# IGLICT/GaussianMesh

Hardware: AMD Instinct MI355X
Metric: frames/sec (fwd), 1M Gaussians @1080p, deform+render (higher is better)
Workload: dtype f32; 1 GPU; C3: 1000000 Gaussians bound to 15k-face torus, per-frame mesh deform + SH colour + forward render 1920x1080, 64-camera orbit, views sharded by rank; gaussians=1000000, width=1920, height=1080, sh_degree=3, frames_per_launch=4, vertex_rs=gm_mesh_rs per frame, hip_streams=4, emission_policy=2, image_only=True, work_hint=True, cov6=True, depth_plan=False, frames_redone=0, parallelism=views x1

## Files before the change

### gaussianmesh_amd/_lib.py

```python
import ctypes as C
import os
import re
import subprocess

_HERE = os.path.dirname(os.path.abspath(__file__))
CSRC = os.path.join(_HERE, "csrc")
SO_PATH = os.path.join(CSRC, "libgmesh_hip.so")
HEADER = os.path.join(os.path.dirname(_HERE), "include", "gmesh_hip.h")
_lib = None

vp, i32, i64, f32, f64, sz = C.c_void_p, C.c_int, C.c_int64, C.c_float, C.c_double, C.c_size_t

GM_BATCH_MAX = 8
GM_SCENE_OBJECTS_MAX = 32
GM_ARAP_BATCH_MAX = 64


class BatchFrame(C.Structure):
    _fields_ = [("packed", vp), ("viewmatrix", vp), ("projmatrix", vp), ("cam_pos", vp), ("tan_fovx", f32), ("tan_fovy", f32),
                ("geom_buffer", vp), ("binning_buffer", vp), ("image_buffer", vp), ("out_color", vp), ("radii", vp), ("status_host", vp)]


SIGNATURES = {
    "gm_abi_version": (i32, []),
    "gm_last_error": (C.c_char_p, []),
    "gm_geom_bytes": (sz, [i32]),
    "gm_image_bytes": (sz, [i32, i32]),
    "gm_work_hint_bytes": (sz, [i32, i32]),
    "gm_binning_bytes": (sz, [i64]),
    "gm_forward_0": (i32, [vp, i32, i32, i32, vp, i32, i32, vp, vp, vp, vp, vp, f32, vp, vp, vp, vp, vp, f32, f32, i32,
                           vp, i32, vp, C.POINTER(i32)]),
    "gm_forward_0_async": (i32, [i32, vp, i32, i32, i32, vp, i32, i32, vp, vp, vp, vp, vp, f32, vp, vp, vp, vp, vp, f32, f32, i32,
                                 vp, i32, vp, vp, vp]),
    "gm_forward_1": (i32, [vp, vp, vp, i32, i32, i32, i32, vp, i32, i32, vp, vp, vp, vp, vp, f32, vp, vp, vp, vp, vp,
                           f32, f32, i32, vp, vp, i32, vp]),
    "gm_backward": (i32, [i32, i32, i32, i32, vp, i32, i32, vp, vp, vp, vp, f32, vp, vp, vp, vp, vp, f32, f32, vp, vp, vp,
                          vp, vp, vp, vp, vp, vp, vp, vp, vp, vp, vp, i32, vp]),
    "gm_backward_p": (i32, [i32, i32, i32, i32, i32, vp, i32, i32, vp, vp, vp, vp, f32, vp, vp, vp, vp, vp, f32, f32, vp, vp, vp,
                            vp, vp, vp, vp, vp, vp, vp, vp, vp, vp, vp, i32, vp]),
    "gm_backward_aux": (i32, [i32, i32, i32, i32, i32, vp, i32, i32, vp, vp, vp, vp, f32, vp, vp, vp, vp, vp, f32, f32, vp, vp, vp,
                              vp, vp, vp, vp, vp, vp, vp, vp, vp, vp, vp, vp, vp, vp, i32, vp]),
    "gm_backward_sh_step": (i32, [i32, i32, i32, i32, i32, vp, i32, i32, vp, vp, vp, f32, vp, vp, vp, vp, vp, f32, f32, vp, vp, vp, vp, vp, vp, vp, vp, vp, vp,
                                  vp, i32, vp, vp, f32, f32, f64, f64, f64, i32, i32, vp]),
    "gm_mark_visible": (i32, [i32, vp, vp, vp, vp, vp]),
    "gm_geom_field": (vp, [vp, i32, C.c_char_p]),
    "gm_splat_floats": (i32, []),
    "gm_image_field": (vp, [vp, i32, i32, C.c_char_p]),
    "gm_binning_field": (vp, [vp, i64, i32, i32, i32, C.c_char_p]),
    "gm_knn_workspace_bytes": (sz, [i32]),
    "gm_knn": (i32, [i32, vp, vp, vp, sz, vp]),
    "gm_knn_nearest_workspace_bytes": (sz, [i32, i32]),
    "gm_knn_nearest": (i32, [i32, vp, i32, vp, vp, vp, vp, sz, vp]),
    "gm_closest_face_workspace_bytes": (sz, [i32, i32]),
    "gm_closest_face": (i32, [i32, vp, i32, vp, i32, vp, vp, vp, vp, vp, sz, vp]),
    "gm_arap_workspace_bytes": (sz, [i32]),
    "gm_arap_solve": (i32, [i32, vp, vp, vp, vp, vp, vp, i32, i32, f64, vp, vp, vp, sz, vp]),
    "gm_arap_grid_workspace_bytes": (sz, [i32]),
    "gm_arap_solve_grid": (i32, [i32, vp, vp, vp, vp, vp, vp, i32, i32, f64, vp, vp, vp, sz, vp]),
    "gm_arap_batch_workspace_bytes": (sz, [i32, i32, i32]),
    "gm_arap_solve_batch": (i32, [i32, i32, i32, vp, vp, vp, vp, vp, vp, i32, i32, f64, vp, vp, vp, sz, vp]),
    "gm_ray_mesh_workspace_bytes": (sz, [i32, i32]),
    "gm_ray_mesh": (i32, [i32, vp, vp, i32, vp, i32, vp, f32, f32, vp, vp, vp, vp, sz, vp]),
    "gm_mesh_geodesic_workspace_bytes": (sz, [i32, i32, i32]),
    "gm_mesh_geodesic": (i32, [i32, vp, vp, vp, i32, vp, vp, f32, i32, i32, vp, vp, vp, sz, vp]),
    "gm_tsdf_integrate": (i32, [i32, i32, i32, vp, vp, vp, vp, i32, i32, i32, C.POINTER(f32), f32, f32, f32, i32, vp, vp, vp]),
    "gm_surface_nets_workspace_bytes": (sz, [i32, i32, i32]),
    "gm_surface_nets": (i32, [i32, i32, i32, C.POINTER(f32), f32, vp, vp, f32, i32, vp, i32, vp, vp, vp, sz, vp]),
    "gm_deform": (i32, [i32, vp, vp, vp, vp, vp, vp, vp, vp, vp, vp, vp, vp]),
    "gm_sh_colors": (i32, [i32, i32, i32, vp, vp, vp, vp, vp, vp]),
    "gm_deform_shade": (i32, [i32, i32, i32, vp, vp, vp, vp, vp, vp, vp, vp, vp, vp, vp, vp, vp, vp, vp]),
    "gm_pack_mesh_state": (i32, [i32, vp, vp, vp, vp]),
    "gm_forward_0_deformed_async": (i32, [i32, vp, i32, i32, i32, i32, i32, vp, vp, vp, vp, vp, vp, vp, vp, vp, vp, f32, f32, vp, vp, vp, vp,
                                          i32, vp, vp, vp]),
    "gm_forward_0_deformed_stream_async": (i32, [i32, vp, i32, i32, i32, i32, i32, vp, vp, vp, vp, vp, vp, vp, vp, vp, vp, f32, f32, vp, vp, vp, vp,
                                                 i32, vp, vp, vp, vp, vp, i32]),
    "gm_depth_plan_bytes": (sz, []),
    "gm_depth_slab_bytes": (sz, [i32]),
    "gm_forward_1_geom": (i32, [i32, vp, vp, vp, i32, i32, i64, vp, i32, i32, vp, i32, vp, vp, i32, vp]),
    "gm_forward_1_aux": (i32, [i32, vp, vp, vp, i32, i32, i64, vp, i32, i32, vp, i32, vp, vp, i32, vp, vp, vp]),
    "gm_forward_status_async": (i32, [vp, i32, vp, vp]),
    "gm_forward_deformed_batch_async": (i32, [i32, i32, C.POINTER(BatchFrame), i32, i32, i32, i32, i32, vp, vp, vp, vp, vp, vp, vp, i64, i32, vp, i32, vp]),
    "gm_forward_deformed_batch_aux_async": (i32, [i32, i32, C.POINTER(BatchFrame), i32, i32, i32, i32, i32, vp, vp, vp, vp, vp, vp, vp, i64, i32, vp,
                                                  i32, vp, C.POINTER(vp), C.POINTER(vp)]),
    "gm_forward_scene_batch_async": (i32, [i32, i32, C.POINTER(BatchFrame), i32, i32, i32, i32, i32, i32, C.POINTER(i32), C.POINTER(C.c_uint),
                                           vp, vp, vp, vp, vp, vp, vp, vp, vp, i64, i32, vp, i32, vp]),
    "gm_mesh_rs_packed_batch": (i32, [i32, i32, i32, vp, C.POINTER(vp), vp, vp, vp, C.POINTER(vp), vp]),
    "gm_deform_shade_packed": (i32, [i32, i32, i32, vp, vp, vp, vp, vp, vp, vp, vp, vp, vp, vp, vp, vp]),
    "gm_cov_to_scale_rot": (i32, [i32, vp, vp, vp, vp]),
    "gm_sh_rotate": (i32, [i32, i32, i32, vp, vp, vp, vp]),
    "gm_mesh_rs": (i32, [i32, i32, vp, vp, vp, vp, vp, vp, vp, vp, vp]),
    "gm_mesh_rs_packed": (i32, [i32, i32, vp, vp, vp, vp, vp, vp, vp]),
    "gm_mesh_activate_fwd": (i32, [i32, f32] + [vp] * 10 + [vp] * 4 + [f32, vp] + [vp]),
    "gm_mesh_activate_bwd": (i32, [i32, f32] + [vp] * 10 + [vp] * 4 + [vp] * 5 + [f32, vp] + [vp]),
    "gm_plain_activate_fwd": (i32, [i32] + [vp] * 4 + [vp] * 4 + [i32, i32, vp]),
    "gm_plain_activate_bwd": (i32, [i32] + [vp] * 3 + [vp] * 4 + [i32, i32] + [vp] * 4 + [vp]),
    "gm_adam_step": (i32, [i32, vp, vp, vp, vp, vp, vp, vp, vp, vp, f64, f64, f64, i32, vp]),
    "gm_adam_step_active": (i32, [i32, vp, vp, vp, vp, vp, vp, vp, vp, vp, vp, f64, f64, f64, i32, vp]),
    "gm_densify_stats": (i32, [i32, vp, vp, vp, vp, vp, vp]),
    "gm_ssim_partials": (i64, [i32, i32, i32]),
    "gm_ssim_fwd": (i32, [vp, vp, i32, i32, i32, vp, vp, vp, vp, vp]),
    "gm_ssim_bwd": (i32, [vp, vp, vp, vp, vp, i32, i32, i32, vp, vp, vp, vp]),
    "gm_loss_combine": (i32, [vp, i64, f64, f64, f64, vp, vp]),
    "gm_ssim_fwd_u8": (i32, [vp, vp, vp, i64, vp, i32, i32, i32, vp, vp, vp, vp, vp]),
    "gm_ssim_bwd_u8": (i32, [vp, vp, vp, i64, vp, vp, vp, vp, i32, i32, i32, vp, vp, vp, vp]),
    "gm_profile_enable": (None, [i32]),
    "gm_profile_reset": (None, []),
    "gm_profile_read": (i32, [C.c_char_p, C.POINTER(C.c_double), C.POINTER(i64)]),
    "gm_debug_render_trace": (None, [vp]),
    "gm_debug_bucket_trace": (None, [vp]),
}


def header_symbols():
    txt = open(HEADER).read()
    txt = re.sub(r"/\*.*?\*/", "", txt, flags=re.S)
    return sorted(set(re.findall(r"\b(gm_[a-z0-9_]+)\s*\(", txt)))


def build(verbose=False):
    cmd = ["make", "-C", CSRC, "-j8"]
    res = subprocess.run(cmd, stdout=subprocess.PIPE, stderr=subprocess.STDOUT, text=True)
    if verbose or res.returncode != 0:
        print(res.stdout)
    if res.returncode != 0:
        raise RuntimeError("building libgmesh_hip.so failed")
    return SO_PATH


def lib():
    global _lib
    if _lib is None:
        if not os.path.exists(SO_PATH):
            raise ImportError(
                "gaussianmesh_amd: %s is missing. Build it with `python -c 'import __graft_entry__ as g; g.build()'` "
                "(or `make -C gaussianmesh_amd/csrc`). There is no CPU fallback." % SO_PATH)
        l = C.CDLL(SO_PATH)
        for name, (res, args) in SIGNATURES.items():
            fn = getattr(l, name)
            fn.restype = res
            fn.argtypes = args
        if l.gm_abi_version() != 3:
            raise ImportError("libgmesh_hip.so ABI version mismatch")
        _lib = l
    return _lib


class GmeshError(RuntimeError):
    pass


def check(rc):
    if rc != 0:
        raise GmeshError("libgmesh_hip: error %d: %s" % (rc, lib().gm_last_error().decode()))
```

### gaussianmesh_amd/csrc/gm_api.hip

```cpp
#include "gm_common.h"
#include <cmath>
#include <cstdlib>
#include "../../include/gmesh_hip.h"
#include <cstdarg>
#include <cstdio>
#include <cstring>
#include <mutex>
#include <vector>

namespace gm {

static thread_local char g_err[512] = "";

void set_error(const char* fmt, ...) {
  va_list ap;
  va_start(ap, fmt);
  vsnprintf(g_err, sizeof g_err, fmt, ap);
  va_end(ap);
}
int hip_fail(hipError_t e, const char* what, const char* file, int line) {
  set_error("HIP error %d (%s) at %s:%d in %s", (int)e, hipGetErrorString(e), file, line, what);
  return GM_ERR_HIP;
}

// ... 167 lines not shown
                       float tan_fovy, int prefiltered, int* radii, int debug, void* stream, int* num_rendered_host,
                       void* count_event) {
  if (int rc = check_policy(emission_policy)) return rc;
  FILL_ARGS(a, emission_policy)
  if (int rc = check_raster_args(a)) return rc;
  if (P == 0) { if (num_rendered_host) *num_rendered_host = 0; return GM_OK; }
  if (!geom_buffer) { set_error("geom_buffer is null"); return GM_ERR_INVALID_ARG; }
  GeomState g = GeomState::from(geom_buffer, (size_t)P);
  if (int rc = launch_arm_counters(g, a.stream)) return rc;
  if (int rc = launch_preprocess(a, g, radii)) return rc;
  return order_and_count(g, P, debug, a.stream, num_rendered_host, count_event);
}

size_t gm_depth_plan_bytes(void) { return sizeof(uint32_t) * GM_PLAN_WORDS; }
size_t gm_depth_slab_bytes(int P) {
  DepthSlab d = DepthSlab::from(nullptr, (size_t)(P > 0 ? P : 1));
  return (size_t)d.end + 256;
}

int gm_forward_0_deformed_async(int emission_policy, void* geom_buffer, int P, int deg, int M, int width, int height, const int* tri,
                                const float* w, const float* packed, const float* cov, const float* pos, const float* shs,
                                const float* opacities, const float* viewmatrix, const float* projmatrix, const float* cam_pos,
                                float tan_fovx, float tan_fovy, float* pos_out, float* cov6_out, float* rgb_out, int* radii, int debug,
                                void* stream, int* num_rendered_host, void* count_event) {
  return gm_forward_0_deformed_stream_async(emission_policy, geom_buffer, P, deg, M, width, height, tri, w, packed, cov, pos, shs, opacities,
                                            viewmatrix, projmatrix, cam_pos, tan_fovx, tan_fovy, pos_out, cov6_out, rgb_out, radii, debug, stream,
                                            num_rendered_host, count_event, nullptr, nullptr, 0);
}

int gm_forward_0_deformed_stream_async(int emission_policy, void* geom_buffer, int P, int deg, int M, int width, int height, const int* tri,
                                       const float* w, const float* packed, const float* cov, const float* pos, const float* shs,
                                       const float* opacities, const float* viewmatrix, const float* projmatrix, const float* cam_pos,
                                       float tan_fovx, float tan_fovy, float* pos_out, float* cov6_out, float* rgb_out, int* radii,
                                       int debug, void* stream, int* num_rendered_host, void* count_event, void* depth_slab,
                                       unsigned int* depth_plan, int flags) {
  if (int rc = check_policy(emission_policy)) return rc;
  if (flags & ~(GM_STREAM_DIRECT | GM_STREAM_COV6)) { set_error("gm_forward_0_deformed_stream: unknown flags 0x%x", flags); return GM_ERR_INVALID_ARG; }
  const int direct = flags & GM_STREAM_DIRECT;
  const bool cov6 = (flags & GM_STREAM_COV6) != 0;
  if (direct && (!depth_slab || !depth_plan)) { set_error("gm_forward_0_deformed_stream: direct placement needs depth_slab and depth_plan"); return GM_ERR_INVALID_ARG; }
  if (P < 0 || width <= 0 || height <= 0) { set_error("invalid sizes P=%d W=%d H=%d", P, width, height); return GM_ERR_INVALID_ARG; }
  if (int rc = check_tile_grid(width, height)) return rc;
  if (P == 0) { if (num_rendered_host) *num_rendered_host = 0; return GM_OK; }
  if (deg < 0 || deg > 3 || M != 16) { set_error("gm_forward_0_deformed: needs SH rows of M == 16 coefficients, degree 0..3"); return GM_ERR_INVALID_ARG; }
  if (!geom_buffer || !tri || !w || !packed || !cov || !pos || !shs || !opacities || !viewmatrix || !projmatrix || !cam_pos) {
    set_error("gm_forward_0_deformed: null required input"); return GM_ERR_INVALID_ARG;
  }
  const int nout = (pos_out != nullptr) + (cov6_out != nullptr) + (rgb_out != nullptr);
  if (nout != 0 && nout != 3) { set_error("gm_forward_0_deformed: pass pos_out, cov6_out and rgb_out together or none"); return GM_ERR_INVALID_ARG; }
  RasterArgs a{};
  a.P = P; a.D = deg; a.M = M; a.W = width; a.H = height; a.opacities = opacities; a.viewmatrix = viewmatrix; a.projmatrix = projmatrix;
  a.cam_pos = cam_pos; a.scale_modifier = 1.0f; a.tan_fovx = tan_fovx; a.tan_fovy = tan_fovy; a.debug = debug; a.tile_cull = emission_policy;
  a.stream = reinterpret_cast<hipStream_t>(stream);
  if (TileGrid(width, height, emission_policy).ptiles > 65536) { set_error("too many list tiles for emission policy %d", emission_policy); return GM_ERR_INVALID_ARG; }
  GeomState g = GeomState::from(geom_buffer, (size_t)P);
  if (direct) {
    DepthSlab d = DepthSlab::from(depth_slab, (size_t)P);
    if (int rc = launch_arm_direct(g, d, depth_plan, a.stream)) return rc;
    GM_HIP(hipMemsetD32Async(reinterpret_cast<hipDeviceptr_t>(g.counters + GM_CNT_DEPTH_STALE), 1, 1, a.stream));
    if (int rc = launch_deform_shade_pre(a, g, radii, deg, tri, w, packed, cov, pos, shs, pos_out, cov6_out, rgb_out, &d, cov6)) return rc;
    if (debug_stop_after() == 1) return GM_OK;
    return launch_depth_order_direct(g, d, depth_plan, P, debug, a.stream, num_rendered_host, reinterpret_cast<hipEvent_t>(count_event));
  }
  if (int rc = launch_arm_counters(g, a.stream)) return rc;
  if (int rc = launch_deform_shade_pre(a, g, radii, deg, tri, w, packed, cov, pos, shs, pos_out, cov6_out, rgb_out, nullptr, cov6)) return rc;
  if (int rc = order_and_count(g, P, debug, a.stream, num_rendered_host, count_event)) return rc;
  if (depth_plan && debug_stop_after() != 1) return launch_publish_depth_plan(g, depth_plan, a.stream);
  return GM_OK;
}

static int forward_1_impl(int emission_policy, void* geom_buffer, void* binning_buffer, void* image_buffer, int P, int num_rendered,
                          int64_t binning_capacity, const float* background, int width, int height, float* out_color, int debug, void* stream,
                          int* status_host, int flags, unsigned int* work_hint, bool aux, float* out_depth, float* out_alpha) {
  if (int rc = check_policy(emission_policy)) return rc;
  if (flags & ~(GM_FWD_IMAGE_ONLY | GM_FWD_EXACT_EXPONENT)) { set_error("unknown flags 0x%x", flags); return GM_ERR_INVALID_ARG; }
  if ((flags & GM_FWD_IMAGE_ONLY) && (flags & GM_FWD_EXACT_EXPONENT)) {
    set_error("GM_FWD_EXACT_EXPONENT is for a forward a backward pass follows: not together with GM_FWD_IMAGE_ONLY"); return GM_ERR_INVALID_ARG;
  }
  if (P < 0 || width <= 0 || height <= 0) { set_error("invalid sizes P=%d W=%d H=%d", P, width, height); return GM_ERR_INVALID_ARG; }
  if (int rc = check_tile_grid(width, height)) return rc;
  if (!image_buffer || !out_color || !background) { set_error("null image_buffer / out_color / background"); return GM_ERR_INVALID_ARG; }
  const bool device_count = num_rendered < 0;
  const int64_t cap = device_count ? binning_capacity : (int64_t)num_rendered;
  if (cap < 0) { set_error("negative binning capacity"); return GM_ERR_INVALID_ARG; }
  if (P > 0 && (!geom_buffer || (cap > 0 && !binning_buffer))) { set_error("null scratch buffer"); return GM_ERR_INVALID_ARG; }
  hipStream_t st = reinterpret_cast<hipStream_t>(stream);
  const int mode = emission_policy;
  ImageState img = ImageState::from(image_buffer, width, height);
  const int tiles = TileGrid(width, height, mode).ptiles;
  if (tiles > 65536) { set_error("too many list tiles for emission policy %d", mode); return GM_ERR_INVALID_ARG; }
  GeomState g = GeomState::from(geom_buffer, (size_t)(P > 0 ? P : 1));
  BinningState b = BinningState::from(binning_buffer, (size_t)cap);
  const int slot = sort_final_slot(tiles);
  bool order_done = false;
  if (const int stop = debug_stop_after()) {
    if (stop <= 2) return GM_OK;
    if (stop == 3) return launch_duplicate(g, b, P, width, height, mode, (size_t)cap, debug, st);
  }
  if (P > 0 && cap > 0) {
    if (int rc = launch_duplicate(g, b, P, width, height, mode, (size_t)cap, debug, st)) return rc;
    if (int rc = launch_tile_sort(g, b, img, (size_t)cap, device_count ? g.counters + GM_CNT_RENDERED : nullptr, tiles, &order_done, work_hint, debug, st)) return rc;
    if (slot == 0)
      if (int rc = launch_tile_ranges(g, b, slot, img, (int)cap, device_count ? g.counters + GM_CNT_RENDERED : nullptr, tiles, debug, st)) return rc;
  } else {
    GM_HIP(hipMemsetAsync(img.ranges, 0, sizeof(uint2) * (size_t)tiles, st));
  }
  if (!order_done)
    if (int rc = launch_tile_order(img, tiles, work_hint, debug, st)) return rc;
  if (status_host && P == 0) {
    status_host[0] = 0; status_host[1] = 0; status_host[2] = mode; status_host[3] = 0;
    status_host = nullptr;
  }
  if (debug_stop_after() == 4) return GM_OK;
  return launch_render_fwd(g, b.pairs[slot], img, width, height, mode, background, out_color, status_host, (flags & GM_FWD_IMAGE_ONLY) != 0,
                           work_hint, debug, st, (flags & GM_FWD_EXACT_EXPONENT) != 0, nullptr, out_depth, out_alpha, aux,
                           P > 0 ? g.counters : nullptr);
}

int gm_forward_1_geom(int emission_policy, void* geom_buffer, void* binning_buffer, void* image_buffer, int P, int num_rendered,
                      int64_t binning_capacity, const float* background, int width, int height, float* out_color, int debug, void* stream,
                      int* status_host, int flags, unsigned int* work_hint) {
  return forward_1_impl(emission_policy, geom_buffer, binning_buffer, image_buffer, P, num_rendered, binning_capacity, background, width, height,
                        out_color, debug, stream, status_host, flags, work_hint, false, nullptr, nullptr);
}

static bool overlaps(const float* a, size_t na, const float* b, size_t nb) {
  return a && b && a < b + nb && b < a + na;
}

int gm_forward_1_aux(int emission_policy, void* geom_buffer, void* binning_buffer, void* image_buffer, int P, int num_rendered,
                     int64_t binning_capacity, const float* background, int width, int height, float* out_color, int debug, void* stream,
                     int* status_host, int flags, unsigned int* work_hint, float* out_depth, float* out_alpha) {
  if (width > 0 && height > 0) {
    const size_t HW = (size_t)width * height;
    if (overlaps(out_depth, HW, out_color, 3 * HW) || overlaps(out_alpha, HW, out_color, 3 * HW) || overlaps(out_depth, HW, out_alpha, HW)) {
      set_error("gm_forward_1_aux: out_depth / out_alpha overlap out_color or each other"); return GM_ERR_INVALID_ARG;
    }
  }
  return forward_1_impl(emission_policy, geom_buffer, binning_buffer, image_buffer, P, num_rendered, binning_capacity, background, width, height,
                        out_color, debug, stream, status_host, flags, work_hint, true, out_depth, out_alpha);
}

struct SceneRows {
  int n_objects;
  const int* object_rows;
  const unsigned int* deformed;
  const float *scales, *rots;
};

static int check_scene_batch(const char* who, const SceneRows& sc, int K, const gm_batch_frame* frames, int P, int width, int height,
                             int64_t binning_capacity, const int* tri, const float* w, const float* cov) {
  const int n = sc.n_objects;
  if (n < 0 || n > GM_SCENE_OBJECTS_MAX) { set_error("%s: n_objects = %d, not in 0..GM_SCENE_OBJECTS_MAX (%d)", who, n, GM_SCENE_OBJECTS_MAX); return GM_ERR_INVALID_ARG; }
  for (int j = 0; j <= n; j++) {
    const int r = sc.object_rows[j];
    if (r < 0 || r > P || (j > 0 && r < sc.object_rows[j - 1])) {
      set_error("%s: object_rows must ascend within [0, P = %d]: object_rows[%d] = %d", who, P, j, r); return GM_ERR_INVALID_ARG;
    }
  }
  for (int k = 0; k < K; k++) {
    const unsigned int m = sc.deformed[k];
    if (n < 32 && (m >> n)) { set_error("%s: frame %d: deformed mask 0x%x has a bit at or above n_objects = %d", who, k, m, n); return GM_ERR_INVALID_ARG; }
    if (m && !frames[k].packed) { set_error("%s: frame %d deforms objects (mask 0x%x) but packed is NULL", who, k, m); return GM_ERR_INVALID_ARG; }
    if (m && (!tri || !w || !cov)) { set_error("%s: frame %d deforms objects: tri / w / cov are required", who, k); return GM_ERR_INVALID_ARG; }
  }
  struct Range { uintptr_t a; size_t n; int k; const char* what; };
  Range rg[6 * GM_BATCH_MAX];
  int nr = 0;
  const size_t HW = (size_t)width * height;
  for (int k = 0; k < K; k++) {
    const gm_batch_frame& f = frames[k];
    rg[nr++] = {reinterpret_cast<uintptr_t>(f.geom_buffer), gm_geom_bytes(P), k, "geometry"};
    rg[nr++] = {reinterpret_cast<uintptr_t>(f.binning_buffer), gm_binning_bytes(binning_capacity), k, "binning"};
    rg[nr++] = {reinterpret_cast<uintptr_t>(f.image_buffer), gm_image_bytes(width, height), k, "image"};
    rg[nr++] = {reinterpret_cast<uintptr_t>(f.out_color), 3 * HW * sizeof(float), k, "out_color"};
    if (f.radii) rg[nr++] = {reinterpret_cast<uintptr_t>(f.radii), (size_t)P * sizeof(int), k, "radii"};
    if (f.status_host) rg[nr++] = {reinterpret_cast<uintptr_t>(f.status_host), 4 * sizeof(int), k, "status_host"};
  }
  for (int x = 0; x < nr; x++)
    for (int y = x + 1; y < nr; y++)
      if (rg[x].a < rg[y].a + rg[y].n && rg[y].a < rg[x].a + rg[x].n) {
        set_error("%s: frame %d's %s buffer overlaps frame %d's %s buffer", who, rg[x].k, rg[x].what, rg[y].k, rg[y].what);
        return GM_ERR_INVALID_ARG;
      }
  return GM_OK;
}

static int forward_batch_impl(const char* who, int emission_policy, int K, const gm_batch_frame* frames, int P, int deg, int M, int width, int height,
                              const int* tri, const float* w, const float* cov, const float* pos, const float* shs, const float* opacities,
                              const float* background, int64_t binning_capacity, int flags, unsigned int* work_hint, int debug, void* stream,
                              bool aux, float* const* out_depth, float* const* out_alpha, const SceneRows* scene = nullptr) {
  if (int rc = check_policy(emission_policy)) return rc;
  if (K < 1 || K > GM_BATCH_MAX || !frames) { set_error("%s: 1..%d frames", who, GM_BATCH_MAX); return GM_ERR_INVALID_ARG; }
  if (flags & ~(scene ? GM_BATCH_IMAGE_ONLY : (GM_BATCH_IMAGE_ONLY | GM_BATCH_COV6))) { set_error("%s: unknown flags 0x%x", who, flags); return GM_ERR_INVALID_ARG; }
  if (P <= 0 || width <= 0 || height <= 0) { set_error("%s: invalid sizes P=%d W=%d H=%d (an empty cloud goes through the single-frame calls)", who, P, width, height); return GM_ERR_INVALID_ARG; }
  if (deg < 0 || deg > 3 || M != 16) { set_error("%s: needs SH rows of M == 16 coefficients, degree 0..3", who); return GM_ERR_INVALID_ARG; }
  if (scene ? (!pos || !scene->scales || !scene->rots || !shs || !opacities || !background || !scene->object_rows || !scene->deformed)
            : (!tri || !w || !cov || !pos || !shs || !opacities || !background)) {
    set_error("%s: null required input", who); return GM_ERR_INVALID_ARG;
  }
  if (binning_capacity <= 0) { set_error("%s: binning_capacity must be positive (sync-free second half)", who); return GM_ERR_INVALID_ARG; }
  if (int rc = check_tile_grid(width, height)) return rc;
  const TileGrid tg(width, height, emission_policy);
  if (tg.ptiles > (1 << GM_BUCKET_BITS)) {
    set_error("%s: %dx%d has %d list tiles under policy %d; a batch needs the one-pass tile sort (<= 2048)", who, width, height, tg.ptiles, emission_policy);
    return GM_ERR_INVALID_ARG;
  }
  hipStream_t st = reinterpret_cast<hipStream_t>(stream);
  BatchFrameArgs fr[GM_BATCH_MAX];
  BatchOfs B{};
  B.frames = K;
  for (int k = 0; k < K; k++) {
    const gm_batch_frame& f = frames[k];
    if ((!scene && !f.packed) || !f.viewmatrix || !f.projmatrix || !f.cam_pos || !f.geom_buffer || !f.binning_buffer || !f.image_buffer || !f.out_color) {
      set_error("%s: frame %d has a null pointer", who, k); return GM_ERR_INVALID_ARG;
    }
    if ((reinterpret_cast<uintptr_t>(f.geom_buffer) | reinterpret_cast<uintptr_t>(f.binning_buffer) | reinterpret_cast<uintptr_t>(f.image_buffer)) & 255) {
      set_error("%s: frame %d: scratch buffers must be 256-byte aligned", who, k); return GM_ERR_INVALID_ARG;
    }
    for (int j = 0; j < k; j++)
      if (frames[j].geom_buffer == f.geom_buffer || frames[j].binning_buffer == f.binning_buffer || frames[j].image_buffer == f.image_buffer || frames[j].out_color == f.out_color) {
        set_error("%s: frames %d and %d share a buffer", who, j, k); return GM_ERR_INVALID_ARG;
      }
    fr[k].packed = f.packed; fr[k].viewmatrix = f.viewmatrix; fr[k].projmatrix = f.projmatrix; fr[k].cam_pos = f.cam_pos;
    fr[k].tan_fovx = f.tan_fovx; fr[k].tan_fovy = f.tan_fovy; fr[k].radii = f.radii;
    fr[k].g = GeomState::from(f.geom_buffer, (size_t)P);
    B.geom.d[k] = (long long)(reinterpret_cast<intptr_t>(f.geom_buffer) - reinterpret_cast<intptr_t>(frames[0].geom_buffer));
    B.binning.d[k] = (long long)(reinterpret_cast<intptr_t>(f.binning_buffer) - reinterpret_cast<intptr_t>(frames[0].binning_buffer));
    B.image.d[k] = (long long)(reinterpret_cast<intptr_t>(f.image_buffer) - reinterpret_cast<intptr_t>(frames[0].image_buffer));
    B.color.d[k] = (long long)(reinterpret_cast<intptr_t>(f.out_color) - reinterpret_cast<intptr_t>(frames[0].out_color));
    B.status[k] = f.status_host;
  }
  if (scene)
    if (int rc = check_scene_batch(who, *scene, K, frames, P, width, height, binning_capacity, tri, w, cov)) return rc;
  if (aux) {
    const size_t HW = (size_t)width * height;
    const float* r[3 * GM_BATCH_MAX];
    for (int k = 0; k < K; k++) {
      if ((out_depth && !out_depth[k]) || (out_alpha && !out_alpha[k])) { set_error("%s: frame %d: null map pointer in a non-null array", who, k); return GM_ERR_INVALID_ARG; }
      r[k] = frames[k].out_color; r[K + k] = out_depth ? out_depth[k] : nullptr; r[2 * K + k] = out_alpha ? out_alpha[k] : nullptr;
    }
    for (int i = K; i < 3 * K; i++) {
      if (!r[i]) continue;
      const int k = i % K;
      if (reinterpret_cast<uintptr_t>(r[i]) & 3) { set_error("%s: frame %d: unaligned map pointer", who, k); return GM_ERR_INVALID_ARG; }
      for (int j = 0; j < 3 * K; j++)
        if (j != i && overlaps(r[i], HW, r[j], j < K ? 3 * HW : HW)) {
          set_error("%s: frame %d's %s map overlaps a colour image or another map of the batch", who, k, i < 2 * K ? "depth" : "alpha");
          return GM_ERR_INVALID_ARG;
        }
      (i < 2 * K ? B.depth : B.alpha).d[k] = (long long)(reinterpret_cast<intptr_t>(r[i]) - reinterpret_cast<intptr_t>(r[i - k]));
    }
  }
  GeomState g = fr[0].g;
  ImageState img = ImageState::from(frames[0].image_buffer, width, height);
  BinningState b = BinningState::from(frames[0].binning_buffer, (size_t)binning_capacity);
  if (int rc = launch_arm_counters(g, st, &B)) return rc;
  if (scene) {
    if (int rc = launch_scene_shade_pre_batch(K, fr, scene->deformed, scene->n_objects, scene->object_rows, P, deg, width, height, emission_policy, pos,
                                              scene->scales, scene->rots, shs, opacities, tri, w, cov, debug, st)) return rc;
  } else if (int rc = launch_deform_shade_pre_batch(K, fr, P, deg, width, height, emission_policy, tri, w, cov, pos, shs, opacities, (flags & GM_BATCH_COV6) != 0, debug, st)) {
    return rc;
  }
  if (int rc = launch_depth_order(g, P, debug, st, nullptr, nullptr, &B)) return rc;
  if (int rc = launch_duplicate(g, b, P, width, height, emission_policy, (size_t)binning_capacity, debug, st, &B)) return rc;
  bool order_done = false;
  if (int rc = launch_tile_sort(g, b, img, (size_t)binning_capacity, g.counters + GM_CNT_RENDERED, tg.ptiles, &order_done, work_hint, debug, st, &B)) return rc;
  if (!order_done) { set_error("%s: internal: the tile pass did not produce the dispatch order", who); return GM_ERR_INVALID_ARG; }
  return launch_render_fwd(g, b.pairs[sort_final_slot(tg.ptiles)], img, width, height, emission_policy, background, frames[0].out_color, frames[0].status_host,
                           (flags & GM_BATCH_IMAGE_ONLY) != 0, work_hint, debug, st, false, &B,
                           aux && out_depth ? out_depth[0] : nullptr, aux && out_alpha ? out_alpha[0] : nullptr, aux, aux ? g.counters : nullptr);
}

int gm_forward_deformed_batch_async(int emission_policy, int K, const gm_batch_frame* frames, int P, int deg, int M, int width, int height,
                                    const int* tri, const float* w, const float* cov, const float* pos, const float* shs, const float* opacities,
                                    const float* background, int64_t binning_capacity, int flags, unsigned int* work_hint, int debug, void* stream) {
  return forward_batch_impl("gm_forward_deformed_batch", emission_policy, K, frames, P, deg, M, width, height, tri, w, cov, pos, shs, opacities,
                            background, binning_capacity, flags, work_hint, debug, stream, false, nullptr, nullptr);
}

int gm_forward_deformed_batch_aux_async(int emission_policy, int K, const gm_batch_frame* frames, int P, int deg, int M, int width, int height,
                                        const int* tri, const float* w, const float* cov, const float* pos, const float* shs, const float* opacities,
                                        const float* background, int64_t binning_capacity, int flags, unsigned int* work_hint, int debug, void* stream,
                                        float* const* out_depth, float* const* out_alpha) {
  return forward_batch_impl("gm_forward_deformed_batch_aux", emission_policy, K, frames, P, deg, M, width, height, tri, w, cov, pos, shs, opacities,
                            background, binning_capacity, flags, work_hint, debug, stream, true, out_depth, out_alpha);
}

int gm_forward_scene_batch_async(int emission_policy, int K, const gm_batch_frame* frames, int P, int deg, int M, int width, int height,
                                 int n_objects, const int* object_rows, const unsigned int* deformed, const float* pos, const float* scales,
                                 const float* rots, const float* shs, const float* opacities, const int* tri, const float* w, const float* cov,
                                 const float* background, int64_t binning_capacity, int flags, unsigned int* work_hint, int debug, void* stream) {
  const SceneRows scene{n_objects, object_rows, deformed, scales, rots};
  return forward_batch_impl("gm_forward_scene_batch", emission_policy, K, frames, P, deg, M, width, height, tri, w, cov, pos, shs, opacities,
                            background, binning_capacity, flags, work_hint, debug, stream, false, nullptr, nullptr, &scene);
}


int gm_mesh_rs_packed_batch(int K, int Vm, int nfaces, const float* V0, const float* const* V1, const int* faces, const int* adj_offsets,
                            const int* adj_faces, float* const* packed, void* stream) {
  if (K < 1 || K > GM_BATCH_MAX || Vm < 0 || nfaces < 0 || !V1 || !packed || (Vm > 0 && (!V0 || !adj_offsets || (nfaces > 0 && (!faces || !adj_faces))))) {
    set_error("gm_mesh_rs_packed_batch: bad args"); return GM_ERR_INVALID_ARG;
  }
  for (int k = 0; k < K; k++)
    if (Vm > 0 && (!V1[k] || !packed[k] || (reinterpret_cast<uintptr_t>(packed[k]) & 15))) { set_error("gm_mesh_rs_packed_batch: frame %d: null or unaligned pointer", k); return GM_ERR_INVALID_ARG; }
  return launch_mesh_rs_batch(K, Vm, V0, V1, faces, adj_offsets, adj_faces, packed, reinterpret_cast<hipStream_t>(stream));
}

int gm_forward_status_async(void* geom_buffer, int P, int* status_host, void* stream) {
  if (!status_host) { set_error("status_host is null"); return GM_ERR_INVALID_ARG; }
  if (P <= 0) { status_host[0] = 0; status_host[1] = 0; status_host[2] = 0; status_host[3] = 0; return GM_OK; }
  if (!geom_buffer) { set_error("geom_buffer is null"); return GM_ERR_INVALID_ARG; }
  GeomState g = GeomState::from(geom_buffer, (size_t)P);
  GM_HIP(hipMemcpyAsync(status_host, g.counters, 4 * sizeof(uint32_t), hipMemcpyDeviceToHost, reinterpret_cast<hipStream_t>(stream)));
  return GM_OK;
}

int gm_forward_0(void* geom_buffer, int P, int D, int M, const float* background, int width, int height,
                 const float* means3D, const float* shs, const float* colors_precomp, const float* opacities,
                 const float* scales, float scale_modifier, const float* rotations, const float* cov3D_precomp,
                 const float* viewmatrix, const float* projmatrix, const float* cam_pos, float tan_fovx,
                 float tan_fovy, int prefiltered, int* radii, int debug, void* stream, int* num_rendered) {
  if (!num_rendered) { set_error("num_rendered is null"); return GM_ERR_INVALID_ARG; }
  *num_rendered = 0;
  if (int rc = gm_forward_0_async(GM_POLICY_DEFAULT, geom_buffer, P, D, M, background, width, height, means3D, shs, colors_precomp, opacities,
                                  scales, scale_modifier, rotations, cov3D_precomp, viewmatrix, projmatrix, cam_pos, tan_fovx, tan_fovy,
                                  prefiltered, radii, debug, stream, nullptr, nullptr)) return rc;
  if (P == 0) return GM_OK;
  GeomState g = GeomState::from(geom_buffer, (size_t)P);
  uint32_t rw[2] = {0u, 0u};
  hipStream_t st = reinterpret_cast<hipStream_t>(stream);
  GM_HIP(hipMemcpyAsync(rw, g.counters + GM_CNT_RENDERED, 2 * sizeof(uint32_t), hipMemcpyDeviceToHost, st));
  GM_HIP(hipStreamSynchronize(st));
  const uint32_t r = rw[0];
  if (rw[1]) { set_error("Point is filtered although prefiltered is set. This shouldn't happen!"); return GM_ERR_INVALID_ARG; }
  if (r > 0x7FFFFFFFu) { set_error("num_rendered overflows int32 (%u)", r); return GM_ERR_INVALID_ARG; }
  *num_rendered = (int)r;
  return GM_OK;
}

int gm_forward_1(void* geom_buffer, void* binning_buffer, void* image_buffer, int P, int D, int M, int num_rendered,
                 const float* background, int width, int height, const float* means3D, const float* shs,
                 const float* colors_precomp, const float* opacities, const float* scales, float scale_modifier,
                 const float* rotations, const float* cov3D_precomp, const float* viewmatrix, const float* projmatrix,
                 const float* cam_pos, float tan_fovx, float tan_fovy, int prefiltered, float* out_color, int* radii,
                 int debug, void* stream) {
  FILL_ARGS(a, GM_POLICY_DEFAULT)
  if (int rc = check_raster_args(a)) return rc;
  (void)radii;
  if (num_rendered < 0) { set_error("negative num_rendered"); return GM_ERR_INVALID_ARG; }
  return gm_forward_1_geom(GM_POLICY_DEFAULT, geom_buffer, binning_buffer, image_buffer, P, num_rendered, 0, background, width, height, out_color,
                           debug, stream, nullptr, 0, nullptr);
}

static int backward_impl(int emission_policy, int P, int D, int M, int R, const float* background, int width, int height, const float* means3D,
                         const float* shs, const float* colors_precomp, const float* scales, float scale_modifier,
                         const float* rotations, const float* cov3D_precomp, const float* viewmatrix, const float* projmatrix,
                         const float* campos, float tan_fovx, float tan_fovy, const int* radii, void* geom_buffer,
                         void* binning_buffer, void* image_buffer, const float* dL_dpix, float* dL_dmean2D, float* dL_dconic,
                         float* dL_dopacity, float* dL_dcolor, float* dL_dmean3D, float* dL_dcov3D, float* dL_dsh,
                         float* dL_dscale, float* dL_drot, int debug, void* stream, const ShAdamArgs* sh_adam,
                         const float* dL_ddepth = nullptr, const float* dL_dalpha = nullptr, float* dL_dz = nullptr) {
  if (int rc = check_policy(emission_policy)) return rc;
  const float* opacities = reinterpret_cast<const float*>(1);
  const float* cam_pos = campos;
  const int prefiltered = 0;
  FILL_ARGS(a, emission_policy)
  if (int rc = check_raster_args(a)) return rc;
  if (P == 0) return GM_OK;
  if (!geom_buffer || !image_buffer || !dL_dpix || !dL_dmean2D || !dL_dopacity || (!shs && !dL_dcolor) ||
      !dL_dmean3D || (!scales && !dL_dcov3D) || (shs && !dL_dsh && !sh_adam) || (scales && (!dL_dscale || !dL_drot))) {
    set_error("gm_backward: null buffer"); return GM_ERR_INVALID_ARG;
  }
  GeomState g = GeomState::from(geom_buffer, (size_t)P);
  ImageState img = ImageState::from(image_buffer, width, height);
  BinningState b = BinningState::from(binning_buffer, (size_t)(R > 0 ? R : 0));
  const int slot = sort_final_slot(TileGrid(width, height, a.tile_cull).ptiles);
  GM_HIP(hipMemsetAsync(g.grad_acc, 0, sizeof(float) * 12 * (size_t)P, a.stream));
  if (R > 0) {
    if (!binning_buffer) { set_error("gm_backward: null binning buffer"); return GM_ERR_INVALID_ARG; }
    if (int rc = launch_render_bwd(g, b.pairs[slot], img, width, height, a.tile_cull, background, dL_dpix, debug, a.stream,
                                   dL_ddepth || dL_dalpha, dL_ddepth, dL_dalpha)) return rc;
  }
  if (int rc = launch_preprocess_bwd(a, g, radii, dL_dmean2D, dL_dconic, dL_dopacity, dL_dcolor, dL_dmean3D, dL_dcov3D, dL_dsh,
                                     dL_dscale, dL_drot, sh_adam)) return rc;
  if (dL_ddepth || dL_dz) return launch_depth_grad(P, g, viewmatrix, dL_dmean3D, dL_dz, a.stream);
  return GM_OK;
}

int gm_backward_aux(int emission_policy, int P, int D, int M, int R, const float* background, int width, int height, const float* means3D,
                    const float* shs, const float* colors_precomp, const float* scales, float scale_modifier,
                    const float* rotations, const float* cov3D_precomp, const float* viewmatrix, const float* projmatrix,
                    const float* campos, float tan_fovx, float tan_fovy, const int* radii, void* geom_buffer,
                    void* binning_buffer, void* image_buffer, const float* dL_dpix, float* dL_dmean2D, float* dL_dconic,
                    float* dL_dopacity, float* dL_dcolor, float* dL_dmean3D, float* dL_dcov3D, float* dL_dsh,
                    float* dL_dscale, float* dL_drot, const float* dL_ddepth, const float* dL_dalpha, float* dL_dz, int debug, void* stream) {
  if (P > 0) {
    const size_t n = (size_t)P;
    if (overlaps(dL_dz, n, dL_dmean3D, 3 * n) || overlaps(dL_dz, n, dL_dmean2D, 3 * n) || overlaps(dL_dz, n, dL_dopacity, n)) {
      set_error("gm_backward_aux: dL_dz overlaps another gradient output"); return GM_ERR_INVALID_ARG;
    }
  }
  return backward_impl(emission_policy, P, D, M, R, background, width, height, means3D, shs, colors_precomp, scales, scale_modifier, rotations, cov3D_precomp,
                       viewmatrix, projmatrix, campos, tan_fovx, tan_fovy, radii, geom_buffer, binning_buffer, image_buffer, dL_dpix, dL_dmean2D, dL_dconic,
                       dL_dopacity, dL_dcolor, dL_dmean3D, dL_dcov3D, dL_dsh, dL_dscale, dL_drot, debug, stream, nullptr, dL_ddepth, dL_dalpha, dL_dz);
}

int gm_backward_p(int emission_policy, int P, int D, int M, int R, const float* background, int width, int height, const float* means3D,
                  const float* shs, const float* colors_precomp, const float* scales, float scale_modifier,
                  const float* rotations, const float* cov3D_precomp, const float* viewmatrix, const float* projmatrix,
                  const float* campos, float tan_fovx, float tan_fovy, const int* radii, void* geom_buffer,
                  void* binning_buffer, void* image_buffer, const float* dL_dpix, float* dL_dmean2D, float* dL_dconic,
                  float* dL_dopacity, float* dL_dcolor, float* dL_dmean3D, float* dL_dcov3D, float* dL_dsh,
                  float* dL_dscale, float* dL_drot, int debug, void* stream) {
  return backward_impl(emission_policy, P, D, M, R, background, width, height, means3D, shs, colors_precomp, scales, scale_modifier, rotations, cov3D_precomp,
                       viewmatrix, projmatrix, campos, tan_fovx, tan_fovy, radii, geom_buffer, binning_buffer, image_buffer, dL_dpix, dL_dmean2D, dL_dconic,
                       dL_dopacity, dL_dcolor, dL_dmean3D, dL_dcov3D, dL_dsh, dL_dscale, dL_drot, debug, stream, nullptr);
}

int gm_backward_sh_step(int emission_policy, int P, int D, int M, int R, const float* background, int width, int height, const float* means3D,
                        float* shs, const float* scales, float scale_modifier, const float* rotations, const float* cov3D_precomp,
                        const float* viewmatrix, const float* projmatrix, const float* campos, float tan_fovx, float tan_fovy, const int* radii,
                        void* geom_buffer, void* binning_buffer, void* image_buffer, const float* dL_dpix, float* dL_dmean2D, float* dL_dopacity,
                        float* dL_dmean3D, float* dL_dcov3D, float* dL_dscale, float* dL_drot, int rows, float* exp_avg, float* exp_avg_sq,
                        float lr_dc, float lr_rest, double beta1, double beta2, double eps, int step, int debug, void* stream) {
  if (!shs || M != 16 || D < 0 || D > 3) { set_error("gm_backward_sh_step: needs the [P,16,3] SH operand"); return GM_ERR_INVALID_ARG; }
  if (rows < 0 || rows > P || !exp_avg || !exp_avg_sq || step < 1) { set_error("gm_backward_sh_step: bad optimizer state (rows %d of %d, step %d)", rows, P, step); return GM_ERR_INVALID_ARG; }
  ShAdamArgs ad;
  ad.p = shs; ad.m = exp_avg; ad.v = exp_avg_sq; ad.rows = rows;
  ad.b1 = (float)beta1; ad.b2 = (float)beta2; ad.c1 = (float)(1.0 - beta1); ad.c2 = (float)(1.0 - beta2); ad.eps = (float)eps;
  const double corr = sqrt(1.0 - pow(beta2, (double)step)) / (1.0 - pow(beta1, (double)step));
  ad.step_lo = (float)(lr_dc * corr); ad.step_hi = (float)(lr_rest * corr);
  return backward_impl(emission_policy, P, D, M, R, background, width, height, means3D, shs, nullptr, scales, scale_modifier, rotations, cov3D_precomp,
                       viewmatrix, projmatrix, campos, tan_fovx, tan_fovy, radii, geom_buffer, binning_buffer, image_buffer, dL_dpix, dL_dmean2D, nullptr,
                       dL_dopacity, nullptr, dL_dmean3D, dL_dcov3D, nullptr, dL_dscale, dL_drot, debug, stream, &ad);
}

int gm_backward(int P, int D, int M, int R, const float* background, int width, int height, const float* means3D,
                const float* shs, const float* colors_precomp, const float* scales, float scale_modifier,
                const float* rotations, const float* cov3D_precomp, const float* viewmatrix, const float* projmatrix,
                const float* campos, float tan_fovx, float tan_fovy, const int* radii, void* geom_buffer,
                void* binning_buffer, void* image_buffer, const float* dL_dpix, float* dL_dmean2D, float* dL_dconic,
                float* dL_dopacity, float* dL_dcolor, float* dL_dmean3D, float* dL_dcov3D, float* dL_dsh,
                float* dL_dscale, float* dL_drot, int debug, void* stream) {
  return gm_backward_p(GM_POLICY_DEFAULT, P, D, M, R, background, width, height, means3D, shs, colors_precomp, scales, scale_modifier, rotations,
                       cov3D_precomp, viewmatrix, projmatrix, campos, tan_fovx, tan_fovy, radii, geom_buffer, binning_buffer, image_buffer,
                       dL_dpix, dL_dmean2D, dL_dconic, dL_dopacity, dL_dcolor, dL_dmean3D, dL_dcov3D, dL_dsh, dL_dscale, dL_drot, debug, stream);
}

int gm_mark_visible(int P, const float* means3D, const float* viewmatrix, const float* projmatrix, uint8_t* present,
                    void* stream) {
  (void)projmatrix;
  if (P < 0 || (P > 0 && (!means3D || !viewmatrix || !present))) { set_error("gm_mark_visible: bad args"); return GM_ERR_INVALID_ARG; }
  return launch_mark_visible(P, means3D, viewmatrix, present, reinterpret_cast<hipStream_t>(stream));
}

int gm_splat_floats(void) { return GM_SPLAT_STRIDE; }
void* gm_geom_field(void* geom_buffer, int P, const char* name) {
  GeomState g = GeomState::from(geom_buffer, (size_t)(P > 0 ? P : 1));
  if (!strcmp(name, "splat")) return g.splat;
  if (!strcmp(name, "depth_key")) return g.depth_key;
  if (!strcmp(name, "radii")) return g.radii;
  if (!strcmp(name, "tiles_touched")) return g.tiles_touched;
  if (!strcmp(name, "bin")) return g.bin;
  if (!strcmp(name, "inst16")) return g.inst16;
  if (!strcmp(name, "bin_sorted")) return g.bin_sorted;
  if (!strcmp(name, "grad_acc")) return g.grad_acc;
  if (!strcmp(name, "cov3D")) return g.cov3D;
  if (!strcmp(name, "clamped")) return g.clamped;
  if (!strcmp(name, "order")) return g.order;
  if (!strcmp(name, "bucket_start")) return g.bucket_start;
  if (!strcmp(name, "counters")) return g.counters;
  if (!strcmp(name, "bmap")) return g.bmap;
  if (!strcmp(name, "dmap")) return g.dmap;
  return nullptr;
}
void* gm_image_field(void* image_buffer, int W, int H, const char* name) {
  ImageState s = ImageState::from(image_buffer, W, H);
  if (!strcmp(name, "final_T")) return s.final_T;
  if (!strcmp(name, "n_contrib")) return s.n_contrib;
  if (!strcmp(name, "ranges")) return s.ranges;
  if (!strcmp(name, "tile_order")) return s.tile_order;
  return nullptr;
}
void* gm_binning_field(void* binning_buffer, int64_t R, int W, int H, int emission_policy, const char* name) {
  BinningState b = BinningState::from(binning_buffer, (size_t)(R > 0 ? R : 0));
  const int slot = sort_final_slot(TileGrid(W, H, emission_policy < 0 ? 0 : (emission_policy > 3 ? 3 : emission_policy)).ptiles);
  if (!strcmp(name, "pairs")) return b.pairs[slot];
  return nullptr;
}

size_t gm_knn_workspace_bytes(int P) { return knn_workspace_bytes(P); }
int gm_knn(int P, const float* points, float* meanDists, void* workspace, size_t workspace_bytes, void* stream) {
  if (P < 0 || (P > 0 && (!points || !meanDists || !workspace))) { set_error("gm_knn: bad args"); return GM_ERR_INVALID_ARG; }
  return launch_knn(P, points, meanDists, workspace, workspace_bytes, reinterpret_cast<hipStream_t>(stream));
}

size_t gm_knn_nearest_workspace_bytes(int Pq, int Pr) { return knn_nearest_workspace_bytes(Pq, Pr); }
int gm_knn_nearest(int Pq, const float* query, int Pr, const float* ref, float* out_d2, int* out_idx, void* workspace, size_t workspace_bytes,
                   void* stream) {
  if (Pq < 0 || Pr < 0) { set_error("gm_knn_nearest: negative size"); return GM_ERR_INVALID_ARG; }
  if (Pr == 0) { set_error("gm_knn_nearest: empty reference set (Pr == 0)"); return GM_ERR_INVALID_ARG; }
  if (Pq > 0 && (!query || !ref || !out_d2 || !out_idx || !workspace)) { set_error("gm_knn_nearest: null pointer"); return GM_ERR_INVALID_ARG; }
  return launch_knn_nearest(Pq, query, Pr, ref, out_d2, out_idx, workspace, workspace_bytes, reinterpret_cast<hipStream_t>(stream));
}

size_t gm_closest_face_workspace_bytes(int N, int F) { return closest_face_workspace_bytes(N, F); }
int gm_closest_face(int N, const float* points, int Vm, const float* vertices, int F, const int* faces, float* out_d2, int* out_face,
                    float* out_closest, void* workspace, size_t workspace_bytes, void* stream) {
  if (N < 0 || Vm < 0 || F < 0) { set_error("gm_closest_face: negative size N=%d Vm=%d F=%d", N, Vm, F); return GM_ERR_INVALID_ARG; }
  if (N == 0) return GM_OK;
  if (F == 0 || Vm == 0) { set_error("gm_closest_face: empty mesh (F == %d, Vm == %d)", F, Vm); return GM_ERR_INVALID_ARG; }
  if (!points || !vertices || !faces || !out_d2 || !out_face || !workspace) { set_error("gm_closest_face: null pointer"); return GM_ERR_INVALID_ARG; }
  return launch_closest_face(N, points, Vm, vertices, F, faces, out_d2, out_face, out_closest, workspace, workspace_bytes,
                             reinterpret_cast<hipStream_t>(stream));
}

size_t gm_arap_workspace_bytes(int Vm) { return arap_workspace_bytes(Vm); }
int gm_arap_solve(int Vm, const int* row_offsets, const int* cols, const double* weights, const float* V0, const unsigned char* fixed,
                  const float* V_init, int outer_iterations, int cg_iterations, double cg_tolerance, float* V_out, double* stats,
                  void* workspace, size_t workspace_bytes, void* stream) {
  return arap_solve_checked("gm_arap_solve", launch_arap_solve, Vm, row_offsets, cols, weights, V0, fixed, V_init, outer_iterations, cg_iterations,
                            cg_tolerance, V_out, stats, workspace, workspace_bytes, stream);
}

size_t gm_arap_grid_workspace_bytes(int Vm) { return arap_grid_workspace_bytes(Vm); }
int gm_arap_solve_grid(int Vm, const int* row_offsets, const int* cols, const double* weights, const float* V0, const unsigned char* fixed,
                       const float* V_init, int outer_iterations, int cg_iterations, double cg_tolerance, float* V_out, double* stats,
                       void* workspace, size_t workspace_bytes, void* stream) {
  return arap_solve_checked("gm_arap_solve_grid", launch_arap_solve_grid, Vm, row_offsets, cols, weights, V0, fixed, V_init, outer_iterations,
                            cg_iterations, cg_tolerance, V_out, stats, workspace, workspace_bytes, stream);
}

size_t gm_arap_batch_workspace_bytes(int Vm, int B, int global_step) {
  if (Vm <= 0 || B < 1 || B > GM_ARAP_BATCH_MAX || (global_step != 0 && global_step != 1)) return 0;
  return arap_batch_workspace_bytes(Vm, B, global_step);
}
int gm_arap_solve_batch(int B, int global_step, int Vm, const int* row_offsets, const int* cols, const double* weights, const float* V0,
                        const unsigned char* fixed, const float* V_init, int outer_iterations, int cg_iterations, double cg_tolerance, float* V_out,
                        double* stats, void* workspace, size_t workspace_bytes, void* stream) {
  const char* fn = "gm_arap_solve_batch";
  if (B < 1 || B > GM_ARAP_BATCH_MAX) { set_error("%s: B = %d (1 .. %d)", fn, B, GM_ARAP_BATCH_MAX); return GM_ERR_INVALID_ARG; }
  if (global_step != 0 && global_step != 1) { set_error("%s: global_step = %d (0 column, 1 grid)", fn, global_step); return GM_ERR_INVALID_ARG; }
  if (int rc = arap_args_checked(fn, B, Vm, row_offsets, cols, weights, V0, fixed, V_init, outer_iterations, cg_iterations, cg_tolerance, V_out, stats,
                                 workspace, workspace_bytes))
    return rc;
  return launch_arap_solve_batch(B, global_step, Vm, row_offsets, cols, weights, V0, fixed, V_init, outer_iterations, cg_iterations, cg_tolerance, V_out, stats,
                                 workspace, workspace_bytes, reinterpret_cast<hipStream_t>(stream));
}

size_t gm_ray_mesh_workspace_bytes(int R, int F) { return ray_mesh_workspace_bytes(R, F); }
int gm_ray_mesh(int R, const float* origins, const float* dirs, int Vm, const float* vertices, int F, const int* faces, float t_min, float t_max,
                float* out_t, int* out_face, float* out_uv, void* workspace, size_t workspace_bytes, void* stream) {
  if (R < 0 || Vm < 0 || F < 0) { set_error("gm_ray_mesh: negative size R=%d Vm=%d F=%d", R, Vm, F); return GM_ERR_INVALID_ARG; }
  if (!(t_min >= 0.f) || t_max != t_max) { set_error("gm_ray_mesh: t_min must be >= 0 and neither bound NaN"); return GM_ERR_INVALID_ARG; }
  if (R == 0) return GM_OK;
  if (F == 0 || Vm == 0) { set_error("gm_ray_mesh: empty mesh (F == %d, Vm == %d)", F, Vm); return GM_ERR_INVALID_ARG; }
  if (!origins || !dirs || !vertices || !faces || !out_t || !out_face || !workspace) { set_error("gm_ray_mesh: null pointer"); return GM_ERR_INVALID_ARG; }
  if (ray_mesh_blocks(R, F) > 0x7FFFFFFFull) {
    set_error("gm_ray_mesh: R x F too large for one launch (%llu workgroups); split the rays", ray_mesh_blocks(R, F)); return GM_ERR_INVALID_ARG;
  }
  return launch_ray_mesh(R, origins, dirs, Vm, vertices, F, faces, t_min, t_max, out_t, out_face, out_uv, workspace, workspace_bytes,
                         reinterpret_cast<hipStream_t>(stream));
}

size_t gm_mesh_geodesic_workspace_bytes(int Vm, int B, int sweeps) { return mesh_geodesic_workspace_bytes(Vm, B, sweeps); }
int gm_mesh_geodesic(int Vm, const int* row_offsets, const int* cols, const float* lengths, int B, const int* source_offsets, const int* sources,
                     float max_distance, int sweeps, int resume, float* dist, int* unsettled, void* workspace, size_t workspace_bytes, void* stream) {
  if (Vm < 0 || B < 0) { set_error("gm_mesh_geodesic: negative size Vm=%d B=%d", Vm, B); return GM_ERR_INVALID_ARG; }
  if (sweeps < 1) { set_error("gm_mesh_geodesic: sweeps must be >= 1; got %d", sweeps); return GM_ERR_INVALID_ARG; }
  if (!(max_distance >= 0.f)) { set_error("gm_mesh_geodesic: max_distance must be >= 0 and not NaN (+inf: no cutoff)"); return GM_ERR_INVALID_ARG; }
  if (Vm == 0) return GM_OK;
  if (B < 1 || B > 65535) { set_error("gm_mesh_geodesic: B must be 1 .. 65535 source sets; got %d", B); return GM_ERR_INVALID_ARG; }
  if (!row_offsets || !cols || !lengths || !source_offsets || !sources || !dist || !unsettled || !workspace) {
    set_error("gm_mesh_geodesic: null pointer"); return GM_ERR_INVALID_ARG;
  }
  return launch_mesh_geodesic(Vm, row_offsets, cols, lengths, B, source_offsets, sources, max_distance, sweeps, resume, dist, unsettled, workspace,
                              workspace_bytes, reinterpret_cast<hipStream_t>(stream));
}

#define GM_TSDF_MAX_SAMPLES (1ll << 28)
static int check_tsdf_grid(const char* fn, int nx, int ny, int nz, int least, const float* origin, float voxel) {
  if (nx < least || ny < least || nz < least) { set_error("%s: grid %d x %d x %d (every side at least %d)", fn, nx, ny, nz, least); return GM_ERR_INVALID_ARG; }
  if ((long long)nx * ny > GM_TSDF_MAX_SAMPLES || (long long)nx * ny * nz > GM_TSDF_MAX_SAMPLES) {
    set_error("%s: grid %d x %d x %d has more than 2^28 samples", fn, nx, ny, nz); return GM_ERR_INVALID_ARG;
  }
  if (!origin) { set_error("%s: null pointer (origin)", fn); return GM_ERR_INVALID_ARG; }
  if (!(voxel > 0.f) || voxel > 3.4028234e38f || !(origin[0] - origin[0] == 0.f) || !(origin[1] - origin[1] == 0.f) || !(origin[2] - origin[2] == 0.f)) {
    set_error("%s: voxel must be positive and finite, origin finite", fn); return GM_ERR_INVALID_ARG;
  }
  return 0;
}

int gm_tsdf_integrate(int K, int H, int W, const float* depth, const float* alpha, const float* views, const float* tanfov, int nx, int ny, int nz,
                      const float* origin, float voxel, float trunc, float alpha_min, int carve, float* tsdf, float* weight, void* stream) {
  if (K < 0 || H <= 0 || W <= 0 || H > (1 << 24) || W > (1 << 24)) {
    set_error("gm_tsdf_integrate: invalid sizes K=%d H=%d W=%d", K, H, W); return GM_ERR_INVALID_ARG;
  }
  if (int rc = check_tsdf_grid("gm_tsdf_integrate", nx, ny, nz, 1, origin, voxel)) return rc;
  if (!(trunc > 0.f) || trunc > 3.4028234e38f || alpha_min != alpha_min) {
    set_error("gm_tsdf_integrate: trunc must be positive and finite, alpha_min not NaN"); return GM_ERR_INVALID_ARG;
  }
  if (!tsdf || !weight) { set_error("gm_tsdf_integrate: null pointer (tsdf / weight)"); return GM_ERR_INVALID_ARG; }
  const size_t n = (size_t)nx * ny * nz, maps = (size_t)K * H * W;
  if (overlaps(tsdf, n, weight, n)) { set_error("gm_tsdf_integrate: tsdf overlaps weight"); return GM_ERR_INVALID_ARG; }
  if (K == 0) return GM_OK;
  if (!depth || !alpha || !views || !tanfov) { set_error("gm_tsdf_integrate: null pointer"); return GM_ERR_INVALID_ARG; }
  const struct { const float* p; size_t n; const char* what; } in[4] = {{depth, maps, "depth"}, {alpha, maps, "alpha"}, {views, 16 * (size_t)K, "views"},
                                                                       {tanfov, 2 * (size_t)K, "tanfov"}};
  for (int i = 0; i < 4; i++)
    if (overlaps(tsdf, n, in[i].p, in[i].n) || overlaps(weight, n, in[i].p, in[i].n)) {
      set_error("gm_tsdf_integrate: the volume overlaps %s", in[i].what); return GM_ERR_INVALID_ARG;
    }
  return launch_tsdf_integrate(K, H, W, depth, alpha, views, tanfov, nx, ny, nz, origin, voxel, trunc, alpha_min, carve, tsdf, weight,
                               reinterpret_cast<hipStream_t>(stream));
}

size_t gm_surface_nets_workspace_bytes(int nx, int ny, int nz) { return surface_nets_workspace_bytes(nx, ny, nz); }
int gm_surface_nets(int nx, int ny, int nz, const float* origin, float voxel, const float* tsdf, const float* weight, float min_weight,
                    int max_vertices, float* out_vertices, int max_faces, int* out_faces, int* out_counts, void* workspace, size_t workspace_bytes,
                    void* stream) {
  if (int rc = check_tsdf_grid("gm_surface_nets", nx, ny, nz, 2, origin, voxel)) return rc;
  if (min_weight != min_weight) { set_error("gm_surface_nets: min_weight is NaN"); return GM_ERR_INVALID_ARG; }
  if (max_vertices < 0 || max_faces < 0) { set_error("gm_surface_nets: negative capacity (%d vertices, %d faces)", max_vertices, max_faces); return GM_ERR_INVALID_ARG; }
  if (!tsdf || !weight || !out_counts || !workspace || (max_vertices > 0 && !out_vertices) || (max_faces > 0 && !out_faces)) {
    set_error("gm_surface_nets: null pointer"); return GM_ERR_INVALID_ARG;
  }
  const size_t n = (size_t)nx * ny * nz;
  const struct { const char* p; size_t n; const char* what; } rg[6] = {
      {reinterpret_cast<const char*>(tsdf), 4 * n, "tsdf"}, {reinterpret_cast<const char*>(weight), 4 * n, "weight"},
      {reinterpret_cast<const char*>(out_vertices), 12 * (size_t)max_vertices, "out_vertices"},
      {reinterpret_cast<const char*>(out_faces), 12 * (size_t)max_faces, "out_faces"}, {reinterpret_cast<const char*>(out_counts), 8, "out_counts"},
      {reinterpret_cast<const char*>(workspace), workspace_bytes, "workspace"}};
  for (int a = 0; a < 6; a++)
    for (int b = (a < 2 ? 2 : a + 1); b < 6; b++) {
      if (!rg[a].p || !rg[b].p || !rg[a].n || !rg[b].n) continue;
      if (rg[a].p < rg[b].p + rg[b].n && rg[b].p < rg[a].p + rg[a].n) {
        set_error("gm_surface_nets: %s overlaps %s", rg[a].what, rg[b].what); return GM_ERR_INVALID_ARG;
      }
    }
  return launch_surface_nets(nx, ny, nz, origin, voxel, tsdf, weight, min_weight, max_vertices, out_vertices, max_faces, out_faces, out_counts, workspace,
                             workspace_bytes, reinterpret_cast<hipStream_t>(stream));
}

int gm_deform(int N, const int* tri, const float* w, const float* dV, const float* Rv, const float* Sv,
              const float* cov, const float* pos, float* pos_out, float* cov_out, float* rot_out, float* cov6_out,
              void* stream) {
  if (N < 0 || (N > 0 && (!tri || !w || !dV || !Rv || !Sv || !cov || !pos || !pos_out || !cov_out || !rot_out))) {
    set_error("gm_deform: bad args"); return GM_ERR_INVALID_ARG;
  }
  return launch_deform(N, tri, w, dV, Rv, Sv, cov, pos, pos_out, cov_out, rot_out, cov6_out, reinterpret_cast<hipStream_t>(stream));
}

int gm_sh_colors(int N, int deg, int M, const float* pos, const float* campos, const float* rot, const float* shs,
                 float* rgb, void* stream) {
  if (N < 0 || deg < 0 || deg > 3 || M < (deg + 1) * (deg + 1) || (N > 0 && (!pos || !campos || !shs || !rgb))) {
    set_error("gm_sh_colors: bad args"); return GM_ERR_INVALID_ARG;
  }
  return launch_sh_colors(N, deg, M, pos, campos, rot, shs, rgb, reinterpret_cast<hipStream_t>(stream));
}

int gm_deform_shade(int N, int deg, int M, const int* tri, const float* w, const float* dV, const float* Rv, const float* Sv,
                    const float* cov, const float* pos, const float* shs, const float* campos, float* pos_out, float* cov6_out,
                    float* rgb_out, float* cov_out, float* rot_out, void* stream) {
  if (N < 0 || deg < 0 || deg > 3 || M < (deg + 1) * (deg + 1) ||
      (N > 0 && (!tri || !w || !dV || !Rv || !Sv || !cov || !pos || !shs || !campos || !pos_out || !cov6_out || !rgb_out)) ||
      ((cov_out == nullptr) != (rot_out == nullptr))) {
    set_error("gm_deform_shade: bad args"); return GM_ERR_INVALID_ARG;
  }
  return launch_deform_shade(N, deg, M, tri, w, dV, Rv, Sv, cov, pos, shs, campos, pos_out, cov6_out, rgb_out, cov_out, rot_out,
                             reinterpret_cast<hipStream_t>(stream));
}

int gm_pack_mesh_state(int Vm, const float* state, const float* verts, float* packed, void* stream) {
  if (Vm < 0 || (Vm > 0 && (!state || !verts || !packed))) { set_error("gm_pack_mesh_state: bad args"); return GM_ERR_INVALID_ARG; }
  if (Vm > 0 && (reinterpret_cast<uintptr_t>(packed) & 15)) { set_error("gm_pack_mesh_state: packed must be 16-byte aligned"); return GM_ERR_INVALID_ARG; }
  return launch_pack_mesh_state(Vm, state, verts, packed, reinterpret_cast<hipStream_t>(stream));
}

int gm_deform_shade_packed(int N, int deg, int M, const int* tri, const float* w, const float* packed, const float* cov,
                           const float* pos, const float* shs, const float* campos, float* pos_out, float* cov6_out,
                           float* rgb_out, float* cov_out, float* rot_out, void* stream) {
  if (N < 0 || deg < 0 || deg > 3 || M < (deg + 1) * (deg + 1) ||
      (N > 0 && (!tri || !w || !packed || !cov || !pos || !shs || !campos || !pos_out || !cov6_out || !rgb_out)) ||
      ((cov_out == nullptr) != (rot_out == nullptr))) {
    set_error("gm_deform_shade_packed: bad args"); return GM_ERR_INVALID_ARG;
  }
  return launch_deform_shade_packed(N, deg, M, tri, w, packed, cov, pos, shs, campos, pos_out, cov6_out, rgb_out, cov_out, rot_out,
                                    reinterpret_cast<hipStream_t>(stream));
}

int gm_mesh_rs(int Vm, int nfaces, const float* V0, const float* V1, const int* faces, const int* adj_offsets, const int* adj_faces,
               float* R, float* S, float* state, void* stream) {
  if (Vm < 0 || nfaces < 0 || (Vm > 0 && (!V0 || !V1 || !adj_offsets || (nfaces > 0 && (!faces || !adj_faces)) || (!R && !S && !state)))) {
    set_error("gm_mesh_rs: bad args"); return GM_ERR_INVALID_ARG;
  }
  if ((R == nullptr) != (S == nullptr)) { set_error("gm_mesh_rs: pass R and S together"); return GM_ERR_INVALID_ARG; }
  return launch_mesh_rs(Vm, V0, V1, faces, adj_offsets, adj_faces, R, S, state, nullptr, reinterpret_cast<hipStream_t>(stream));
}

int gm_mesh_rs_packed(int Vm, int nfaces, const float* V0, const float* V1, const int* faces, const int* adj_offsets, const int* adj_faces,
                      float* packed, void* stream) {
  if (Vm < 0 || nfaces < 0 || (Vm > 0 && (!V0 || !V1 || !adj_offsets || !packed || (nfaces > 0 && (!faces || !adj_faces))))) {
    set_error("gm_mesh_rs_packed: bad args"); return GM_ERR_INVALID_ARG;
  }
  if (reinterpret_cast<uintptr_t>(packed) & 15) { set_error("gm_mesh_rs_packed: packed must be 16-byte aligned"); return GM_ERR_INVALID_ARG; }
  return launch_mesh_rs(Vm, V0, V1, faces, adj_offsets, adj_faces, nullptr, nullptr, nullptr, packed, reinterpret_cast<hipStream_t>(stream));
}

int gm_cov_to_scale_rot(int N, const float* cov, float* scales, float* rots, void* stream) {
  if (N < 0 || (N > 0 && (!cov || !scales || !rots))) { set_error("gm_cov_to_scale_rot: bad args"); return GM_ERR_INVALID_ARG; }
  if (N > 0 && (reinterpret_cast<uintptr_t>(rots) & 15)) { set_error("gm_cov_to_scale_rot: rots must be 16-byte aligned"); return GM_ERR_INVALID_ARG; }
  return launch_cov_to_scale_rot(N, cov, scales, rots, reinterpret_cast<hipStream_t>(stream));
}

int gm_sh_rotate(int N, int deg, int M, const float* shs, const float* rot, float* shs_out, void* stream) {
  if (N < 0) { set_error("gm_sh_rotate: negative N = %d", N); return GM_ERR_INVALID_ARG; }
  if (N == 0) return GM_OK;
  if (deg < 0 || deg > 3) { set_error("gm_sh_rotate: degree %d out of range 0..3", deg); return GM_ERR_INVALID_ARG; }
  if (M < (deg + 1) * (deg + 1)) { set_error("gm_sh_rotate: rows of M = %d coefficients hold no degree %d", M, deg); return GM_ERR_INVALID_ARG; }
  if (!shs || !rot || !shs_out) { set_error("gm_sh_rotate: null pointer"); return GM_ERR_INVALID_ARG; }
  const size_t n = (size_t)N * (size_t)M * 3;
  if (shs_out != shs && overlaps(shs_out, n, shs, n)) { set_error("gm_sh_rotate: shs_out overlaps shs without being equal to it"); return GM_ERR_INVALID_ARG; }
  if (overlaps(shs_out, n, rot, (size_t)N * 9)) { set_error("gm_sh_rotate: shs_out overlaps rot"); return GM_ERR_INVALID_ARG; }
  return launch_sh_rotate(N, deg, M, shs, rot, shs_out, reinterpret_cast<hipStream_t>(stream));
}

int64_t gm_ssim_partials(int planes, int H, int W) {
  if (planes < 0 || H < 0 || W < 0) return 0;
  return (int64_t)planes * ((H + 31) / 32) * ((W + 31) / 32);
}

int gm_ssim_fwd(const float* img1, const float* img2, int planes, int H, int W, float* dS_dmu1, float* dS_dE11, float* dS_dE12,
                float* partial, void* stream) {
  if (planes < 0 || H < 0 || W < 0) { set_error("gm_ssim_fwd: negative size"); return GM_ERR_INVALID_ARG; }
  if (planes == 0 || H == 0 || W == 0) return GM_OK;
  if (!img1 || !img2 || !partial) { set_error("gm_ssim_fwd: null image or partial buffer"); return GM_ERR_INVALID_ARG; }
  const int nmaps = (dS_dmu1 != nullptr) + (dS_dE11 != nullptr) + (dS_dE12 != nullptr);
  if (nmaps != 0 && nmaps != 3) { set_error("gm_ssim_fwd: pass all three derivative maps or none"); return GM_ERR_INVALID_ARG; }
  if (planes > 65535) { set_error("gm_ssim_fwd: at most 65535 image planes per call"); return GM_ERR_INVALID_ARG; }
  return launch_ssim_fwd(img1, img2, planes, H, W, dS_dmu1, dS_dE11, dS_dE12, partial, reinterpret_cast<hipStream_t>(stream));
}

int gm_ssim_bwd(const float* img1, const float* img2, const float* dS_dmu1, const float* dS_dE11, const float* dS_dE12, int planes,
                int H, int W, const float* g_ssim, const float* g_l1, float* dL_dimg1, void* stream) {
  if (planes < 0 || H < 0 || W < 0) { set_error("gm_ssim_bwd: negative size"); return GM_ERR_INVALID_ARG; }
  if (planes == 0 || H == 0 || W == 0) return GM_OK;
  if (!img1 || !img2 || !dS_dmu1 || !dS_dE11 || !dS_dE12 || !g_ssim || !dL_dimg1) { set_error("gm_ssim_bwd: null argument"); return GM_ERR_INVALID_ARG; }
  if (planes > 65535) { set_error("gm_ssim_bwd: at most 65535 image planes per call"); return GM_ERR_INVALID_ARG; }
  return launch_ssim_bwd(img1, img2, dS_dmu1, dS_dE11, dS_dE12, planes, H, W, g_ssim, g_l1, dL_dimg1, reinterpret_cast<hipStream_t>(stream));
}

static int check_u8_target(const char* who, const unsigned char* rgb, const unsigned char* mask, int64_t mask_plane_stride,
                           const float* background, int planes, int H, int W) {
  char msg[160];
  if (planes != 3) { snprintf(msg, sizeof msg, "%s: an 8-bit target has 3 planes", who); set_error(msg); return GM_ERR_INVALID_ARG; }
  if (!rgb) { snprintf(msg, sizeof msg, "%s: null rgb", who); set_error(msg); return GM_ERR_INVALID_ARG; }
  if (mask && !background) { snprintf(msg, sizeof msg, "%s: a mask needs the background colour (device float[3])", who); set_error(msg); return GM_ERR_INVALID_ARG; }
  if (mask && mask_plane_stride != 0 && mask_plane_stride < (int64_t)H * W) {
    snprintf(msg, sizeof msg, "%s: mask_plane_stride is 0 (one shared plane) or at least H*W", who); set_error(msg); return GM_ERR_INVALID_ARG;
  }
  return GM_OK;
}

int gm_ssim_fwd_u8(const float* img1, const uint8_t* rgb, const uint8_t* mask, int64_t mask_plane_stride, const float* background,
                   int planes, int H, int W, float* dS_dmu1, float* dS_dE11, float* dS_dE12, float* partial, void* stream) {
  if (planes < 0 || H < 0 || W < 0) { set_error("gm_ssim_fwd_u8: negative size"); return GM_ERR_INVALID_ARG; }
  if (planes == 0 || H == 0 || W == 0) return GM_OK;
  if (!img1 || !partial) { set_error("gm_ssim_fwd_u8: null image or partial buffer"); return GM_ERR_INVALID_ARG; }
  const int nmaps = (dS_dmu1 != nullptr) + (dS_dE11 != nullptr) + (dS_dE12 != nullptr);
  if (nmaps != 0 && nmaps != 3) { set_error("gm_ssim_fwd_u8: pass all three derivative maps or none"); return GM_ERR_INVALID_ARG; }
  if (int rc = check_u8_target("gm_ssim_fwd_u8", rgb, mask, mask_plane_stride, background, planes, H, W)) return rc;
  return launch_ssim_fwd_u8(img1, rgb, mask, (size_t)mask_plane_stride, background, H, W, dS_dmu1, dS_dE11, dS_dE12, partial,
                            reinterpret_cast<hipStream_t>(stream));
}

int gm_ssim_bwd_u8(const float* img1, const uint8_t* rgb, const uint8_t* mask, int64_t mask_plane_stride, const float* background,
                   const float* dS_dmu1, const float* dS_dE11, const float* dS_dE12, int planes, int H, int W, const float* g_ssim,
                   const float* g_l1, float* dL_dimg1, void* stream) {
  if (planes < 0 || H < 0 || W < 0) { set_error("gm_ssim_bwd_u8: negative size"); return GM_ERR_INVALID_ARG; }
  if (planes == 0 || H == 0 || W == 0) return GM_OK;
  if (!img1 || !dS_dmu1 || !dS_dE11 || !dS_dE12 || !g_ssim || !dL_dimg1) { set_error("gm_ssim_bwd_u8: null argument"); return GM_ERR_INVALID_ARG; }
  if (int rc = check_u8_target("gm_ssim_bwd_u8", rgb, mask, mask_plane_stride, background, planes, H, W)) return rc;
  return launch_ssim_bwd_u8(img1, rgb, mask, (size_t)mask_plane_stride, background, dS_dmu1, dS_dE11, dS_dE12, H, W, g_ssim, g_l1,
                            dL_dimg1, reinterpret_cast<hipStream_t>(stream));
}

int gm_loss_combine(const float* partial, int64_t n_partials, double c_ssim, double c_l1, double offset, float* out, void* stream) {
  if (n_partials < 0) { set_error("gm_loss_combine: negative count"); return GM_ERR_INVALID_ARG; }
  if (!out || (n_partials > 0 && !partial)) { set_error("gm_loss_combine: null partial / out"); return GM_ERR_INVALID_ARG; }
  return launch_loss_combine(partial, (long long)n_partials, c_ssim, c_l1, offset, out, reinterpret_cast<hipStream_t>(stream));
}

static int fill_act(ActArgs& a, int N, float alpha, const float* bc, const float* dist, const float* scaling, const float* rotation,
                    const float* opacity, const float* v1, const float* v2, const float* v3, const float* normal, const float* r) {
  if (N < 0) { set_error("gm_mesh_activate: negative N"); return GM_ERR_INVALID_ARG; }
  if (N > 0 && (!bc || !dist || !scaling || !rotation || !opacity || !v1 || !v2 || !v3 || !normal || !r)) {
    set_error("gm_mesh_activate: null input"); return GM_ERR_INVALID_ARG;
  }
  if (N > 0 && (reinterpret_cast<uintptr_t>(rotation) & 15)) { set_error("gm_mesh_activate: rotation must be 16-byte aligned"); return GM_ERR_INVALID_ARG; }
  a.N = N; a.alpha = alpha; a.bc = bc; a.dist = dist; a.scaling = scaling; a.rotation = rotation; a.opacity = opacity;
  a.v1 = v1; a.v2 = v2; a.v3 = v3; a.normal = normal; a.r = r;
  return GM_OK;
}

int gm_mesh_activate_fwd(int N, float alpha, const float* bc, const float* dist, const float* scaling, const float* rotation,
                         const float* opacity, const float* v1, const float* v2, const float* v3, const float* normal, const float* r,
                         float* xyz, float* scales, float* rots, float* opac, float mr_weight, float* mr_partial, void* stream) {
  ActArgs a;
  if (int rc = fill_act(a, N, alpha, bc, dist, scaling, rotation, opacity, v1, v2, v3, normal, r)) return rc;
  if (N > 0 && (!xyz || !scales || !rots || !opac || (reinterpret_cast<uintptr_t>(rots) & 15))) {
    set_error("gm_mesh_activate_fwd: null output or unaligned rots"); return GM_ERR_INVALID_ARG;
  }
  return launch_mesh_activate_fwd(a, xyz, scales, rots, opac, mr_weight, mr_partial, reinterpret_cast<hipStream_t>(stream));
}

int gm_mesh_activate_bwd(int N, float alpha, const float* bc, const float* dist, const float* scaling, const float* rotation,
                         const float* opacity, const float* v1, const float* v2, const float* v3, const float* normal, const float* r,
                         const float* d_xyz, const float* d_scales, const float* d_rots, const float* d_opac, float* d_bc, float* d_dist,
                         float* d_scaling, float* d_rotation, float* d_opacity, float mr_weight, const float* d_mr, void* stream) {
  ActArgs a;
  if (int rc = fill_act(a, N, alpha, bc, dist, scaling, rotation, opacity, v1, v2, v3, normal, r)) return rc;
  if (N > 0 && (!d_bc || !d_dist || !d_scaling || !d_rotation || !d_opacity || (reinterpret_cast<uintptr_t>(d_rotation) & 15) ||
                (d_rots && (reinterpret_cast<uintptr_t>(d_rots) & 15)))) {
    set_error("gm_mesh_activate_bwd: null output or unaligned rotation gradient"); return GM_ERR_INVALID_ARG;
  }
  return launch_mesh_activate_bwd(a, d_xyz, d_scales, d_rots, d_opac, d_bc, d_dist, d_scaling, d_rotation, d_opacity, mr_weight, d_mr,
                                  reinterpret_cast<hipStream_t>(stream));
}

int gm_plain_activate_fwd(int N, const float* xyz, const float* scaling, const float* rotation, const float* opacity, float* out_xyz,
                          float* out_scales, float* out_rots, float* out_opac, int row0, int capacity, void* stream) {
  if (N < 0 || row0 < 0 || capacity < 0 || (long long)row0 + N > capacity) {
    set_error("gm_plain_activate_fwd: rows [%d, %d + %d) do not fit a capacity of %d", row0, row0, N, capacity); return GM_ERR_INVALID_ARG;
  }
  if (N > 0 && (!xyz || !scaling || !rotation || !opacity || !out_xyz || !out_scales || !out_rots || !out_opac)) {
    set_error("gm_plain_activate_fwd: null pointer"); return GM_ERR_INVALID_ARG;
  }
  if (N > 0 && ((reinterpret_cast<uintptr_t>(rotation) | reinterpret_cast<uintptr_t>(out_rots)) & 15)) {
    set_error("gm_plain_activate_fwd: rotation / out_rots must be 16-byte aligned"); return GM_ERR_INVALID_ARG;
  }
  const size_t r = (size_t)row0;
  return launch_plain_activate_fwd(N, xyz, scaling, rotation, opacity, out_xyz + 3 * r, out_scales + 3 * r, out_rots + 4 * r, out_opac + r,
                                   reinterpret_cast<hipStream_t>(stream));
}

int gm_plain_activate_bwd(int N, const float* scaling, const float* rotation, const float* opacity, const float* g_xyz, const float* g_scales,
                          const float* g_rots, const float* g_opac, int row0, int capacity, float* d_xyz, float* d_scaling, float* d_rotation,
                          float* d_opacity, void* stream) {
  if (N < 0 || row0 < 0 || capacity < 0 || (long long)row0 + N > capacity) {
    set_error("gm_plain_activate_bwd: rows [%d, %d + %d) do not fit a capacity of %d", row0, row0, N, capacity); return GM_ERR_INVALID_ARG;
  }
  if (N > 0 && (!scaling || !rotation || !opacity || !d_xyz || !d_scaling || !d_rotation || !d_opacity)) {
    set_error("gm_plain_activate_bwd: null pointer"); return GM_ERR_INVALID_ARG;
  }
  if (N > 0 && ((reinterpret_cast<uintptr_t>(rotation) | reinterpret_cast<uintptr_t>(d_rotation) | reinterpret_cast<uintptr_t>(g_rots)) & 15)) {
    set_error("gm_plain_activate_bwd: rotation / g_rots / d_rotation must be 16-byte aligned"); return GM_ERR_INVALID_ARG;
  }
  const size_t r = (size_t)row0;
  return launch_plain_activate_bwd(N, scaling, rotation, opacity, g_xyz ? g_xyz + 3 * r : nullptr, g_scales ? g_scales + 3 * r : nullptr,
                                   g_rots ? g_rots + 4 * r : nullptr, g_opac ? g_opac + r : nullptr, d_xyz, d_scaling, d_rotation, d_opacity,
                                   reinterpret_cast<hipStream_t>(stream));
}

int gm_adam_step(int count, float* const* params, const float* const* grads, float* const* exp_avg, float* const* exp_avg_sq,
                 const uint64_t* sizes, const float* lr, const float* lr_rest, const uint32_t* period, const uint32_t* split,
                 double beta1, double beta2, double eps, int step, void* stream) {
  return gm_adam_step_active(count, params, grads, exp_avg, exp_avg_sq, sizes, lr, lr_rest, period, split, nullptr, beta1, beta2, eps, step, stream);
}

int gm_adam_step_active(int count, float* const* params, const float* const* grads, float* const* exp_avg, float* const* exp_avg_sq,
                        const uint64_t* sizes, const float* lr, const float* lr_rest, const uint32_t* period, const uint32_t* split,
                        const uint32_t* active, double beta1, double beta2, double eps, int step, void* stream) {
  if (count < 0 || count > 8 || step < 1) { set_error("gm_adam_step: 0..8 tensors per call, step >= 1"); return GM_ERR_INVALID_ARG; }
  if (count > 0 && (!params || !grads || !exp_avg || !exp_avg_sq || !sizes || !lr)) { set_error("gm_adam_step: null table"); return GM_ERR_INVALID_ARG; }
  AdamTable tab;
  tab.count = 0; tab.b1 = (float)beta1; tab.b2 = (float)beta2; tab.eps = (float)eps;
  tab.omb1 = (float)(1.0 - beta1); tab.omb2 = (float)(1.0 - beta2);
  const double corr = sqrt(1.0 - pow(beta2, (double)step)) / (1.0 - pow(beta1, (double)step));
  for (int i = 0; i < count; i++) {
    if (sizes[i] == 0) continue;
    if (!params[i] || !grads[i] || !exp_avg[i] || !exp_avg_sq[i]) { set_error("gm_adam_step: null tensor %d", i); return GM_ERR_INVALID_ARG; }
    if ((reinterpret_cast<uintptr_t>(params[i]) | reinterpret_cast<uintptr_t>(grads[i]) | reinterpret_cast<uintptr_t>(exp_avg[i]) |
         reinterpret_cast<uintptr_t>(exp_avg_sq[i])) & 15) { set_error("gm_adam_step: tensor %d is not 16-byte aligned", i); return GM_ERR_INVALID_ARG; }
    AdamTensor& t = tab.t[tab.count++];
    t.p = params[i]; t.g = grads[i]; t.m = exp_avg[i]; t.v = exp_avg_sq[i]; t.n = sizes[i];
    t.step_lo = (float)(lr[i] * corr);
    t.period = period ? period[i] : 0u; t.split = split ? split[i] : 0u;
    if (t.period & 3u) { set_error("gm_adam_step: period must be a multiple of 4"); return GM_ERR_INVALID_ARG; }
    t.active = (active && active[i] && t.period && active[i] < t.period) ? active[i] : 0u;
    if (t.active && (t.n % t.period) != 0) { set_error("gm_adam_step_active: tensor %d is not a whole number of periods", i); return GM_ERR_INVALID_ARG; }
    t.step_hi = (float)((lr_rest && t.period) ? lr_rest[i] * corr : lr[i] * corr);
  }
  return launch_adam(tab, reinterpret_cast<hipStream_t>(stream));
}

int gm_densify_stats(int N, const int* radii, const float* viewspace_grad, float* max_radii2D, float* grad_accum, float* denom, void* stream) {
  if (N < 0 || (N > 0 && (!radii || !viewspace_grad || !max_radii2D || !grad_accum || !denom))) {
    set_error("gm_densify_stats: bad args"); return GM_ERR_INVALID_ARG;
  }
  return launch_densify_stats(N, radii, viewspace_grad, max_radii2D, grad_accum, denom, reinterpret_cast<hipStream_t>(stream));
}

void gm_profile_enable(int on) { g_prof_on = on != 0; }
void gm_profile_reset(void) {
  drain_profile();
  std::lock_guard<std::mutex> lk(g_prof_mu);
  for (int i = 0; i < ST_COUNT; i++) { g_ms[i] = 0; g_n[i] = 0; }
}
int gm_profile_read(const char* stage, double* total_ms, int64_t* launches) {
  drain_profile();
  for (int i = 0; i < ST_COUNT; i++)
    if (!strcmp(stage, kStageNames[i])) {
      if (total_ms) *total_ms = g_ms[i];
      if (launches) *launches = g_n[i];
      return GM_OK;
    }
  set_error("unknown stage '%s'", stage);
  return GM_ERR_INVALID_ARG;
}

}
```

### gaussianmesh_amd/csrc/gm_common.h

```cpp
#pragma once
#include <hip/hip_runtime.h>
#include <stdint.h>
#include <stddef.h>
#include <string>
#include <type_traits>

#define GM_TILE 16
#define GM_WAVE 64

namespace gm {

void set_error(const char* fmt, ...);
int hip_fail(hipError_t e, const char* what, const char* file, int line);

#define GM_HIP(call)                                                            \
  do {                                                                          \
    hipError_t _e = (call);                                                     \
    if (_e != hipSuccess) return gm::hip_fail(_e, #call, __FILE__, __LINE__);   \
  } while (0)

#define GM_LAUNCH_CHECK(debug, stream)                                          \
  do {                                                                          \
    GM_HIP(hipGetLastError());                                                  \
    if (debug) GM_HIP(hipStreamSynchronize(stream));                            \
// ... 36 lines not shown
#endif
#ifndef GM_TP_ROUNDS
#define GM_TP_ROUNDS 16
#endif
#ifndef GM_BS_ROUNDS
#define GM_BS_ROUNDS 16
#endif
#define GM_BK_ROUNDS_MIN (GM_DP_ROUNDS < GM_TP_ROUNDS ? GM_DP_ROUNDS : GM_TP_ROUNDS)
#define GM_BK_TILE (4 * GM_BK_ROUNDS_MIN * 64)
#define GM_BK_CHUNK 32
static inline size_t bk_blocks(size_t n) { return (n + GM_BK_TILE - 1) / GM_BK_TILE; }
static inline size_t bk_chunks(size_t n) { return (bk_blocks(n) + GM_BK_CHUNK - 1) / GM_BK_CHUNK; }
#define GM_ACC_SLOTS 512
static inline size_t bk_acc_words(size_t n) { return GM_ACC_SLOTS + (bk_chunks(n) << GM_BUCKET_BITS); }
#define GM_COARSE_SHIFT 20
#define GM_COARSE_BINS 2048
#define GM_COARSE_COPIES 8
__host__ __device__ __forceinline__ uint32_t coarse_index(uint32_t bin, uint32_t copy) {
  return ((bin & 15u) * GM_COARSE_COPIES + copy) * (GM_COARSE_BINS / 16u) + (bin >> 4);
}
#define GM_BUCKET_BUDGET 1792
#define GM_CNT_RENDERED 0
#define GM_CNT_PREFILTER 1
#define GM_CNT_POLICY 2
#define GM_CNT_REFUSED 3
#define GM_CNT_VISIBLE 4
#define GM_CNT_NBUCKETS 5
#define GM_CNT_CMIN 6
#define GM_CNT_CMAX 7
#define GM_CNT_DIRECT_FAIL 8
#define GM_CNT_DEPTH_STALE 9
#define GM_CNT_COUNT 32
#define GM_SLOTS 256
#define GM_SLOT_STRIDE 32

#define GM_BIN_COUNT_SAT 0xFFFFu
__host__ __device__ __forceinline__ uint4 bin_pack(uint32_t x0, uint32_t y0, uint32_t w, uint32_t h, uint32_t count, unsigned long long mask) {
  const uint32_t c = count < GM_BIN_COUNT_SAT ? count : GM_BIN_COUNT_SAT;
  return make_uint4(x0 | ((c & 0xFu) << 12) | (y0 << 16) | (((c >> 4) & 0xFu) << 28),
                    w | (((c >> 8) & 0xFu) << 12) | (h << 16) | ((c >> 12) << 28), (uint32_t)mask, (uint32_t)(mask >> 32));
}
__host__ __device__ __forceinline__ uint32_t bin_x0(const uint4& b) { return b.x & 0xFFFu; }
__host__ __device__ __forceinline__ uint32_t bin_y0(const uint4& b) { return (b.x >> 16) & 0xFFFu; }
__host__ __device__ __forceinline__ uint32_t bin_w(const uint4& b) { return b.y & 0xFFFu; }
__host__ __device__ __forceinline__ uint32_t bin_h(const uint4& b) { return (b.y >> 16) & 0xFFFu; }
__host__ __device__ __forceinline__ uint32_t bin_count(const uint4& b) {
  return ((b.x >> 12) & 0xFu) | ((b.x >> 28) << 4) | (((b.y >> 12) & 0xFu) << 8) | ((b.y >> 28) << 12);
}

#ifndef GM_SPLAT_STRIDE
#define GM_SPLAT_STRIDE 9
#endif
typedef float gm_f4u __attribute__((ext_vector_type(4), aligned(4)));
__device__ __forceinline__ float4 splat_row(const float4* splat, size_t id, int row) {
  const gm_f4u v = *reinterpret_cast<const gm_f4u*>(reinterpret_cast<const float*>(splat) + GM_SPLAT_STRIDE * id + 4 * row);
  return make_float4(v.x, v.y, v.z, v.w);
}
__device__ __forceinline__ float splat_blue(const float4* splat, size_t id) { return reinterpret_cast<const float*>(splat)[GM_SPLAT_STRIDE * id + 8]; }
__device__ __forceinline__ void splat_store(float4* splat, size_t id, float x, float y, float conx, float cony, float conz, float opacity,
                                            float r, float g, float b, float depth) {
  float* p = reinterpret_cast<float*>(splat) + GM_SPLAT_STRIDE * id;
  *reinterpret_cast<gm_f4u*>(p) = gm_f4u{x, y, conx, cony};
  *reinterpret_cast<gm_f4u*>(p + 4) = gm_f4u{conz, opacity, r, g};
  if (GM_SPLAT_STRIDE >= 12) *reinterpret_cast<gm_f4u*>(p + 8) = gm_f4u{b, depth, 0.f, 0.f};
  else p[8] = b;
}

struct GeomState {
  float4* splat;
  int* radii;
  uint32_t* tiles_touched;
  uint4* bin;
  uint16_t* inst16;
  float* cov3D;
  uint8_t* clamped;
  uint32_t* depth_key;
  uint2* dpairs[2];
  uint32_t* order;
  uint4* bin_sorted;
  uint32_t* hist;
  uint32_t* bucket_start;
  uint32_t* chunk_inst;
  uint32_t* dmap;
  uint32_t* bmap;
  uint32_t* slots;
  uint32_t* coarse;
  uint32_t* counters;
  uint32_t* acc;
  float* grad_acc;
  static GeomState from(void* buf, size_t P) {
    char* p = reinterpret_cast<char*>(buf);
    GeomState g;
    constexpr size_t ND = size_t(1) << GM_BUCKET_BITS;
    g.splat = reinterpret_cast<float4*>(carve<float>(p, GM_SPLAT_STRIDE * P + 4));
    g.radii = carve<int>(p, P);
    g.tiles_touched = carve<uint32_t>(p, P);
    g.bin = carve<uint4>(p, P);
    g.inst16 = carve<uint16_t>(p, P);
    g.cov3D = carve<float>(p, 6 * P);
    g.clamped = carve<uint8_t>(p, P);
    g.depth_key = carve<uint32_t>(p, P);
    g.dpairs[0] = carve<uint2>(p, P);
    g.dpairs[1] = carve<uint2>(p, P);
    g.order = carve<uint32_t>(p, P);
    g.bin_sorted = carve<uint4>(p, P);
    g.hist = carve<uint32_t>(p, ND * bk_blocks(P));
    g.bucket_start = carve<uint32_t>(p, ND + 1);
    g.dmap = carve<uint32_t>(p, GM_COARSE_BINS);
    g.bmap = carve<uint32_t>(p, 2 * ND);
    const size_t nchunk = (P / GM_SCAN_ITEMS + 1 + 63) & ~size_t(63);
    g.slots = carve<uint32_t>(p, GM_SLOT_STRIDE * GM_SLOTS + GM_CNT_COUNT + GM_COARSE_COPIES * GM_COARSE_BINS + bk_acc_words(P) + nchunk);
    g.counters = g.slots + GM_SLOT_STRIDE * GM_SLOTS;
    g.coarse = g.counters + GM_CNT_COUNT;
    g.acc = g.coarse + GM_COARSE_COPIES * GM_COARSE_BINS;
    g.chunk_inst = g.acc + bk_acc_words(P);
    g.arm_words = GM_SLOT_STRIDE * GM_SLOTS + GM_CNT_COUNT + GM_COARSE_COPIES * GM_COARSE_BINS + bk_acc_words(P) + nchunk;
    g.grad_acc = carve<float>(p, 12 * P);
    g.end = p;
    return g;
  }
  size_t arm_words;
  char* end;
};

#define GM_PLAN_SLOTS 16
#define GM_PLAN_WORDS (2 + GM_PLAN_SLOTS + GM_PLAN_SLOTS * GM_COARSE_BINS)
#define GM_SLAB_CNT_STRIDE 32
#define GM_SLAB_HDR_WORDS 64
static inline uint32_t slab_capacity(size_t P) {
  size_t c = 256;
  while (c < 4096 && c * 128 < P) c <<= 1;
  return (uint32_t)c;
}
struct DepthSlab {
  uint32_t* hdr;
  uint32_t* cnt;
  uint2* pairs;
  uint4* recs;
  uint32_t cap;
  static DepthSlab from(void* buf, size_t P) {
    char* p = reinterpret_cast<char*>(buf);
    DepthSlab d;
    constexpr size_t ND = size_t(1) << GM_BUCKET_BITS;
    d.cap = slab_capacity(P);
    d.hdr = carve<uint32_t>(p, GM_SLAB_HDR_WORDS);
    d.cnt = carve<uint32_t>(p, ND * GM_SLAB_CNT_STRIDE);
    d.pairs = carve<uint2>(p, ND * d.cap);
    d.recs = carve<uint4>(p, ND * d.cap);
    d.end = p;
    return d;
  }
  char* end;
};

struct ImageState {
  float* final_T;
  uint32_t* n_contrib;
  uint2* ranges;
  uint32_t* tile_order;
  uint32_t* tile_work;
  uint32_t* tile_order_bwd;
  uint32_t* epoch;
  static ImageState from(void* buf, int W, int H) {
    char* p = reinterpret_cast<char*>(buf);
    const size_t N = (size_t)W * H;
    const size_t T = (size_t)((W + GM_TILE - 1) / GM_TILE) * ((H + GM_TILE - 1) / GM_TILE);
    ImageState s;
    s.final_T = carve<float>(p, N);
    s.n_contrib = carve<uint32_t>(p, N);
    s.ranges = carve<uint2>(p, T);
    s.tile_order = carve<uint32_t>(p, T);
    s.tile_work = carve<uint32_t>(p, T);
    s.tile_order_bwd = carve<uint32_t>(p, T);
    s.epoch = carve<uint32_t>(p, 1);
    s.end = p;
    return s;
  }
  char* end;
};

struct BinningState {
  uint2* pairs[2];
  uint32_t* hist;
  uint32_t* acc;
  static BinningState from(void* buf, size_t R) {
    char* p = reinterpret_cast<char*>(buf);
    BinningState b;
    const size_t Rp = R ? R : 1;
    constexpr size_t ND = size_t(1) << GM_BUCKET_BITS;
    b.pairs[0] = carve<uint2>(p, Rp);
    b.pairs[1] = carve<uint2>(p, Rp);
    b.hist = carve<uint32_t>(p, ND * bk_blocks(Rp));
    b.acc = carve<uint32_t>(p, bk_acc_words(Rp));
    b.end = p;
    return b;
  }
  char* end;
};

#define GM_BATCH_MAX 8
#define GM_SCENE_OBJECTS_MAX 32
struct FrameOfs { long long d[GM_BATCH_MAX]; };
template <class T>
__device__ __forceinline__ T* frame_ptr(T* p, const FrameOfs& o) {
  typedef typename std::conditional<std::is_const<T>::value, const char, char>::type B;
  return p ? reinterpret_cast<T*>(reinterpret_cast<B*>(p) + o.d[blockIdx.z]) : p;
}
struct BatchOfs {
  int frames;
  FrameOfs geom, binning, image, color;
  int* status[GM_BATCH_MAX];
  FrameOfs depth, alpha;
};
static inline BatchOfs single_frame() { BatchOfs b{}; b.frames = 1; return b; }

static inline int tile_bits(int tiles) {
  int b = 1;
  while ((1 << b) < tiles) b++;
  return b;
}
static inline int sort_final_slot(int tiles) { return tiles <= (1 << GM_BUCKET_BITS) ? 1 : 0; }

#define GM_KEY_MASK_SHIFT 16
#define GM_KEY_TILE_MASK 0xFFFFu
static inline int tile_shift_of(int mode) { return mode >= 2 ? mode - 1 : 0; }
struct TileGrid {
  int s, gx, gy, pgx, pgy, ptiles;
  TileGrid(int W, int H, int mode) {
    s = tile_shift_of(mode);
    gx = (W + GM_TILE - 1) / GM_TILE; gy = (H + GM_TILE - 1) / GM_TILE;
    pgx = (gx + (1 << s) - 1) >> s; pgy = (gy + (1 << s) - 1) >> s;
    ptiles = pgx * pgy;
  }
};

struct RasterArgs {
  int P, D, M, W, H;
  const float *background, *means3D, *shs, *colors_precomp, *opacities, *scales, *rotations, *cov3D_precomp;
  const float *viewmatrix, *projmatrix, *cam_pos;
  float scale_modifier, tan_fovx, tan_fovy;
  int prefiltered, debug;
  int tile_cull;
  hipStream_t stream;
};

int launch_preprocess(const RasterArgs& a, GeomState& g, int* radii);
int launch_mark_visible(int P, const float* means3D, const float* view, uint8_t* present, hipStream_t s);
int launch_preprocess_bwd(const RasterArgs& a, GeomState& g, const int* radii, float* dL_dmean2D, float* dL_dconic,
                          float* dL_dopacity, float* dL_dcolor, float* dL_dmean3D, float* dL_dcov3D, float* dL_dsh,
                          float* dL_dscale, float* dL_drot, const struct ShAdamArgs* sh_adam = nullptr);

int radix_sort_pairs(uint32_t* keys[2], uint32_t* vals[2], uint32_t* hist, uint32_t* digit_total, size_t n,
                     int bits, bool iota_values, int debug, hipStream_t s);

int launch_depth_order(GeomState& g, int P, int debug, hipStream_t s, int* num_rendered_host, hipEvent_t count_event, const BatchOfs* bt = nullptr);
int launch_arm_counters(GeomState& g, hipStream_t s, const BatchOfs* bt = nullptr);
int launch_arm_direct(GeomState& g, DepthSlab& d, uint32_t* plan, hipStream_t s);
int launch_depth_order_direct(GeomState& g, DepthSlab& d, uint32_t* plan, int P, int debug, hipStream_t s, int* num_rendered_host, hipEvent_t count_event);
int launch_publish_depth_plan(GeomState& g, uint32_t* plan, hipStream_t s);
int launch_duplicate(GeomState& g, BinningState& b, int P, int W, int H, int tile_cull, size_t capacity, int debug, hipStream_t s, const BatchOfs* bt = nullptr);
int launch_tile_sort(GeomState& g, BinningState& b, ImageState& img, size_t n, const uint32_t* n_dev, int tiles, bool* order_done,
                     uint32_t* work_hint, int debug, hipStream_t s, const BatchOfs* bt = nullptr);
int launch_tile_ranges(const GeomState& g, BinningState& b, int slot, ImageState& img, int R, const uint32_t* R_dev, int tiles, int debug, hipStream_t s);
int launch_tile_order(ImageState& img, int tiles, uint32_t* work_hint, int debug, hipStream_t s);
int launch_render_fwd(const GeomState& g, const uint2* pairs, ImageState& img, int W, int H, int mode,
                      const float* background, float* out_color, int* status_host, bool image_only, uint32_t* work_hint, int debug,
                      hipStream_t s, bool exact_exponent = false, const BatchOfs* bt = nullptr,
                      float* out_depth = nullptr, float* out_alpha = nullptr, bool aux = false,
                      uint32_t* aux_latch = nullptr);
int launch_render_bwd(const GeomState& g, const uint2* pairs, ImageState& img, int W, int H, int mode,
                      const float* background, const float* dL_dpix, int debug, hipStream_t s,
                      bool aux = false, const float* dL_ddepth = nullptr, const float* dL_dalpha = nullptr);
int launch_depth_grad(int P, const GeomState& g, const float* viewmatrix, float* dL_dmean3D, float* dL_dz, hipStream_t s);

int launch_deform(int N, const int* tri, const float* w, const float* dV, const float* Rv, const float* Sv,
                  const float* cov, const float* pos, float* pos_out, float* cov_out, float* rot_out, float* cov6_out,
                  hipStream_t s);
int launch_sh_colors(int N, int deg, int M, const float* pos, const float* campos, const float* rot,
                     const float* shs, float* rgb, hipStream_t s);
int launch_deform_shade(int N, int deg, int M, const int* tri, const float* w, const float* dV, const float* Rv, const float* Sv,
                        const float* cov, const float* pos, const float* shs, const float* campos, float* pos_out,
                        float* cov6_out, float* rgb_out, float* cov_out, float* rot_out, hipStream_t s);
int launch_deform_shade_pre(const RasterArgs& r, GeomState& g, int* radii, int deg, const int* tri, const float* w, const float* packed,
                            const float* cov, const float* pos, const float* shs, float* pos_out, float* cov6_out, float* rgb_out,
                            const struct DepthSlab* slab = nullptr, bool cov6 = false);
int launch_pack_mesh_state(int Vm, const float* state, const float* verts, float* packed, hipStream_t s);
int launch_deform_shade_packed(int N, int deg, int M, const int* tri, const float* w, const float* packed, const float* cov,
                               const float* pos, const float* shs, const float* campos, float* pos_out, float* cov6_out,
                               float* rgb_out, float* cov_out, float* rot_out, hipStream_t s);
int launch_cov_to_scale_rot(int N, const float* cov, float* scales, float* rots, hipStream_t s);
int launch_sh_rotate(int N, int deg, int M, const float* shs, const float* rot, float* shs_out, hipStream_t s);
int launch_mesh_rs(int Vm, const float* V0, const float* V1, const int* faces, const int* adj_offsets, const int* adj_faces, float* R,
                   float* S, float* state, float* packed, hipStream_t s);
int launch_mesh_rs_batch(int frames, int Vm, const float* V0, const float* const* V1, const int* faces, const int* adj_offsets, const int* adj_faces,
                         float* const* packed, hipStream_t s);
struct BatchFrameArgs {
  const float *packed, *viewmatrix, *projmatrix, *cam_pos;
  float tan_fovx, tan_fovy;
  GeomState g;
  int* radii;
};
int launch_deform_shade_pre_batch(int frames, const BatchFrameArgs* fr, int P, int deg, int W, int H, int tile_cull, const int* tri, const float* w,
                                  const float* cov, const float* pos, const float* shs, const float* opacities, bool cov6, int debug, hipStream_t s);
int launch_scene_shade_pre_batch(int frames, const BatchFrameArgs* fr, const uint32_t* deformed, int n_obj, const int* object_rows, int P, int deg,
                                 int W, int H, int tile_cull, const float* pos, const float* scales, const float* rots, const float* shs,
                                 const float* opacities, const int* tri, const float* w, const float* cov, int debug, hipStream_t s);
int launch_ssim_fwd(const float* img1, const float* img2, int planes, int H, int W, float* d_mu1, float* d_e11, float* d_e12,
                    float* partial, hipStream_t s);
int launch_loss_combine(const float* partial, long long n, double c_ssim, double c_l1, double offset, float* out, hipStream_t s);
int launch_ssim_bwd(const float* img1, const float* img2, const float* d_mu1, const float* d_e11, const float* d_e12, int planes,
                    int H, int W, const float* g_ssim, const float* g_l1, float* dL_dimg1, hipStream_t s);
int launch_ssim_fwd_u8(const float* img1, const unsigned char* rgb, const unsigned char* mask, size_t mask_stride, const float* bg, int H,
                       int W, float* d_mu1, float* d_e11, float* d_e12, float* partial, hipStream_t s);
int launch_ssim_bwd_u8(const float* img1, const unsigned char* rgb, const unsigned char* mask, size_t mask_stride, const float* bg,
                       const float* d_mu1, const float* d_e11, const float* d_e12, int H, int W, const float* g_ssim, const float* g_l1,
                       float* dL_dimg1, hipStream_t s);
struct ActArgs {
  int N;
  float alpha;
  const float *bc, *dist, *scaling, *rotation, *opacity, *v1, *v2, *v3, *normal, *r;
};
struct AdamTensor {
  float* p; const float* g; float* m; float* v;
  unsigned long long n;
  float step_lo, step_hi;
  unsigned period, split;
  unsigned active;
};
struct AdamTable { AdamTensor t[8]; int count; float b1, b2, eps, omb1, omb2; };
__device__ __forceinline__ void adam_update(float& p, float& m, float& v, float g, float b1, float b2, float c1, float c2, float eps, float st) {
  m = __builtin_fmaf(b1, m, c1 * g);
  v = __builtin_fmaf(b2, v, c2 * g * g);
  p -= st * m / (sqrtf(v) + eps);
}
struct ShAdamArgs {
  float *p, *m, *v;
  int rows;
  float b1, b2, c1, c2, eps, step_lo, step_hi;
};
int launch_mesh_activate_fwd(const ActArgs& a, float* xyz, float* scales, float* rots, float* opac, float mr_weight, float* mr_partial,
                             hipStream_t s);
int launch_mesh_activate_bwd(const ActArgs& a, const float* d_xyz, const float* d_scales, const float* d_rots, const float* d_opac,
                             float* d_bc, float* d_dist, float* d_scaling, float* d_rotation, float* d_opacity, float mr_weight,
                             const float* d_mr, hipStream_t s);
int launch_plain_activate_fwd(int N, const float* xyz_in, const float* scaling, const float* rotation, const float* opacity, float* xyz,
                              float* scales, float* rots, float* opac, hipStream_t s);
int launch_plain_activate_bwd(int N, const float* scaling, const float* rotation, const float* opacity, const float* g_xyz,
                              const float* g_scales, const float* g_rots, const float* g_opac, float* d_xyz, float* d_scaling,
                              float* d_rotation, float* d_opacity, hipStream_t s);
int launch_adam(const AdamTable& tab, hipStream_t s);
int launch_densify_stats(int N, const int* radii, const float* grad2d, float* max_radii2D, float* grad_accum, float* denom, hipStream_t s);
int launch_knn(int P, const float* points, float* meanDists, void* ws, size_t ws_bytes, hipStream_t s);
size_t knn_workspace_bytes(int P);
int launch_knn_nearest(int Pq, const float* query, int Pr, const float* ref, float* out_d2, int* out_idx, void* ws, size_t ws_bytes,
                       hipStream_t s);
size_t knn_nearest_workspace_bytes(int Pq, int Pr);
int launch_closest_face(int N, const float* points, int Vm, const float* vertices, int F, const int* faces, float* out_d2, int* out_face,
                        float* out_closest, void* ws, size_t ws_bytes, hipStream_t s);
size_t closest_face_workspace_bytes(int N, int F);
int launch_arap_solve(int Vm, const int* row_offsets, const int* cols, const double* weights, const float* V0, const unsigned char* fixed,
                      const float* V_init, int outer_iterations, int cg_iterations, double cg_tolerance, float* V_out, double* stats, void* ws,
                      size_t ws_bytes, hipStream_t s);
size_t arap_workspace_bytes(int Vm);
int launch_arap_solve_grid(int Vm, const int* row_offsets, const int* cols, const double* weights, const float* V0, const unsigned char* fixed,
                           const float* V_init, int outer_iterations, int cg_iterations, double cg_tolerance, float* V_out, double* stats, void* ws,
                           size_t ws_bytes, hipStream_t s);
size_t arap_grid_workspace_bytes(int Vm);
int launch_arap_solve_batch(int B, int global_step, int Vm, const int* row_offsets, const int* cols, const double* weights, const float* V0,
                            const unsigned char* fixed, const float* V_init, int outer_iterations, int cg_iterations, double cg_tolerance, float* V_out,
                            double* stats, void* ws, size_t ws_bytes, hipStream_t s);
size_t arap_batch_workspace_bytes(int Vm, int B, int global_step);
int launch_ray_mesh(int R, const float* origins, const float* dirs, int Vm, const float* vertices, int F, const int* faces, float t_min,
                    float t_max, float* out_t, int* out_face, float* out_uv, void* ws, size_t ws_bytes, hipStream_t s);
size_t ray_mesh_workspace_bytes(int R, int F);
unsigned long long ray_mesh_blocks(int R, int F);
int launch_mesh_geodesic(int Vm, const int* row_offsets, const int* cols, const float* lengths, int B, const int* source_offsets,
                         const int* sources, float max_distance, int sweeps, int resume, float* dist, int* unsettled, void* ws,
                         size_t ws_bytes, hipStream_t s);
size_t mesh_geodesic_workspace_bytes(int Vm, int B, int sweeps);
int launch_tsdf_integrate(int K, int H, int W, const float* depth, const float* alpha, const float* views, const float* tans, int nx, int ny,
                          int nz, const float* origin, float voxel, float trunc, float alpha_min, int carve, float* tsdf, float* weight,
                          hipStream_t s);
int launch_surface_nets(int nx, int ny, int nz, const float* origin, float voxel, const float* tsdf, const float* weight, float min_weight,
                        int max_vertices, float* out_vertices, int max_faces, int* out_faces, int* out_counts, void* ws, size_t ws_bytes,
                        hipStream_t s);
size_t surface_nets_workspace_bytes(int nx, int ny, int nz);

__device__ __forceinline__ uint32_t lanes_below(unsigned long long mask) {
  return __builtin_amdgcn_mbcnt_hi((uint32_t)(mask >> 32), __builtin_amdgcn_mbcnt_lo((uint32_t)mask, 0u));
}

}
```

### gaussianmesh_amd/csrc/gm_deform.hip

```cpp
#include "gm_common.h"
#pragma clang fp contract(off)
#include "gm_sh.h"
#include "gm_stage.h"
#include "gm_pre_body.h"
#include <cstdlib>

namespace gm {

__global__ __launch_bounds__(256) void deform_kernel(int N, const int* __restrict__ tri, const float* __restrict__ w,
                                                     const float* __restrict__ dV, const float* __restrict__ Rv,
                                                     const float* __restrict__ Sv, const float* __restrict__ cov,
                                                     const float* __restrict__ pos, float* __restrict__ pos_out,
                                                     float* __restrict__ cov_out, float* __restrict__ rot_out,
                                                     float* __restrict__ cov6_out) {
  const int i = blockIdx.x * 256 + threadIdx.x;
  if (i >= N) return;
  const int t0 = tri[3 * (size_t)i], t1 = tri[3 * (size_t)i + 1], t2 = tri[3 * (size_t)i + 2];
  const float w0 = w[3 * (size_t)i], w1 = w[3 * (size_t)i + 1], w2 = w[3 * (size_t)i + 2];
  float d[3], Rb[9], Sb[9];
#pragma unroll
  for (int k = 0; k < 3; k++) d[k] = (w0 * dV[3 * (size_t)t0 + k] + w1 * dV[3 * (size_t)t1 + k]) + w2 * dV[3 * (size_t)t2 + k];
#pragma unroll
  for (int k = 0; k < 9; k++) {
    Rb[k] = (w0 * Rv[9 * (size_t)t0 + k] + w1 * Rv[9 * (size_t)t1 + k]) + w2 * Rv[9 * (size_t)t2 + k];
    Sb[k] = (w0 * Sv[9 * (size_t)t0 + k] + w1 * Sv[9 * (size_t)t1 + k]) + w2 * Sv[9 * (size_t)t2 + k];
  }
  float Rt[9], RS[9], A[9], C[9], O[9];
#pragma unroll
  for (int a = 0; a < 3; a++)
#pragma unroll
    for (int b = 0; b < 3; b++) Rt[3 * a + b] = Rb[3 * b + a];
#pragma unroll
  for (int a = 0; a < 3; a++)
#pragma unroll
    for (int b = 0; b < 3; b++) RS[3 * a + b] = (Rt[3 * a] * Sb[b] + Rt[3 * a + 1] * Sb[3 + b]) + Rt[3 * a + 2] * Sb[6 + b];
#pragma unroll
  for (int k = 0; k < 9; k++) C[k] = cov[9 * (size_t)i + k];
#pragma unroll
  for (int a = 0; a < 3; a++)
#pragma unroll
    for (int b = 0; b < 3; b++) A[3 * a + b] = (RS[3 * a] * C[b] + RS[3 * a + 1] * C[3 + b]) + RS[3 * a + 2] * C[6 + b];
#pragma unroll
  for (int a = 0; a < 3; a++)
#pragma unroll
    for (int b = 0; b < 3; b++) O[3 * a + b] = (A[3 * a] * RS[3 * b] + A[3 * a + 1] * RS[3 * b + 1]) + A[3 * a + 2] * RS[3 * b + 2];
#pragma unroll
  for (int k = 0; k < 9; k++) { cov_out[9 * (size_t)i + k] = O[k]; rot_out[9 * (size_t)i + k] = Rt[k]; }
#pragma unroll
  for (int k = 0; k < 3; k++) pos_out[3 * (size_t)i + k] = pos[3 * (size_t)i + k] + d[k];
  if (cov6_out) {
    float* o = cov6_out + 6 * (size_t)i;
    o[0] = O[0]; o[1] = O[1]; o[2] = O[2]; o[3] = O[4]; o[4] = O[5]; o[5] = O[8];
  }
}

int launch_deform(int N, const int* tri, const float* w, const float* dV, const float* Rv, const float* Sv,
                  const float* cov, const float* pos, float* pos_out, float* cov_out, float* rot_out, float* cov6_out,
                  hipStream_t s) {
  StageScope sc(ST_DEFORM, s);
  if (N > 0)
    hipLaunchKernelGGL(deform_kernel, dim3((N + 255) / 256), dim3(256), 0, s, N, tri, w, dV, Rv, Sv, cov, pos, pos_out, cov_out,
                       rot_out, cov6_out);
  GM_HIP(hipGetLastError());
  return 0;
}

__global__ __launch_bounds__(256) void sh_colors_kernel(int N, int deg, int M, const float* __restrict__ pos,
                                                        const float* __restrict__ campos, const float* __restrict__ rot,
                                                        const float* __restrict__ shs, float* __restrict__ rgb) {
  const int i = blockIdx.x * 256 + threadIdx.x;
  if (i >= N) return;
  float dx = pos[3 * (size_t)i] - campos[0], dy = pos[3 * (size_t)i + 1] - campos[1], dz = pos[3 * (size_t)i + 2] - campos[2];
  const float len = sqrtf(dx * dx + dy * dy + dz * dz);
  dx = dx / len; dy = dy / len; dz = dz / len;
  float x = dx, y = dy, z = dz;
  if (rot) {
    const float* R = rot + 9 * (size_t)i;
    x = (R[0] * dx + R[3] * dy) + R[6] * dz;
    y = (R[1] * dx + R[4] * dy) + R[7] * dz;
    z = (R[2] * dx + R[5] * dy) + R[8] * dz;
  }
  float sh[48];
  load_sh(shs, i, M, (deg + 1) * (deg + 1), sh);
#pragma unroll
  for (int ch = 0; ch < 3; ch++) {
    const float r = sh_channel(deg, [&](int k) { return sh[3 * k + ch]; }, x, y, z);
    rgb[3 * (size_t)i + ch] = fmaxf(r + 0.5f, 0.0f);
  }
}

int launch_sh_colors(int N, int deg, int M, const float* pos, const float* campos, const float* rot,
                     const float* shs, float* rgb, hipStream_t s) {
  StageScope sc(ST_SH_COLORS, s);
  if (N > 0) hipLaunchKernelGGL(sh_colors_kernel, dim3((N + 255) / 256), dim3(256), 0, s, N, deg, M, pos, campos, rot, shs, rgb);
  GM_HIP(hipGetLastError());
  return 0;
}

constexpr int DS_THREADS = 64;

__device__ __forceinline__ void stage_sh_rows(float4* l_sh, const float* __restrict__ shs, size_t row0, int nrows, int t, size_t i) {
  if (nrows == DS_THREADS) {
    const char* gsh = reinterpret_cast<const char*>(shs + row0 * 48) + t * 16;
#pragma unroll
    for (int q = 0; q < 12; q++) dma16(gsh + q * 1024, reinterpret_cast<char*>(l_sh) + q * 1024);
  } else if (t < nrows) {
#pragma unroll
    for (int c = 0; c < 12; c++) l_sh[t * 12 + c] = reinterpret_cast<const float4*>(shs)[i * 12 + c];
  }
}

__device__ __forceinline__ void load_rest_cov(float* C, const float* __restrict__ cov, size_t i, bool live, bool cov6) {
  if (!live) {
#pragma unroll
    for (int k = 0; k < 9; k++) C[k] = 0.f;
    return;
  }
  if (cov6) {
    float c6[6];
#pragma unroll
    for (int k = 0; k < 6; k++) c6[k] = cov[i * 6 + k];
    C[0] = c6[0]; C[1] = c6[1]; C[2] = c6[2]; C[3] = c6[1]; C[4] = c6[3]; C[5] = c6[4]; C[6] = c6[2]; C[7] = c6[4]; C[8] = c6[5];
  } else {
#pragma unroll
    for (int k = 0; k < 9; k++) C[k] = cov[i * 9 + k];
  }
}

__device__ __forceinline__ void gather_blend(const float4* __restrict__ tab, int t0, int t1, int t2, float w0, float w1, float w2, float* d,
                                             float* Rb, float* Sb) {
  float va[24], vb[24], vc[24];
#pragma unroll
  for (int q = 0; q < 6; q++) {
    const float4 a = tab[6 * (size_t)t0 + q], b = tab[6 * (size_t)t1 + q], c = tab[6 * (size_t)t2 + q];
    va[4 * q] = a.x; va[4 * q + 1] = a.y; va[4 * q + 2] = a.z; va[4 * q + 3] = a.w;
    vb[4 * q] = b.x; vb[4 * q + 1] = b.y; vb[4 * q + 2] = b.z; vb[4 * q + 3] = b.w;
    vc[4 * q] = c.x; vc[4 * q + 1] = c.y; vc[4 * q + 2] = c.z; vc[4 * q + 3] = c.w;
  }
#pragma unroll
  for (int k = 0; k < 3; k++) d[k] = (w0 * va[k] + w1 * vb[k]) + w2 * vc[k];
#pragma unroll
  for (int k = 0; k < 9; k++) {
    Rb[k] = (w0 * va[4 + k] + w1 * vb[4 + k]) + w2 * vc[4 + k];
    Sb[k] = (w0 * va[13 + k] + w1 * vb[13 + k]) + w2 * vc[13 + k];
  }
}

__device__ __forceinline__ void deform_cov(const float* Rb, const float* Sb, const float* C, float* Rt, float* O) {
  float RS[9], A[9];
#pragma unroll
  for (int a = 0; a < 3; a++)
#pragma unroll
    for (int b = 0; b < 3; b++) Rt[3 * a + b] = Rb[3 * b + a];
#pragma unroll
  for (int a = 0; a < 3; a++)
#pragma unroll
    for (int b = 0; b < 3; b++) RS[3 * a + b] = (Rt[3 * a] * Sb[b] + Rt[3 * a + 1] * Sb[3 + b]) + Rt[3 * a + 2] * Sb[6 + b];
#pragma unroll
  for (int a = 0; a < 3; a++)
#pragma unroll
    for (int b = 0; b < 3; b++) A[3 * a + b] = (RS[3 * a] * C[b] + RS[3 * a + 1] * C[3 + b]) + RS[3 * a + 2] * C[6 + b];
#pragma unroll
  for (int a = 0; a < 3; a++)
#pragma unroll
    for (int b = 0; b < 3; b++) O[3 * a + b] = (A[3 * a] * RS[3 * b] + A[3 * a + 1] * RS[3 * b + 1]) + A[3 * a + 2] * RS[3 * b + 2];
}

__device__ __forceinline__ void shade_rotated(int deg, const float* Rt, const float* npos, const float* __restrict__ campos, const float4* row,
                                              float* col) {
  float dx = npos[0] - campos[0], dy = npos[1] - campos[1], dz = npos[2] - campos[2];
  const float len = sqrtf(dx * dx + dy * dy + dz * dz);
  dx = dx / len; dy = dy / len; dz = dz / len;
  const float x = (Rt[0] * dx + Rt[3] * dy) + Rt[6] * dz;
  const float y = (Rt[1] * dx + Rt[4] * dy) + Rt[7] * dz;
  const float z = (Rt[2] * dx + Rt[5] * dy) + Rt[8] * dz;
  float sh[48];
#pragma unroll
  for (int c = 0; c < 12; c++) {
    const float4 v = row[c];
    sh[4 * c] = v.x; sh[4 * c + 1] = v.y; sh[4 * c + 2] = v.z; sh[4 * c + 3] = v.w;
  }
#pragma unroll
  for (int ch = 0; ch < 3; ch++) {
    const float r = sh_channel(deg, [&](int k) { return sh[3 * k + ch]; }, x, y, z);
    col[ch] = fmaxf(r + 0.5f, 0.0f);
  }
}

struct PreSinks { float4* splat; int* radii_int; int* radii_out; uint32_t* tiles; uint4* bin; uint16_t* inst16; uint32_t* counters; uint32_t* slots; uint32_t* coarse; uint32_t* depth_key; };

static PreSinks pre_sinks(const GeomState& g, int* radii) {
  return PreSinks{g.splat, g.radii, radii, g.tiles_touched, g.bin, g.inst16, g.counters, g.slots, g.coarse, g.depth_key};
}

template <bool DIRECT>
__device__ __forceinline__ void pre_write_row(const PreSinks& o, size_t i, int radius_i, uint32_t tiles, const uint4& dbin, uint32_t dkey,
                                              int tile_cull) {
  if (o.radii_out) o.radii_out[i] = radius_i; else o.radii_int[i] = radius_i;
  if (tiles >= GM_BIN_COUNT_SAT) o.tiles[i] = tiles;
  if (!DIRECT) {
    o.bin[i] = dbin;
    o.inst16[i] = (uint16_t)bin_count(dbin);
    o.depth_key[i] = dkey;
  }
  if (i == 0) o.counters[GM_CNT_POLICY] = (uint32_t)tile_cull;
}

static PreCam pre_cam(int W, int H, int tile_cull, const float* view, const float* proj, float tanx, float tany) {
  PreCam c;
  c.W = W; c.H = H; c.gx = (W + GM_TILE - 1) / GM_TILE; c.gy = (H + GM_TILE - 1) / GM_TILE;
  c.tile_cull = tile_cull; c.view = view; c.proj = proj;
  c.tanx = tanx; c.tany = tany;
  c.fy = H / (2.0f * tany); c.fx = W / (2.0f * tanx);
  return c;
}

struct FusedPre {
  PreCam cam;
  const float* opac;
  PreSinks out;
  const uint32_t* dmap; uint32_t* slab_cnt; uint2* slab_pairs; uint4* slab_recs; uint32_t slab_cap;
  int cov6;
};

#ifndef GM_DIRECT_GROUPS
#define GM_DIRECT_GROUPS 6
#endif
struct DirectSlot { uint32_t bucket, base, rank; int leader; };
__device__ __forceinline__ DirectSlot direct_reserve(const FusedPre& fp, uint32_t dkey) {
  const bool vis = dkey != 0xFFFFFFFFu;
  const int lane = threadIdx.x & 63;
  DirectSlot d;
  d.bucket = 0;
  if (vis) {
    const uint32_t e = fp.dmap[(dkey >> GM_COARSE_SHIFT) & (GM_COARSE_BINS - 1)];
    d.bucket = (e >> 16) + (((dkey & ((1u << GM_COARSE_SHIFT) - 1u)) * (e & 0xFFFFu)) >> GM_COARSE_SHIFT);
    d.bucket = min(d.bucket, (1u << GM_BUCKET_BITS) - 1u);
  }
  unsigned long long todo = __ballot(vis);
  uint32_t nsame = 1;
  d.rank = 0; d.leader = lane;
#pragma unroll 1
  for (int it = 0; it < GM_DIRECT_GROUPS && todo; it++) {
    const int l = __ffsll(todo) - 1;
    const uint32_t bl = (uint32_t)__builtin_amdgcn_readlane((int)d.bucket, l);
    const unsigned long long same = __ballot(vis && d.bucket == bl);
    if (vis && d.bucket == bl) { d.rank = lanes_below(same); d.leader = l; nsame = (uint32_t)__popcll(same); }
    todo &= ~same;
  }
  d.base = 0;
  if (vis && d.leader == lane) d.base = atomicAdd(fp.slab_cnt + (size_t)d.bucket * GM_SLAB_CNT_STRIDE, nsame);
  return d;
}
__device__ __forceinline__ void direct_store(const FusedPre& fp, const DirectSlot& d, uint32_t id, uint32_t dkey, const uint4& bin) {
  const uint32_t pos = (uint32_t)__shfl((int)d.base, d.leader) + d.rank;
  if (dkey != 0xFFFFFFFFu && pos < fp.slab_cap) {
    const size_t at = (size_t)d.bucket * fp.slab_cap + pos;
    fp.slab_pairs[at] = make_uint2(dkey, id);
    fp.slab_recs[at] = bin;
  }
}

template <bool PACKED, bool PRE, bool DIRECT = false>
__global__ __launch_bounds__(64) void deform_shade_kernel(int N, int deg, const int* __restrict__ tri, const float* __restrict__ w,
                                                          const float* __restrict__ dV, const float* __restrict__ Rv,
                                                          const float* __restrict__ Sv, const float* __restrict__ cov,
                                                          const float* __restrict__ pos, const float* __restrict__ shs,
                                                          const float* __restrict__ campos, float* __restrict__ pos_out,
                                                          float* __restrict__ cov6_out, float* __restrict__ rgb_out,
                                                          float* __restrict__ cov_out, float* __restrict__ rot_out, const FusedPre fp) {
  extern __shared__ __attribute__((aligned(16))) float lds[];
  float4* l_sh = reinterpret_cast<float4*>(lds);
  const size_t row0 = (size_t)blockIdx.x * DS_THREADS;
  const int nrows = min(DS_THREADS, N - (int)row0);
  const int t = threadIdx.x;
  const size_t i = row0 + t;
  const bool live = t < nrows;
  float O[9], Rt[9], npos[3], col[3];
  int t0 = 0, t1 = 0, t2 = 0; float w0 = 0.f, w1 = 0.f, w2 = 0.f, p0 = 0.f, p1 = 0.f, p2 = 0.f;
  if (live) {
    t0 = tri[3 * i]; t1 = tri[3 * i + 1]; t2 = tri[3 * i + 2];
    w0 = w[3 * i]; w1 = w[3 * i + 1]; w2 = w[3 * i + 2];
    p0 = pos[3 * i]; p1 = pos[3 * i + 1]; p2 = pos[3 * i + 2];
  }
  __builtin_amdgcn_sched_barrier(0);
  stage_sh_rows(l_sh, shs, row0, nrows, t, i);
  float C[9];
  load_rest_cov(C, cov, i, live, PRE && fp.cov6);
  float d[3], Rb[9], Sb[9];
  if (PACKED) {
    gather_blend(reinterpret_cast<const float4*>(dV), t0, t1, t2, w0, w1, w2, d, Rb, Sb);
  } else {
#pragma unroll
    for (int k = 0; k < 3; k++) d[k] = (w0 * dV[3 * (size_t)t0 + k] + w1 * dV[3 * (size_t)t1 + k]) + w2 * dV[3 * (size_t)t2 + k];
#pragma unroll
    for (int k = 0; k < 9; k++) {
      Rb[k] = (w0 * Rv[9 * (size_t)t0 + k] + w1 * Rv[9 * (size_t)t1 + k]) + w2 * Rv[9 * (size_t)t2 + k];
      Sb[k] = (w0 * Sv[9 * (size_t)t0 + k] + w1 * Sv[9 * (size_t)t1 + k]) + w2 * Sv[9 * (size_t)t2 + k];
    }
  }
  __builtin_amdgcn_s_waitcnt(0x0F70);
  __syncthreads();
  deform_cov(Rb, Sb, C, Rt, O);
  npos[0] = p0 + d[0]; npos[1] = p1 + d[1]; npos[2] = p2 + d[2];
  shade_rotated(deg, Rt, npos, campos, l_sh + t * 12, col);
  uint32_t tiles = 0, dkey = 0xFFFFFFFFu;
  uint4 dbin = make_uint4(0u, 0u, 0u, 0u);
  PreGeom pg;
  bool vis = false;
  if (PRE && live) {
    const V3 p = {npos[0], npos[1], npos[2]};
    const float c3[6] = {O[0], O[1], O[2], O[4], O[5], O[8]};
    vis = pre_project(fp.cam, p, c3, pg);
    if (vis) dkey = __float_as_uint(pg.depth);
  }
  DirectSlot slot;
  if (PRE && DIRECT) slot = direct_reserve(fp, dkey);
  if (PRE && live) {
    int radius_i = 0;
    if (vis) {
      const float opac = fp.opac[i];
      splat_store(fp.out.splat, i, pg.pix, pg.piy, pg.conx, pg.cony, pg.conz, opac, col[0], col[1], col[2], pg.depth);
      radius_i = (int)pg.radius;
      pre_emit(fp.cam, pg, opac, tiles, dbin);
    }
    pre_write_row<DIRECT>(fp.out, i, radius_i, tiles, dbin, dkey, fp.cam.tile_cull);
  }
  if (PRE && DIRECT) direct_store(fp, slot, (uint32_t)i, dkey, dbin);
  if (PRE) slot_accumulate(fp.out.slots, fp.out.coarse, tiles, dkey);
  if (!pos_out) return;
  __syncthreads();
  float* o_pos = lds;
  float* o_rgb = lds + DS_THREADS * 3;
  float* o_c6 = lds + DS_THREADS * 6;
  float* o_cov = lds + DS_THREADS * 13;
  float* o_rot = lds + DS_THREADS * 22;
#pragma unroll
  for (int k = 0; k < 3; k++) { o_pos[t * 3 + k] = npos[k]; o_rgb[t * 3 + k] = col[k]; }
  o_c6[t * 7 + 0] = O[0]; o_c6[t * 7 + 1] = O[1]; o_c6[t * 7 + 2] = O[2]; o_c6[t * 7 + 3] = O[4]; o_c6[t * 7 + 4] = O[5]; o_c6[t * 7 + 5] = O[8];
  if (cov_out) {
#pragma unroll
    for (int k = 0; k < 9; k++) { o_cov[t * 9 + k] = O[k]; o_rot[t * 9 + k] = Rt[k]; }
  }
  __syncthreads();
  unstage_rows<3, 3, DS_THREADS>(pos_out, row0, nrows, o_pos);
  unstage_rows<3, 3, DS_THREADS>(rgb_out, row0, nrows, o_rgb);
  unstage_rows<6, 7, DS_THREADS>(cov6_out, row0, nrows, o_c6);
  if (cov_out) {
    unstage_rows<9, 9, DS_THREADS>(cov_out, row0, nrows, o_cov);
    unstage_rows<9, 9, DS_THREADS>(rot_out, row0, nrows, o_rot);
  }
}

struct FusedFrame {
  PreCam cam;
  const float4* tab; const float* campos;
  PreSinks out;
};
struct FusedBatch { int frames, cov6; const float* opac; FusedFrame f[GM_BATCH_MAX]; };

__global__ __launch_bounds__(64) void deform_shade_pre_batch_kernel(int N, int deg, const int* __restrict__ tri, const float* __restrict__ w,
                                                                     const float* __restrict__ cov, const float* __restrict__ pos,
                                                                     const float* __restrict__ shs, const FusedBatch fb) {
  extern __shared__ __attribute__((aligned(16))) float lds[];
  float4* l_sh = reinterpret_cast<float4*>(lds);
  const size_t row0 = (size_t)blockIdx.x * DS_THREADS;
  const int nrows = min(DS_THREADS, N - (int)row0);
  const int t = threadIdx.x;
  const size_t i = row0 + t;
  const bool live = t < nrows;
  int t0 = 0, t1 = 0, t2 = 0; float w0 = 0.f, w1 = 0.f, w2 = 0.f, p0 = 0.f, p1 = 0.f, p2 = 0.f, opac = 0.f;
  if (live) {
    t0 = tri[3 * i]; t1 = tri[3 * i + 1]; t2 = tri[3 * i + 2];
    w0 = w[3 * i]; w1 = w[3 * i + 1]; w2 = w[3 * i + 2];
    p0 = pos[3 * i]; p1 = pos[3 * i + 1]; p2 = pos[3 * i + 2];
    opac = fb.opac[i];
  }
  __builtin_amdgcn_sched_barrier(0);
  stage_sh_rows(l_sh, shs, row0, nrows, t, i);
  float C[9];
  load_rest_cov(C, cov, i, live, fb.cov6);
  __builtin_amdgcn_s_waitcnt(0x0F70);
  __syncthreads();
#pragma unroll 1
  for (int f = 0; f < fb.frames; f++) {
    const FusedFrame& F = fb.f[f];
    float d[3], Rb[9], Sb[9], O[9], Rt[9], npos[3], col[3];
    gather_blend(F.tab, t0, t1, t2, w0, w1, w2, d, Rb, Sb);
    deform_cov(Rb, Sb, C, Rt, O);
    npos[0] = p0 + d[0]; npos[1] = p1 + d[1]; npos[2] = p2 + d[2];
    shade_rotated(deg, Rt, npos, F.campos, l_sh + t * 12, col);
    uint32_t tiles = 0, dkey = 0xFFFFFFFFu;
    uint4 dbin = make_uint4(0u, 0u, 0u, 0u);
    PreGeom pg;
    bool vis = false;
    if (live) {
      const V3 p = {npos[0], npos[1], npos[2]};
      const float c3[6] = {O[0], O[1], O[2], O[4], O[5], O[8]};
      vis = pre_project(F.cam, p, c3, pg);
      if (vis) dkey = __float_as_uint(pg.depth);
      int radius_i = 0;
      if (vis) {
        splat_store(F.out.splat, i, pg.pix, pg.piy, pg.conx, pg.cony, pg.conz, opac, col[0], col[1], col[2], pg.depth);
        radius_i = (int)pg.radius;
        pre_emit(F.cam, pg, opac, tiles, dbin);
      }
      pre_write_row<false>(F.out, i, radius_i, tiles, dbin, dkey, F.cam.tile_cull);
    }
    slot_accumulate(F.out.slots, F.out.coarse, tiles, dkey);
  }
}

static FusedFrame fused_frame(const BatchFrameArgs& a, int W, int H, int tile_cull) {
  return FusedFrame{pre_cam(W, H, tile_cull, a.viewmatrix, a.projmatrix, a.tan_fovx, a.tan_fovy), reinterpret_cast<const float4*>(a.packed),
                    a.cam_pos, pre_sinks(a.g, a.radii)};
}

int launch_deform_shade_pre_batch(int frames, const BatchFrameArgs* fr, int P, int deg, int W, int H, int tile_cull, const int* tri, const float* w,
                                  const float* cov, const float* pos, const float* shs, const float* opacities, bool cov6, int debug, hipStream_t s) {
  if (P <= 0) return 0;
  if (frames < 1 || frames > GM_BATCH_MAX) { set_error("batched fused pass: 1..%d frames", GM_BATCH_MAX); return 1; }
  if (!aligned16(shs) || !aligned16(cov)) { set_error("gm_forward_deformed_batch: shs / cov must be 16-byte aligned"); return 1; }
  StageScope sc(ST_DEFORM, s);
  FusedBatch fb{};
  fb.frames = frames; fb.cov6 = cov6 ? 1 : 0; fb.opac = opacities;
  for (int k = 0; k < frames; k++) {
    if (!aligned16(fr[k].packed)) { set_error("gm_forward_deformed_batch: packed tables must be 16-byte aligned"); return 1; }
    fb.f[k] = fused_frame(fr[k], W, H, tile_cull);
  }
  hipLaunchKernelGGL(deform_shade_pre_batch_kernel, dim3((P + 63) / 64), dim3(64), sizeof(float) * 64 * 48, s, P, deg, tri, w, cov, pos, shs, fb);
  GM_LAUNCH_CHECK(debug, s);
  return 0;
}

__global__ __launch_bounds__(256) void pack_mesh_state_kernel(int Vm, const float* __restrict__ state, const float* __restrict__ verts,
                                                               float4* __restrict__ packed) {
  const int v = blockIdx.x * 256 + threadIdx.x;
  if (v >= Vm) return;
  const float* s = state + 21 * (size_t)v;
  float4* o = packed + 6 * (size_t)v;
  o[0] = make_float4(s[0] - verts[3 * (size_t)v], s[1] - verts[3 * (size_t)v + 1], s[2] - verts[3 * (size_t)v + 2], 0.f);
  o[1] = make_float4(s[3], s[4], s[5], s[6]);
  o[2] = make_float4(s[7], s[8], s[9], s[10]);
  o[3] = make_float4(s[11], s[12], s[13], s[14]);
  o[4] = make_float4(s[15], s[16], s[17], s[18]);
  o[5] = make_float4(s[19], s[20], 0.f, 0.f);
}

int launch_pack_mesh_state(int Vm, const float* state, const float* verts, float* packed, hipStream_t s) {
  if (Vm <= 0) return 0;
  StageScope sc(ST_DEFORM, s);
  hipLaunchKernelGGL(pack_mesh_state_kernel, dim3((Vm + 255) / 256), dim3(256), 0, s, Vm, state, verts, reinterpret_cast<float4*>(packed));
  GM_HIP(hipGetLastError());
  return 0;
}

int launch_deform_shade_packed(int N, int deg, int M, const int* tri, const float* w, const float* packed, const float* cov,
                               const float* pos, const float* shs, const float* campos, float* pos_out, float* cov6_out,
                               float* rgb_out, float* cov_out, float* rot_out, hipStream_t s) {
  if (N <= 0) return 0;
  if (M != 16 || !aligned16(shs) || !aligned16(cov) || !aligned16(pos_out) || !aligned16(cov6_out) || !aligned16(rgb_out) ||
      !aligned16(packed) || (cov_out && (!aligned16(cov_out) || !aligned16(rot_out)))) {
    set_error("gm_deform_shade_packed: needs M == 16 and 16-byte aligned buffers"); return 1;
  }
  StageScope sc(ST_DEFORM, s);
  const size_t lds_bytes = sizeof(float) * 64 * 48;
  hipLaunchKernelGGL((deform_shade_kernel<true, false>), dim3((N + 63) / 64), dim3(64), lds_bytes, s, N, deg, tri, w, packed, nullptr, nullptr,
                     cov, pos, shs, campos, pos_out, cov6_out, rgb_out, cov_out, rot_out, FusedPre{});
  GM_HIP(hipGetLastError());
  return 0;
}

int launch_deform_shade_pre(const RasterArgs& r, GeomState& g, int* radii, int deg, const int* tri, const float* w, const float* packed,
                            const float* cov, const float* pos, const float* shs, float* pos_out, float* cov6_out, float* rgb_out,
                            const DepthSlab* slab, bool cov6) {
  const int N = r.P;
  if (N <= 0) return 0;
  if (!aligned16(shs) || !aligned16(cov) || !aligned16(packed) ||
      (pos_out && (!aligned16(pos_out) || !aligned16(cov6_out) || !aligned16(rgb_out)))) {
    set_error("gm_forward_0_deformed: shs / cov / packed / outputs must be 16-byte aligned"); return 1;
  }
  StageScope sc(ST_DEFORM, r.stream);
  FusedPre fp;
  fp.cam = pre_cam(r.W, r.H, r.tile_cull, r.viewmatrix, r.projmatrix, r.tan_fovx, r.tan_fovy);
  fp.opac = r.opacities;
  fp.out = pre_sinks(g, radii);
  fp.cov6 = cov6 ? 1 : 0;
  fp.dmap = g.dmap; fp.slab_cnt = nullptr; fp.slab_pairs = nullptr; fp.slab_recs = nullptr; fp.slab_cap = 0;
  if (slab) { fp.slab_cnt = slab->cnt; fp.slab_pairs = slab->pairs; fp.slab_recs = slab->recs; fp.slab_cap = slab->cap; }
  const size_t lds_bytes = sizeof(float) * 64 * 48;
  if (slab)
    hipLaunchKernelGGL((deform_shade_kernel<true, true, true>), dim3((N + 63) / 64), dim3(64), lds_bytes, r.stream, N, deg, tri, w, packed, nullptr,
                       nullptr, cov, pos, shs, r.cam_pos, pos_out, cov6_out, rgb_out, nullptr, nullptr, fp);
  else
    hipLaunchKernelGGL((deform_shade_kernel<true, true>), dim3((N + 63) / 64), dim3(64), lds_bytes, r.stream, N, deg, tri, w, packed, nullptr,
                       nullptr, cov, pos, shs, r.cam_pos, pos_out, cov6_out, rgb_out, nullptr, nullptr, fp);
  GM_LAUNCH_CHECK(r.debug, r.stream);
  return 0;
}

int launch_deform_shade(int N, int deg, int M, const int* tri, const float* w, const float* dV, const float* Rv, const float* Sv,
                        const float* cov, const float* pos, const float* shs, const float* campos, float* pos_out,
                        float* cov6_out, float* rgb_out, float* cov_out, float* rot_out, hipStream_t s) {
  if (N <= 0) return 0;
  if (M != 16 || !aligned16(shs) || !aligned16(cov) || !aligned16(pos_out) || !aligned16(cov6_out) || !aligned16(rgb_out) ||
      (cov_out && (!aligned16(cov_out) || !aligned16(rot_out)))) {
    if (!cov_out || !rot_out) { set_error("gm_deform_shade: M != 16 or unaligned buffers need cov_out/rot_out"); return 1; }
    if (int rc = launch_deform(N, tri, w, dV, Rv, Sv, cov, pos, pos_out, cov_out, rot_out, cov6_out, s)) return rc;
    return launch_sh_colors(N, deg, M, pos_out, campos, rot_out, shs, rgb_out, s);
  }
  StageScope sc(ST_DEFORM, s);
  const size_t lds_bytes = sizeof(float) * 64 * 48;
  hipLaunchKernelGGL((deform_shade_kernel<false, false>), dim3((N + 63) / 64), dim3(64), lds_bytes, s, N, deg, tri, w, dV, Rv, Sv, cov, pos,
                     shs, campos, pos_out, cov6_out, rgb_out, cov_out, rot_out, FusedPre{});
  GM_HIP(hipGetLastError());
  return 0;
}

__device__ __forceinline__ void cov_to_scale_rot_row(const float* cov, float4* rots, float* scales, int i) {
#include "gm_cov_to_scale_rot_body.inc"
}

__global__ __launch_bounds__(256) void cov_to_scale_rot_kernel(int N, const float* __restrict__ cov, float* __restrict__ scales,
                                                               float* __restrict__ rots) {
  const int i = blockIdx.x * 256 + threadIdx.x;
  if (i >= N) return;
#include "gm_cov_to_scale_rot_body.inc"
}

int launch_cov_to_scale_rot(int N, const float* cov, float* scales, float* rots, hipStream_t s) {
  if (N > 0) hipLaunchKernelGGL(cov_to_scale_rot_kernel, dim3((N + 255) / 256), dim3(256), 0, s, N, cov, scales, rots);
  GM_HIP(hipGetLastError());
  return 0;
}

struct SceneBatch {
  int frames, n_obj;
  uint32_t moving;
  int rows[GM_SCENE_OBJECTS_MAX + 1];
  uint32_t mask[GM_BATCH_MAX];
  const float* opac;
  FusedFrame f[GM_BATCH_MAX];
};

__global__ __launch_bounds__(64) void scene_shade_pre_batch_kernel(int N, int deg, const float* __restrict__ pos, const float* __restrict__ scales,
                                                                   const float* __restrict__ rots, const float* __restrict__ shs,
                                                                   const int* __restrict__ tri, const float* __restrict__ w,
                                                                   const float* __restrict__ cov, const SceneBatch sb) {
  extern __shared__ __attribute__((aligned(16))) float lds[];
  float4* l_sh = reinterpret_cast<float4*>(lds);
  const size_t row0 = (size_t)blockIdx.x * DS_THREADS;
  const int nrows = min(DS_THREADS, N - (int)row0);
  const int t = threadIdx.x;
  const size_t i = row0 + t;
  const bool live = t < nrows;
  int obj = -1;
  if (live && (int)i >= sb.rows[0] && (int)i < sb.rows[sb.n_obj]) {
    obj = 0;
    for (int j = 1; j < sb.n_obj; j++) obj = (int)i >= sb.rows[j] ? j : obj;
  }
  const bool moving = obj >= 0 && ((sb.moving >> obj) & 1u);
  float p0 = 0.f, p1 = 0.f, p2 = 0.f, s0 = 0.f, s1 = 0.f, s2 = 0.f, opac = 0.f;
  float4 q0 = make_float4(0.f, 0.f, 0.f, 0.f);
  int t0 = 0, t1 = 0, t2 = 0; float w0 = 0.f, w1 = 0.f, w2 = 0.f;
  if (live) {
    p0 = pos[3 * i]; p1 = pos[3 * i + 1]; p2 = pos[3 * i + 2];
    s0 = scales[3 * i]; s1 = scales[3 * i + 1]; s2 = scales[3 * i + 2];
    q0 = reinterpret_cast<const float4*>(rots)[i];
    opac = sb.opac[i];
  }
  const size_t r = moving ? i - (size_t)sb.rows[0] : 0;
  if (moving) {
    t0 = tri[3 * r]; t1 = tri[3 * r + 1]; t2 = tri[3 * r + 2];
    w0 = w[3 * r]; w1 = w[3 * r + 1]; w2 = w[3 * r + 2];
  }
  __builtin_amdgcn_sched_barrier(0);
  stage_sh_rows(l_sh, shs, row0, nrows, t, i);
  float C[9];
  load_rest_cov(C, cov, r, moving, false);
  __builtin_amdgcn_s_waitcnt(0x0F70);
  __syncthreads();
#pragma unroll 1
  for (int f = 0; f < sb.frames; f++) {
    const FusedFrame& F = sb.f[f];
    V3 p = {p0, p1, p2};
    float4 q = q0;
    float sc[3] = {s0, s1, s2};
    if (moving && ((sb.mask[f] >> obj) & 1u)) {
      float d[3], Rb[9], Sb[9], Rt[9], O[9];
      gather_blend(F.tab, t0, t1, t2, w0, w1, w2, d, Rb, Sb);
      deform_cov(Rb, Sb, C, Rt, O);
      p = V3{p0 + d[0], p1 + d[1], p2 + d[2]};
      if (!(xform4x3(p, F.cam.view).z <= 0.2f)) cov_to_scale_rot_row(O, &q, sc, 0);
    }
    uint32_t tiles = 0, dkey = 0xFFFFFFFFu;
    uint4 dbin = make_uint4(0u, 0u, 0u, 0u);
    if (live) {
      float c3[6];
      cov3d_from_scale_rot(q, sc, c3);
      PreGeom pg;
      const bool vis = pre_project(F.cam, p, c3, pg);
      int radius_i = 0;
      if (vis) {
        float col[3];
        sh_color(deg, p, F.campos, l_sh + t * 12, col);
        dkey = __float_as_uint(pg.depth);
        splat_store(F.out.splat, i, pg.pix, pg.piy, pg.conx, pg.cony, pg.conz, opac, col[0], col[1], col[2], pg.depth);
        radius_i = (int)pg.radius;
        pre_emit(F.cam, pg, opac, tiles, dbin);
      }
      pre_write_row<false>(F.out, i, radius_i, tiles, dbin, dkey, F.cam.tile_cull);
    }
    slot_accumulate(F.out.slots, F.out.coarse, tiles, dkey);
  }
}

int launch_scene_shade_pre_batch(int frames, const BatchFrameArgs* fr, const uint32_t* deformed, int n_obj, const int* object_rows, int P, int deg,
                                 int W, int H, int tile_cull, const float* pos, const float* scales, const float* rots, const float* shs,
                                 const float* opacities, const int* tri, const float* w, const float* cov, int debug, hipStream_t s) {
  if (P <= 0) return 0;
  if (frames < 1 || frames > GM_BATCH_MAX || n_obj < 0 || n_obj > GM_SCENE_OBJECTS_MAX) {
    set_error("scene fused pass: 1..%d frames, 0..%d objects", GM_BATCH_MAX, GM_SCENE_OBJECTS_MAX); return 1;
  }
  if (!aligned16(shs) || !aligned16(rots)) { set_error("gm_forward_scene_batch: shs / rots must be 16-byte aligned"); return 1; }
  StageScope sc(ST_DEFORM, s);
  SceneBatch sb{};
  sb.frames = frames; sb.n_obj = n_obj; sb.opac = opacities;
  for (int j = 0; j <= n_obj; j++) sb.rows[j] = object_rows[j];
  for (int k = 0; k < frames; k++) {
    sb.mask[k] = deformed[k];
    sb.moving |= deformed[k];
    if (deformed[k] && !aligned16(fr[k].packed)) { set_error("gm_forward_scene_batch: packed tables must be 16-byte aligned"); return 1; }
    sb.f[k] = fused_frame(fr[k], W, H, tile_cull);
  }
  hipLaunchKernelGGL(scene_shade_pre_batch_kernel, dim3((P + 63) / 64), dim3(64), sizeof(float) * 64 * 48, s, P, deg, pos, scales, rots, shs, tri, w,
                     cov, sb);
  GM_LAUNCH_CHECK(debug, s);
  return 0;
}

}
```

### gaussianmesh_amd/csrc/gm_pre_body.h

```cpp
#pragma once
#include "gm_common.h"
#include "gm_cull.h"
#include "gm_sh.h"

namespace gm {

struct V3 { float x, y, z; };

__device__ __forceinline__ V3 xform4x3(const V3 p, const float* __restrict__ m) {
#pragma clang fp contract(off)
  V3 o;
  o.x = m[0] * p.x + m[4] * p.y + m[8] * p.z + m[12];
  o.y = m[1] * p.x + m[5] * p.y + m[9] * p.z + m[13];
  o.z = m[2] * p.x + m[6] * p.y + m[10] * p.z + m[14];
  return o;
}

__device__ __forceinline__ float ndc2pix(float v, int S) {
#pragma clang fp contract(off)
  return (float)(((v + 1.0) * S - 1.0) * 0.5);
}

__device__ __forceinline__ void get_rect(float px, float py, int r, int gx, int gy, int& x0, int& y0, int& x1, int& y1) {
#pragma clang fp contract(off)
  x0 = min(gx, max(0, (int)((px - r) / GM_TILE)));
  y0 = min(gy, max(0, (int)((py - r) / GM_TILE)));
  x1 = min(gx, max(0, (int)((px + r + GM_TILE - 1) / GM_TILE)));
  y1 = min(gy, max(0, (int)((py + r + GM_TILE - 1) / GM_TILE)));
}

__device__ __forceinline__ void quat_cols(float r, float x, float y, float z, float* Rg) {
#pragma clang fp contract(off)
  Rg[0] = 1.f - 2.f * (y * y + z * z); Rg[1] = 2.f * (x * y - r * z); Rg[2] = 2.f * (x * z + r * y);
  Rg[3] = 2.f * (x * y + r * z); Rg[4] = 1.f - 2.f * (x * x + z * z); Rg[5] = 2.f * (y * z - r * x);
  Rg[6] = 2.f * (x * z - r * y); Rg[7] = 2.f * (y * z + r * x); Rg[8] = 1.f - 2.f * (x * x + y * y);
}

__device__ __forceinline__ void cov2d_T(V3 mean, float fx, float fy, float tanx, float tany, const float* __restrict__ v,
                                        V3& t, float* T0, float* T1, float& xmul, float& ymul) {
#pragma clang fp contract(off)
  t = xform4x3(mean, v);
  const float limx = 1.3f * tanx, limy = 1.3f * tany;
  const float txtz = t.x / t.z, tytz = t.y / t.z;
  t.x = fminf(limx, fmaxf(-limx, txtz)) * t.z;
  t.y = fminf(limy, fmaxf(-limy, tytz)) * t.z;
  xmul = (txtz < -limx || txtz > limx) ? 0.f : 1.f;
  ymul = (tytz < -limy || tytz > limy) ? 0.f : 1.f;
  const float j00 = fx / t.z, j02 = -(fx * t.x) / (t.z * t.z);
  const float j11 = fy / t.z, j12 = -(fy * t.y) / (t.z * t.z);
#pragma unroll
  for (int i = 0; i < 3; i++) {
    T0[i] = (v[4 * i] * j00 + v[4 * i + 1] * 0.0f) + v[4 * i + 2] * j02;
    T1[i] = (v[4 * i] * 0.0f + v[4 * i + 1] * j11) + v[4 * i + 2] * j12;
  }
}

__device__ __forceinline__ void cov2d_from_T(const float* T0, const float* T1, const float* c, float& a, float& b, float& cc) {
#pragma clang fp contract(off)
  const float V[9] = {c[0], c[1], c[2], c[1], c[3], c[4], c[2], c[4], c[5]};
  float A0[3], A1[3];
#pragma unroll
  for (int k = 0; k < 3; k++) {
    A0[k] = (T0[0] * V[0 + k] + T0[1] * V[3 + k]) + T0[2] * V[6 + k];
    A1[k] = (T1[0] * V[0 + k] + T1[1] * V[3 + k]) + T1[2] * V[6 + k];
  }
  a = (A0[0] * T0[0] + A0[1] * T0[1]) + A0[2] * T0[2];
  b = (A1[0] * T0[0] + A1[1] * T0[1]) + A1[2] * T0[2];
  cc = (A1[0] * T1[0] + A1[1] * T1[1]) + A1[2] * T1[2];
}

__device__ __forceinline__ void cov3d_from_scale_rot(const float4 q, const float* scale, float* c3) {
#pragma clang fp contract(off)
#define GM_COV3D_SCALE(k) scale[k]
#include "gm_cov3d_body.inc"
#undef GM_COV3D_SCALE
}

__device__ __forceinline__ uint8_t sh_color(int D, const V3 p, const float* campos, const float4* row, float* col) {
#pragma clang fp contract(off)
  uint8_t clampbits = 0;
#define GM_SH_DEG D
#define GM_SH_CAMPOS campos
#define GM_SH_LOAD(sh)                                                                                                                  \
  _Pragma("unroll")                                                                                                                     \
  for (int c = 0; c < 12; c++) { const float4 v = row[c]; sh[4 * c] = v.x; sh[4 * c + 1] = v.y; sh[4 * c + 2] = v.z; sh[4 * c + 3] = v.w; }
#include "gm_sh_color_body.inc"
#undef GM_SH_LOAD
#undef GM_SH_CAMPOS
#undef GM_SH_DEG
  return clampbits;
}


struct PreCam {
  int W, H, gx, gy, tile_cull;
  const float *view, *proj;
  float tanx, tany, fx, fy;
};

struct PreGeom {
  float pix, piy, conx, cony, conz, depth, radius;
  int x0, y0, x1, y1;
};

__device__ __forceinline__ bool pre_project(const PreCam& a, const V3 p, const float* c3, PreGeom& o) {
#pragma clang fp contract(off)
  const float* pm = a.proj;
  const float hx = pm[0] * p.x + pm[4] * p.y + pm[8] * p.z + pm[12];
  const float hy = pm[1] * p.x + pm[5] * p.y + pm[9] * p.z + pm[13];
  const float hw = pm[3] * p.x + pm[7] * p.y + pm[11] * p.z + pm[15];
  const float p_w = 1.0f / (hw + 0.0000001f);
  const float prx = hx * p_w, pry = hy * p_w;
  const V3 pv = xform4x3(p, a.view);
  if (pv.z <= 0.2f) return false;
  V3 t; float T0[3], T1[3], xm, ym, ca, cb, cc;
  cov2d_T(p, a.fx, a.fy, a.tanx, a.tany, a.view, t, T0, T1, xm, ym);
  cov2d_from_T(T0, T1, c3, ca, cb, cc);
  ca += 0.3f; cc += 0.3f;
  const float det = ca * cc - cb * cb;
  if (det == 0.0f) return false;
  const float det_inv = 1.f / det;
  o.conx = cc * det_inv; o.cony = -cb * det_inv; o.conz = ca * det_inv;
  const float mid = 0.5f * (ca + cc);
  const float lambda1 = mid + sqrtf(fmaxf(0.1f, mid * mid - det));
  const float lambda2 = mid - sqrtf(fmaxf(0.1f, mid * mid - det));
  o.radius = ceilf(3.f * sqrtf(fmaxf(lambda1, lambda2)));
  o.pix = ndc2pix(prx, a.W); o.piy = ndc2pix(pry, a.H);
  get_rect(o.pix, o.piy, (int)o.radius, a.gx, a.gy, o.x0, o.y0, o.x1, o.y1);
  if ((o.x1 - o.x0) * (o.y1 - o.y0) == 0) return false;
  o.depth = pv.z;
  return true;
}

__device__ __forceinline__ void pre_emit(const PreCam& a, const PreGeom& g, float opac, uint32_t& tiles, uint4& bin) {
#pragma clang fp contract(off)
  const int x0 = g.x0, y0 = g.y0, x1 = g.x1, y1 = g.y1;
  const int rw = x1 - x0, rh = y1 - y0, ncand = rw * rh;
  unsigned long long mask = 0ull;
  if (!a.tile_cull) {
    tiles = (uint32_t)ncand;
    mask = ncand >= 64 ? ~0ull : ((1ull << ncand) - 1ull);
  } else {
    const TileCull tc = tile_cull_setup(g.pix, g.piy, g.conx, g.cony, g.conz, opac, (float)(x0 * GM_TILE), (float)(x1 * GM_TILE - 1),
                                        (float)(y0 * GM_TILE), (float)(y1 * GM_TILE - 1));
    const int s = a.tile_cull >= 2 ? a.tile_cull - 1 : 0;
    const bool small = ncand <= 64 && rw <= 60;
    uint32_t cnt = 0;
    if (s == 1) {
      const bool quad = quad_rect((uint32_t)x0, (uint32_t)y0, (uint32_t)rw, (uint32_t)rh);
      const bool all_quad = __all(quad);
      const int px0 = x0 >> 1, py0 = y0 >> 1;
      int bqx0 = 0, bqx1 = 7, bqy0 = 0, bqy1 = 7;
      if (quad && tc.mode == 1) {
        const float ex = tc.xext + 2e-3f, ey = tc.dymax + 2e-3f;
        bqx0 = (int)fmaxf(ceilf((g.pix - ex - 7.f) * 0.125f), -1e9f) - 4 * px0; bqx1 = (int)fminf(floorf((g.pix + ex) * 0.125f), 1e9f) - 4 * px0;
        bqy0 = (int)fmaxf(ceilf((g.piy - ey - 7.f) * 0.125f), -1e9f) - 4 * py0; bqy1 = (int)fminf(floorf((g.piy + ey) * 0.125f), 1e9f) - 4 * py0;
      }
      uint32_t qw[2] = {0u, 0u};
      const int pr_last = tc.mode != 0 ? (y1 - 1) >> 1 : (y0 >> 1) - 1;
      for (int pr = y0 >> 1; pr <= pr_last; pr++) {
        const int ty = 2 * pr;
        int ta[2], tb[2];
        row_tiles_pair(tc, g.pix, g.piy, ty, x0, x1, ta, tb);
        if (ty < y0) { ta[0] = GM_ROW_EMPTY_LO; tb[0] = -1; }
        if (ty + 1 >= y1) { ta[1] = GM_ROW_EMPTY_LO; tb[1] = -1; }
        if (!all_quad) {
          const int la = ta[0] >> 1, ha = tb[0] >> 1, lb = ta[1] >> 1, hb = tb[1] >> 1;
          const int uni = max(ha - la + 1, 0) + max(hb - lb + 1, 0) - max(min(ha, hb) - max(la, lb) + 1, 0);
          const int hull = max((max(tb[0], tb[1]) >> 1) - (min(ta[0], ta[1]) >> 1) + 1, 0);
          cnt += (uint32_t)(small ? uni : hull);
#pragma unroll
          for (int r = 0; r < 2; r++) {
            const int len = max(tb[r] - ta[r] + 1, 0);
            const unsigned long long run = len >= 64 ? ~0ull : ((1ull << len) - 1ull);
            mask |= run << (((ty + r - y0) * rw + (ta[r] - x0)) & 63);
          }
        }
        if (quad) {
          uint32_t word = 0;
#pragma unroll
          for (int r = 0; r < 2; r++) {
            const int qa = max(2 * ta[r] - 4 * px0, bqx0), qb = min(2 * tb[r] + 1 - 4 * px0, bqx1);
            const uint32_t r8 = qa <= qb ? ((1u << (qb - qa + 1)) - 1u) << qa : 0u;
            const uint32_t two = (r8 & 0xFu) | ((r8 >> 4) << 16);
#pragma unroll
            for (int h = 0; h < 2; h++) {
              const int ql = 2 * r + h, qrow = 4 * (pr - py0) + ql;
              if (qrow >= bqy0 && qrow <= bqy1) word |= two << (4 * ql);
            }
          }
          if (pr == py0) qw[0] = word; else qw[1] = word;
        }
      }
      if (ncand > 64) mask = 0ull;
      if (quad) {
        mask = (unsigned long long)qw[0] | ((unsigned long long)qw[1] << 32);
        cnt = ((qw[0] & 0xFFFFu) ? 1u : 0u) + ((qw[0] >> 16) ? 1u : 0u) + ((qw[1] & 0xFFFFu) ? 1u : 0u) + ((qw[1] >> 16) ? 1u : 0u);
      }
    } else {
    int cur_pr = -1, hull_lo = 0x7fffffff, hull_hi = -1;
    unsigned long long prow = 0ull;
    for (int ry = 0; ry < rh; ry++) {
      const int pr = (y0 + ry) >> s;
      if (s > 0 && pr != cur_pr) {
        cnt += small ? parents_in_row(prow, x0, s) : (hull_hi >= 0 ? (uint32_t)((hull_hi >> s) - (hull_lo >> s) + 1) : 0u);
        cur_pr = pr; prow = 0ull; hull_lo = 0x7fffffff; hull_hi = -1;
      }
      int ta, tb;
      if (!row_tiles(tc, g.pix, g.piy, y0 + ry, x0, x1, ta, tb)) continue;
      const int len = tb - ta + 1, bit0 = ry * rw + (ta - x0);
      const unsigned long long run = len >= 64 ? ~0ull : ((1ull << len) - 1ull);
      if (ncand <= 64) mask |= run << bit0;
      if (s == 0) cnt += (uint32_t)len;
      else if (small) prow |= run << (ta - x0);
      else { hull_lo = min(hull_lo, ta); hull_hi = max(hull_hi, tb); }
    }
    if (s > 0) cnt += small ? parents_in_row(prow, x0, s) : (hull_hi >= 0 ? (uint32_t)((hull_hi >> s) - (hull_lo >> s) + 1) : 0u);
    }
    tiles = cnt;
  }
  bin = bin_pack((uint32_t)x0, (uint32_t)y0, (uint32_t)rw, (uint32_t)rh, tiles, mask);
}

__device__ __forceinline__ void slot_accumulate(uint32_t* __restrict__ slots, uint32_t* __restrict__ coarse, uint32_t tiles, uint32_t dkey) {
  const bool vis = dkey != 0xFFFFFFFFu;
  const int lane = threadIdx.x & 63;
  uint32_t s = tiles;
#pragma unroll
  for (int d = 32; d >= 1; d >>= 1) s += (uint32_t)__shfl_xor((int)s, d);
  const unsigned long long visb = __ballot(vis);
  const uint32_t c = (dkey >> GM_COARSE_SHIFT) & (GM_COARSE_BINS - 1);
  uint32_t ncmin = vis ? (GM_COARSE_BINS - 1u) - c : 0u, cmax = vis ? c : 0u;
#pragma unroll
  for (int d = 32; d >= 1; d >>= 1) {
    ncmin = max(ncmin, (uint32_t)__shfl_xor((int)ncmin, d));
    cmax = max(cmax, (uint32_t)__shfl_xor((int)cmax, d));
  }
  if (lane == 0 && visb) {
    uint32_t* slot = slots + GM_SLOT_STRIDE * ((blockIdx.x * (blockDim.x >> 6) + (threadIdx.x >> 6)) & (GM_SLOTS - 1));
    if (s) atomicAdd(slot, s);
    atomicAdd(slot + 1, (uint32_t)__popcll(visb));
    atomicMax(slot + 2, ncmin);
    atomicMax(slot + 3, cmax);
  }
  const uint32_t copy = blockIdx.x & (GM_COARSE_COPIES - 1);
  unsigned long long todo = visb;
  while (todo) {
    const int l = __ffsll(todo) - 1;
    const uint32_t cl = (uint32_t)__builtin_amdgcn_readlane((int)c, l);
    const unsigned long long same = __ballot(vis && c == cl);
    if (lane == l) atomicAdd(coarse + coarse_index(cl, copy), (uint32_t)__popcll(same));
    todo &= ~same;
  }
}

}
```

### gaussianmesh_amd/csrc/gm_sh.h

```cpp
#pragma once
#include <hip/hip_runtime.h>
#include <stdint.h>

namespace gm {

__device__ static const float SH_C0 = 0.28209479177387814f;
__device__ static const float SH_C1 = 0.4886025119029199f;
__device__ static const float SH_C2[5] = {1.0925484305920792f, -1.0925484305920792f, 0.31539156525252005f,
                                           -1.0925484305920792f, 0.5462742152960396f};
__device__ static const float SH_C3[7] = {-0.5900435899266435f, 2.890611442640554f, -0.4570457994644658f,
                                           0.3731763325901154f, -0.4570457994644658f, 1.445305721320277f,
                                           -0.5900435899266435f};

template <typename F>
__device__ __forceinline__ float sh_channel(int deg, F S, float x, float y, float z) {
  float r = SH_C0 * S(0);
  if (deg > 0) {
    r = r - SH_C1 * y * S(1) + SH_C1 * z * S(2) - SH_C1 * x * S(3);
    if (deg > 1) {
      const float xx = x * x, yy = y * y, zz = z * z, xy = x * y, yz = y * z, xz = x * z;
      r = r + SH_C2[0] * xy * S(4) + SH_C2[1] * yz * S(5) + SH_C2[2] * (2.0f * zz - xx - yy) * S(6) +
          SH_C2[3] * xz * S(7) + SH_C2[4] * (xx - yy) * S(8);
      if (deg > 2) {
        r = r + SH_C3[0] * y * (3.0f * xx - yy) * S(9) + SH_C3[1] * xy * z * S(10) +
            SH_C3[2] * y * (4.0f * zz - xx - yy) * S(11) + SH_C3[3] * z * (2.0f * zz - 3.0f * xx - 3.0f * yy) * S(12) +
            SH_C3[4] * x * (4.0f * zz - xx - yy) * S(13) + SH_C3[5] * z * (xx - yy) * S(14) +
            SH_C3[6] * x * (xx - 3.0f * yy) * S(15);
      }
    }
  }
  return r;
}

__device__ __forceinline__ void load_sh(const float* __restrict__ shs, size_t idx, int M, int ncoef, float* sh) {
  const float* base = shs + idx * (size_t)M * 3;
  const int nf = ncoef * 3;
  if ((((size_t)M * 3) & 3) == 0 && (reinterpret_cast<uintptr_t>(shs) & 15) == 0) {
    const float4* b4 = reinterpret_cast<const float4*>(base);
#pragma unroll
    for (int k = 0; k < 12; k++) {
      if (4 * k < nf) {
        const float4 q = b4[k];
        sh[4 * k] = q.x; sh[4 * k + 1] = q.y; sh[4 * k + 2] = q.z; sh[4 * k + 3] = q.w;
      }
    }
  } else {
#pragma unroll
    for (int k = 0; k < 48; k++)
      if (k < nf) sh[k] = base[k];
  }
}

}
```

### include/gmesh_hip.h

```cpp
#ifndef GMESH_HIP_H_INCLUDED
#define GMESH_HIP_H_INCLUDED

#include <stddef.h>
#include <stdint.h>

#ifdef __cplusplus
extern "C" {
#endif

#define GM_OK 0
#define GM_ERR_INVALID_ARG 1
#define GM_ERR_HIP 2
#define GM_ERR_BUFFER 3

#define GM_ABI_VERSION 3
int gm_abi_version(void);
const char* gm_last_error(void);

#define GM_POLICY_REFERENCE 0
#define GM_POLICY_DEFAULT 2

size_t gm_geom_bytes(int P);
size_t gm_image_bytes(int W, int H);
size_t gm_work_hint_bytes(int W, int H);
size_t gm_binning_bytes(int64_t num_rendered);

int gm_forward_0(void* geom_buffer, int P, int D, int M, const float* background, int width, int height,
                 const float* means3D, const float* shs, const float* colors_precomp, const float* opacities,
                 const float* scales, float scale_modifier, const float* rotations, const float* cov3D_precomp,
                 const float* viewmatrix, const float* projmatrix, const float* cam_pos, float tan_fovx,
                 float tan_fovy, int prefiltered, int* radii, int debug, void* stream, int* num_rendered);

int gm_forward_0_async(int emission_policy, void* geom_buffer, int P, int D, int M, const float* background, int width, int height,
                       const float* means3D, const float* shs, const float* colors_precomp, const float* opacities,
                       const float* scales, float scale_modifier, const float* rotations, const float* cov3D_precomp,
                       const float* viewmatrix, const float* projmatrix, const float* cam_pos, float tan_fovx,
                       float tan_fovy, int prefiltered, int* radii, int debug, void* stream, int* num_rendered_host,
                       void* count_event);

int gm_forward_1(void* geom_buffer, void* binning_buffer, void* image_buffer, int P, int D, int M, int num_rendered,
                 const float* background, int width, int height, const float* means3D, const float* shs,
                 const float* colors_precomp, const float* opacities, const float* scales, float scale_modifier,
                 const float* rotations, const float* cov3D_precomp, const float* viewmatrix, const float* projmatrix,
                 const float* cam_pos, float tan_fovx, float tan_fovy, int prefiltered, float* out_color, int* radii,
                 int debug, void* stream);

int gm_backward(int P, int D, int M, int R, const float* background, int width, int height, const float* means3D,
                const float* shs, const float* colors_precomp, const float* scales, float scale_modifier,
                const float* rotations, const float* cov3D_precomp, const float* viewmatrix, const float* projmatrix,
                const float* campos, float tan_fovx, float tan_fovy, const int* radii, void* geom_buffer,
                void* binning_buffer, void* image_buffer, const float* dL_dpix, float* dL_dmean2D, float* dL_dconic,
                float* dL_dopacity, float* dL_dcolor, float* dL_dmean3D, float* dL_dcov3D, float* dL_dsh,
                float* dL_dscale, float* dL_drot, int debug, void* stream);

int gm_backward_p(int emission_policy, int P, int D, int M, int R, const float* background, int width, int height, const float* means3D,
                  const float* shs, const float* colors_precomp, const float* scales, float scale_modifier,
                  const float* rotations, const float* cov3D_precomp, const float* viewmatrix, const float* projmatrix,
                  const float* campos, float tan_fovx, float tan_fovy, const int* radii, void* geom_buffer,
                  void* binning_buffer, void* image_buffer, const float* dL_dpix, float* dL_dmean2D, float* dL_dconic,
                  float* dL_dopacity, float* dL_dcolor, float* dL_dmean3D, float* dL_dcov3D, float* dL_dsh,
                  float* dL_dscale, float* dL_drot, int debug, void* stream);

int gm_backward_aux(int emission_policy, int P, int D, int M, int R, const float* background, int width, int height, const float* means3D,
                    const float* shs, const float* colors_precomp, const float* scales, float scale_modifier,
                    const float* rotations, const float* cov3D_precomp, const float* viewmatrix, const float* projmatrix,
                    const float* campos, float tan_fovx, float tan_fovy, const int* radii, void* geom_buffer,
                    void* binning_buffer, void* image_buffer, const float* dL_dpix, float* dL_dmean2D, float* dL_dconic,
                    float* dL_dopacity, float* dL_dcolor, float* dL_dmean3D, float* dL_dcov3D, float* dL_dsh,
                    float* dL_dscale, float* dL_drot, const float* dL_ddepth, const float* dL_dalpha, float* dL_dz, int debug, void* stream);

int gm_backward_sh_step(int emission_policy, int P, int D, int M, int R, const float* background, int width, int height, const float* means3D,
                        float* shs, const float* scales, float scale_modifier, const float* rotations, const float* cov3D_precomp,
                        const float* viewmatrix, const float* projmatrix, const float* campos, float tan_fovx, float tan_fovy, const int* radii,
                        void* geom_buffer, void* binning_buffer, void* image_buffer, const float* dL_dpix, float* dL_dmean2D, float* dL_dopacity,
                        float* dL_dmean3D, float* dL_dcov3D, float* dL_dscale, float* dL_drot, int rows, float* exp_avg, float* exp_avg_sq,
                        float lr_dc, float lr_rest, double beta1, double beta2, double eps, int step, int debug, void* stream);

int gm_mark_visible(int P, const float* means3D, const float* viewmatrix, const float* projmatrix, uint8_t* present,
                    void* stream);

int gm_splat_floats(void);
void* gm_geom_field(void* geom_buffer, int P, const char* name);
void* gm_image_field(void* image_buffer, int W, int H, const char* name);
void* gm_binning_field(void* binning_buffer, int64_t R, int W, int H, int emission_policy, const char* name);

size_t gm_knn_workspace_bytes(int P);
int gm_knn(int P, const float* points, float* meanDists, void* workspace, size_t workspace_bytes, void* stream);

size_t gm_knn_nearest_workspace_bytes(int Pq, int Pr);
int gm_knn_nearest(int Pq, const float* query, int Pr, const float* ref, float* out_d2, int* out_idx, void* workspace, size_t workspace_bytes,
                   void* stream);

size_t gm_closest_face_workspace_bytes(int N, int F);
int gm_closest_face(int N, const float* points, int Vm, const float* vertices, int F, const int* faces, float* out_d2, int* out_face,
                    float* out_closest, void* workspace, size_t workspace_bytes, void* stream);

size_t gm_arap_workspace_bytes(int Vm);
int gm_arap_solve(int Vm, const int* row_offsets, const int* cols, const double* weights, const float* V0, const unsigned char* fixed,
                  const float* V_init, int outer_iterations, int cg_iterations, double cg_tolerance, float* V_out, double* stats,
                  void* workspace, size_t workspace_bytes, void* stream);

size_t gm_arap_grid_workspace_bytes(int Vm);
int gm_arap_solve_grid(int Vm, const int* row_offsets, const int* cols, const double* weights, const float* V0, const unsigned char* fixed,
                       const float* V_init, int outer_iterations, int cg_iterations, double cg_tolerance, float* V_out, double* stats,
                       void* workspace, size_t workspace_bytes, void* stream);

#define GM_ARAP_BATCH_MAX 64
size_t gm_arap_batch_workspace_bytes(int Vm, int B, int global_step );
int gm_arap_solve_batch(int B, int global_step, int Vm, const int* row_offsets, const int* cols, const double* weights, const float* V0,
                        const unsigned char* fixed, const float* V_init, int outer_iterations, int cg_iterations, double cg_tolerance,
                        float* V_out, double* stats, void* workspace, size_t workspace_bytes, void* stream);

size_t gm_ray_mesh_workspace_bytes(int R, int F);
int gm_ray_mesh(int R, const float* origins, const float* dirs, int Vm, const float* vertices, int F, const int* faces, float t_min, float t_max,
                float* out_t, int* out_face, float* out_uv, void* workspace, size_t workspace_bytes, void* stream);

size_t gm_mesh_geodesic_workspace_bytes(int Vm, int B, int sweeps);
int gm_mesh_geodesic(int Vm, const int* row_offsets, const int* cols, const float* lengths, int B, const int* source_offsets, const int* sources,
                     float max_distance, int sweeps, int resume, float* dist, int* unsettled, void* workspace, size_t workspace_bytes, void* stream);

int gm_tsdf_integrate(int K, int H, int W, const float* depth, const float* alpha, const float* views, const float* tanfov, int nx, int ny, int nz,
                      const float* origin, float voxel, float trunc, float alpha_min, int carve, float* tsdf, float* weight, void* stream);

size_t gm_surface_nets_workspace_bytes(int nx, int ny, int nz);
int gm_surface_nets(int nx, int ny, int nz, const float* origin, float voxel, const float* tsdf, const float* weight, float min_weight,
                    int max_vertices, float* out_vertices, int max_faces, int* out_faces, int* out_counts, void* workspace, size_t workspace_bytes,
                    void* stream);

int gm_deform(int N, const int* tri, const float* w, const float* dV, const float* Rv, const float* Sv,
              const float* cov, const float* pos, float* pos_out, float* cov_out, float* rot_out, float* cov6_out,
              void* stream);

int gm_sh_colors(int N, int deg, int M, const float* pos, const float* campos, const float* rot, const float* shs,
                 float* rgb, void* stream);

int gm_deform_shade(int N, int deg, int M, const int* tri, const float* w, const float* dV, const float* Rv, const float* Sv,
                    const float* cov, const float* pos, const float* shs, const float* campos, float* pos_out, float* cov6_out,
                    float* rgb_out, float* cov_out, float* rot_out, void* stream);

int gm_pack_mesh_state(int Vm, const float* state, const float* verts, float* packed, void* stream);
int gm_deform_shade_packed(int N, int deg, int M, const int* tri, const float* w, const float* packed, const float* cov,
                           const float* pos, const float* shs, const float* campos, float* pos_out, float* cov6_out,
                           float* rgb_out, float* cov_out, float* rot_out, void* stream);

int gm_forward_0_deformed_async(int emission_policy, void* geom_buffer, int P, int deg, int M, int width, int height, const int* tri,
                                const float* w, const float* packed, const float* cov, const float* pos, const float* shs,
                                const float* opacities, const float* viewmatrix, const float* projmatrix, const float* cam_pos,
                                float tan_fovx, float tan_fovy, float* pos_out, float* cov6_out, float* rgb_out, int* radii, int debug,
                                void* stream, int* num_rendered_host, void* count_event);

size_t gm_depth_plan_bytes(void);
size_t gm_depth_slab_bytes(int P);
int gm_forward_0_deformed_stream_async(int emission_policy, void* geom_buffer, int P, int deg, int M, int width, int height, const int* tri,
                                       const float* w, const float* packed, const float* cov, const float* pos, const float* shs,
                                       const float* opacities, const float* viewmatrix, const float* projmatrix, const float* cam_pos,
                                       float tan_fovx, float tan_fovy, float* pos_out, float* cov6_out, float* rgb_out, int* radii,
                                       int debug, void* stream, int* num_rendered_host, void* count_event, void* depth_slab,
                                       unsigned int* depth_plan, int flags);
#define GM_STREAM_DIRECT 1
#define GM_STREAM_COV6 2

#define GM_FWD_IMAGE_ONLY 1
#define GM_FWD_EXACT_EXPONENT 2
int gm_forward_1_geom(int emission_policy, void* geom_buffer, void* binning_buffer, void* image_buffer, int P, int num_rendered,
                      int64_t binning_capacity, const float* background, int width, int height, float* out_color, int debug, void* stream,
                      int* status_host, int flags, unsigned int* work_hint);
int gm_forward_status_async(void* geom_buffer, int P, int* status_host, void* stream);

int gm_forward_1_aux(int emission_policy, void* geom_buffer, void* binning_buffer, void* image_buffer, int P, int num_rendered,
                     int64_t binning_capacity, const float* background, int width, int height, float* out_color, int debug, void* stream,
                     int* status_host, int flags, unsigned int* work_hint, float* out_depth, float* out_alpha);

#define GM_BATCH_MAX 8
#define GM_BATCH_IMAGE_ONLY 1
#define GM_BATCH_COV6 2
typedef struct gm_batch_frame {
  const float* packed;
  const float* viewmatrix; const float* projmatrix; const float* cam_pos;
  float tan_fovx, tan_fovy;
  void* geom_buffer; void* binning_buffer; void* image_buffer;
  float* out_color;
  int* radii;
  int* status_host;
} gm_batch_frame;
int gm_forward_deformed_batch_async(int emission_policy, int K, const gm_batch_frame* frames, int P, int deg, int M, int width, int height,
                                    const int* tri, const float* w, const float* cov, const float* pos, const float* shs, const float* opacities,
                                    const float* background, int64_t binning_capacity, int flags, unsigned int* work_hint, int debug, void* stream);
int gm_forward_deformed_batch_aux_async(int emission_policy, int K, const gm_batch_frame* frames, int P, int deg, int M, int width, int height,
                                        const int* tri, const float* w, const float* cov, const float* pos, const float* shs, const float* opacities,
                                        const float* background, int64_t binning_capacity, int flags, unsigned int* work_hint, int debug, void* stream,
                                        float* const* out_depth, float* const* out_alpha);
#define GM_SCENE_OBJECTS_MAX 32
int gm_forward_scene_batch_async(int emission_policy, int K, const gm_batch_frame* frames, int P, int deg, int M, int width, int height,
                                 int n_objects, const int* object_rows, const unsigned int* deformed, const float* pos, const float* scales,
                                 const float* rots, const float* shs, const float* opacities, const int* tri, const float* w, const float* cov,
                                 const float* background, int64_t binning_capacity, int flags, unsigned int* work_hint, int debug, void* stream);
int gm_mesh_rs_packed_batch(int K, int Vm, int nfaces, const float* V0, const float* const* V1, const int* faces, const int* adj_offsets,
                            const int* adj_faces, float* const* packed, void* stream);

int gm_mesh_rs(int Vm, int nfaces, const float* V0, const float* V1, const int* faces, const int* adj_offsets, const int* adj_faces,
               float* R, float* S, float* state, void* stream);
int gm_mesh_rs_packed(int Vm, int nfaces, const float* V0, const float* V1, const int* faces, const int* adj_offsets, const int* adj_faces,
                      float* packed, void* stream);

int gm_cov_to_scale_rot(int N, const float* cov, float* scales, float* rots, void* stream);

int gm_sh_rotate(int N, int deg, int M, const float* shs, const float* rot, float* shs_out, void* stream);

int64_t gm_ssim_partials(int planes, int H, int W);
int gm_ssim_fwd(const float* img1, const float* img2, int planes, int H, int W, float* dS_dmu1, float* dS_dE11, float* dS_dE12,
                float* partial, void* stream);
int gm_ssim_bwd(const float* img1, const float* img2, const float* dS_dmu1, const float* dS_dE11, const float* dS_dE12, int planes,
                int H, int W, const float* g_ssim, const float* g_l1, float* dL_dimg1, void* stream);
int gm_loss_combine(const float* partial, int64_t n_partials, double c_ssim, double c_l1, double offset, float* out, void* stream);

int gm_ssim_fwd_u8(const float* img1, const uint8_t* rgb, const uint8_t* mask, int64_t mask_plane_stride, const float* background,
                   int planes, int H, int W, float* dS_dmu1, float* dS_dE11, float* dS_dE12, float* partial, void* stream);
int gm_ssim_bwd_u8(const float* img1, const uint8_t* rgb, const uint8_t* mask, int64_t mask_plane_stride, const float* background,
                   const float* dS_dmu1, const float* dS_dE11, const float* dS_dE12, int planes, int H, int W, const float* g_ssim,
                   const float* g_l1, float* dL_dimg1, void* stream);

int gm_mesh_activate_fwd(int N, float alpha, const float* bc, const float* dist, const float* scaling, const float* rotation,
                         const float* opacity, const float* v1, const float* v2, const float* v3, const float* normal, const float* r,
                         float* xyz, float* scales, float* rots, float* opac, float mr_weight, float* mr_partial, void* stream);
int gm_mesh_activate_bwd(int N, float alpha, const float* bc, const float* dist, const float* scaling, const float* rotation,
                         const float* opacity, const float* v1, const float* v2, const float* v3, const float* normal, const float* r,
                         const float* d_xyz, const float* d_scales, const float* d_rots, const float* d_opac, float* d_bc, float* d_dist,
                         float* d_scaling, float* d_rotation, float* d_opacity, float mr_weight, const float* d_mr, void* stream);

int gm_plain_activate_fwd(int N, const float* xyz, const float* scaling, const float* rotation, const float* opacity, float* out_xyz,
                          float* out_scales, float* out_rots, float* out_opac, int row0, int capacity, void* stream);
int gm_plain_activate_bwd(int N, const float* scaling, const float* rotation, const float* opacity, const float* g_xyz, const float* g_scales,
                          const float* g_rots, const float* g_opac, int row0, int capacity, float* d_xyz, float* d_scaling, float* d_rotation,
                          float* d_opacity, void* stream);

int gm_adam_step(int count, float* const* params, const float* const* grads, float* const* exp_avg, float* const* exp_avg_sq,
                 const uint64_t* sizes, const float* lr, const float* lr_rest, const uint32_t* period, const uint32_t* split,
                 double beta1, double beta2, double eps, int step, void* stream);
int gm_adam_step_active(int count, float* const* params, const float* const* grads, float* const* exp_avg, float* const* exp_avg_sq,
                        const uint64_t* sizes, const float* lr, const float* lr_rest, const uint32_t* period, const uint32_t* split,
                        const uint32_t* active, double beta1, double beta2, double eps, int step, void* stream);

int gm_densify_stats(int N, const int* radii, const float* viewspace_grad, float* max_radii2D, float* grad_accum, float* denom, void* stream);

void gm_profile_enable(int on);
void gm_profile_reset(void);
int gm_profile_read(const char* stage, double* total_ms, int64_t* launches);

void gm_debug_render_trace(void* buffer);
void gm_debug_bucket_trace(void* buffer);

#ifdef __cplusplus
}
#endif
#endif
```

Baseline: 4967 frames/s.

## Trim SH LDS staging, stream SH evaluation, use buffer loads and lane-broadcast cameras

Shrinks the per-block shared-memory SH stage from 12 to 10 float4 granules per row, using an XOR swizzle, and loads the last two granules from global memory into registers only when degree 3 is used. SH evaluation now streams granules instead of materialising a 48-float array, and the mesh gather uses raw buffer loads with 32-bit offsets. Per-frame camera matrices are loaded one value per lane and broadcast with readlane, with the next frame prefetched. The kernels are pinned to 4 waves per EU. Together these aim to cut LDS and register pressure in the fused deform+shade+preprocess kernel. The 32-bit offsets need a new vertex-count limit check, and an occupancy query API is added.

```diff
diff --git a/gaussianmesh_amd/_lib.py b/gaussianmesh_amd/_lib.py
--- a/gaussianmesh_amd/_lib.py
+++ b/gaussianmesh_amd/_lib.py
@@ -84,6 +84,7 @@
                                                   i32, vp, C.POINTER(vp), C.POINTER(vp)]),
     "gm_forward_scene_batch_async": (i32, [i32, i32, C.POINTER(BatchFrame), i32, i32, i32, i32, i32, i32, C.POINTER(i32), C.POINTER(C.c_uint),
                                            vp, vp, vp, vp, vp, vp, vp, vp, vp, i64, i32, vp, i32, vp]),
+    "gm_fused_batch_occupancy": (i32, [C.POINTER(i32)]),
     "gm_mesh_rs_packed_batch": (i32, [i32, i32, i32, vp, C.POINTER(vp), vp, vp, vp, C.POINTER(vp), vp]),
     "gm_deform_shade_packed": (i32, [i32, i32, i32, vp, vp, vp, vp, vp, vp, vp, vp, vp, vp, vp, vp, vp]),
     "gm_cov_to_scale_rot": (i32, [i32, vp, vp, vp, vp]),
diff --git a/gaussianmesh_amd/csrc/gm_api.hip b/gaussianmesh_amd/csrc/gm_api.hip
--- a/gaussianmesh_amd/csrc/gm_api.hip
+++ b/gaussianmesh_amd/csrc/gm_api.hip
@@ -493,9 +493,15 @@
   if (K < 1 || K > GM_BATCH_MAX || Vm < 0 || nfaces < 0 || !V1 || !packed || (Vm > 0 && (!V0 || !adj_offsets || (nfaces > 0 && (!faces || !adj_faces))))) {
     set_error("gm_mesh_rs_packed_batch: bad args"); return GM_ERR_INVALID_ARG;
   }
+  if (Vm > GM_PACKED_VERTICES_MAX) { set_error("gm_mesh_rs_packed_batch: a gather table holds at most %d vertices (4 GiB)", GM_PACKED_VERTICES_MAX); return GM_ERR_INVALID_ARG; }
   for (int k = 0; k < K; k++)
     if (Vm > 0 && (!V1[k] || !packed[k] || (reinterpret_cast<uintptr_t>(packed[k]) & 15))) { set_error("gm_mesh_rs_packed_batch: frame %d: null or unaligned pointer", k); return GM_ERR_INVALID_ARG; }
   return launch_mesh_rs_batch(K, Vm, V0, V1, faces, adj_offsets, adj_faces, packed, reinterpret_cast<hipStream_t>(stream));
+}
+
+int gm_fused_batch_occupancy(int* waves_per_cu) {
+  if (!waves_per_cu) { set_error("gm_fused_batch_occupancy: waves_per_cu is null"); return GM_ERR_INVALID_ARG; }
+  return fused_batch_occupancy(waves_per_cu);
 }
 
 int gm_forward_status_async(void* geom_buffer, int P, int* status_host, void* stream) {
@@ -866,6 +872,7 @@
 int gm_pack_mesh_state(int Vm, const float* state, const float* verts, float* packed, void* stream) {
   if (Vm < 0 || (Vm > 0 && (!state || !verts || !packed))) { set_error("gm_pack_mesh_state: bad args"); return GM_ERR_INVALID_ARG; }
   if (Vm > 0 && (reinterpret_cast<uintptr_t>(packed) & 15)) { set_error("gm_pack_mesh_state: packed must be 16-byte aligned"); return GM_ERR_INVALID_ARG; }
+  if (Vm > GM_PACKED_VERTICES_MAX) { set_error("gm_pack_mesh_state: a gather table holds at most %d vertices (4 GiB)", GM_PACKED_VERTICES_MAX); return GM_ERR_INVALID_ARG; }
   return launch_pack_mesh_state(Vm, state, verts, packed, reinterpret_cast<hipStream_t>(stream));
 }
 
@@ -896,6 +903,7 @@
     set_error("gm_mesh_rs_packed: bad args"); return GM_ERR_INVALID_ARG;
   }
   if (reinterpret_cast<uintptr_t>(packed) & 15) { set_error("gm_mesh_rs_packed: packed must be 16-byte aligned"); return GM_ERR_INVALID_ARG; }
+  if (Vm > GM_PACKED_VERTICES_MAX) { set_error("gm_mesh_rs_packed: a gather table holds at most %d vertices (4 GiB)", GM_PACKED_VERTICES_MAX); return GM_ERR_INVALID_ARG; }
   return launch_mesh_rs(Vm, V0, V1, faces, adj_offsets, adj_faces, nullptr, nullptr, nullptr, packed, reinterpret_cast<hipStream_t>(stream));
 }
 
diff --git a/gaussianmesh_amd/csrc/gm_common.h b/gaussianmesh_amd/csrc/gm_common.h
--- a/gaussianmesh_amd/csrc/gm_common.h
+++ b/gaussianmesh_amd/csrc/gm_common.h
@@ -362,6 +362,8 @@
 };
 int launch_deform_shade_pre_batch(int frames, const BatchFrameArgs* fr, int P, int deg, int W, int H, int tile_cull, const int* tri, const float* w,
                                   const float* cov, const float* pos, const float* shs, const float* opacities, bool cov6, int debug, hipStream_t s);
+int fused_batch_occupancy(int* waves_per_cu);
+constexpr int GM_PACKED_VERTICES_MAX = 44739242;
 int launch_scene_shade_pre_batch(int frames, const BatchFrameArgs* fr, const uint32_t* deformed, int n_obj, const int* object_rows, int P, int deg,
                                  int W, int H, int tile_cull, const float* pos, const float* scales, const float* rots, const float* shs,
                                  const float* opacities, const int* tri, const float* w, const float* cov, int debug, hipStream_t s);
diff --git a/gaussianmesh_amd/csrc/gm_deform.hip b/gaussianmesh_amd/csrc/gm_deform.hip
--- a/gaussianmesh_amd/csrc/gm_deform.hip
+++ b/gaussianmesh_amd/csrc/gm_deform.hip
@@ -99,15 +99,34 @@
 
 constexpr int DS_THREADS = 64;
 
-__device__ __forceinline__ void stage_sh_rows(float4* l_sh, const float* __restrict__ shs, size_t row0, int nrows, int t, size_t i) {
+constexpr int SH_LDS_GRANULES = 10;
+constexpr size_t SH_LDS_BYTES = sizeof(float4) * DS_THREADS * SH_LDS_GRANULES;
+
+struct ShRow {
+  const float4 *even, *odd;
+  float4 g10, g11;
+  __device__ __forceinline__ float4 operator()(int c) const { return c == 10 ? g10 : c == 11 ? g11 : (c & 1) ? odd[c] : even[c]; }
+};
+
+__device__ __forceinline__ ShRow stage_sh_rows(float4* l_sh, const float* __restrict__ shs, size_t row0, int nrows, int t, size_t i, int deg) {
+  const float4* g4 = reinterpret_cast<const float4*>(shs);
   if (nrows == DS_THREADS) {
-    const char* gsh = reinterpret_cast<const char*>(shs + row0 * 48) + t * 16;
-#pragma unroll
-    for (int q = 0; q < 12; q++) dma16(gsh + q * 1024, reinterpret_cast<char*>(l_sh) + q * 1024);
+    const char* gsh = reinterpret_cast<const char*>(shs + row0 * 48);
+#pragma unroll
+    for (int q = 0; q < SH_LDS_GRANULES; q++) {
+      const int n = q * 64 + t, r = n / SH_LDS_GRANULES, c = (n - r * SH_LDS_GRANULES) ^ ((r >> 3) & 1);
+      dma16(gsh + r * 192 + c * 16, reinterpret_cast<char*>(l_sh) + q * 1024);
+    }
   } else if (t < nrows) {
 #pragma unroll
-    for (int c = 0; c < 12; c++) l_sh[t * 12 + c] = reinterpret_cast<const float4*>(shs)[i * 12 + c];
-  }
+    for (int c = 0; c < SH_LDS_GRANULES; c++) l_sh[t * SH_LDS_GRANULES + (c ^ ((t >> 3) & 1))] = g4[i * 12 + c];
+  }
+  const int swap = (t >> 3) & 1;
+  ShRow row;
+  row.even = l_sh + t * SH_LDS_GRANULES + swap; row.odd = l_sh + t * SH_LDS_GRANULES - swap;
+  row.g10 = row.g11 = make_float4(0.f, 0.f, 0.f, 0.f);
+  if (deg > 2 && t < nrows) { row.g10 = g4[i * 12 + 10]; row.g11 = g4[i * 12 + 11]; }
+  return row;
 }
 
 __device__ __forceinline__ void load_rest_cov(float* C, const float* __restrict__ cov, size_t i, bool live, bool cov6) {
@@ -129,21 +148,24 @@
 
 __device__ __forceinline__ void gather_blend(const float4* __restrict__ tab, int t0, int t1, int t2, float w0, float w1, float w2, float* d,
                                              float* Rb, float* Sb) {
-  float va[24], vb[24], vc[24];
+  typedef uint32_t u32x4 __attribute__((ext_vector_type(4)));
+  const __amdgpu_buffer_rsrc_t rs = __builtin_amdgcn_make_buffer_rsrc(const_cast<float4*>(tab), 0, 0xFFFFFFFF, 0x00020000);
+  const uint32_t o0 = (uint32_t)t0 * 96u, o1 = (uint32_t)t1 * 96u, o2 = (uint32_t)t2 * 96u;
+  float o[24];
 #pragma unroll
   for (int q = 0; q < 6; q++) {
-    const float4 a = tab[6 * (size_t)t0 + q], b = tab[6 * (size_t)t1 + q], c = tab[6 * (size_t)t2 + q];
-    va[4 * q] = a.x; va[4 * q + 1] = a.y; va[4 * q + 2] = a.z; va[4 * q + 3] = a.w;
-    vb[4 * q] = b.x; vb[4 * q + 1] = b.y; vb[4 * q + 2] = b.z; vb[4 * q + 3] = b.w;
-    vc[4 * q] = c.x; vc[4 * q + 1] = c.y; vc[4 * q + 2] = c.z; vc[4 * q + 3] = c.w;
-  }
-#pragma unroll
-  for (int k = 0; k < 3; k++) d[k] = (w0 * va[k] + w1 * vb[k]) + w2 * vc[k];
-#pragma unroll
-  for (int k = 0; k < 9; k++) {
-    Rb[k] = (w0 * va[4 + k] + w1 * vb[4 + k]) + w2 * vc[4 + k];
-    Sb[k] = (w0 * va[13 + k] + w1 * vb[13 + k]) + w2 * vc[13 + k];
-  }
+    const u32x4 ua = __builtin_amdgcn_raw_buffer_load_b128(rs, o0 + 16 * q, 0, 0), ub = __builtin_amdgcn_raw_buffer_load_b128(rs, o1 + 16 * q, 0, 0),
+                uc = __builtin_amdgcn_raw_buffer_load_b128(rs, o2 + 16 * q, 0, 0);
+    const float4 a = make_float4(__uint_as_float(ua.x), __uint_as_float(ua.y), __uint_as_float(ua.z), __uint_as_float(ua.w));
+    const float4 b = make_float4(__uint_as_float(ub.x), __uint_as_float(ub.y), __uint_as_float(ub.z), __uint_as_float(ub.w));
+    const float4 c = make_float4(__uint_as_float(uc.x), __uint_as_float(uc.y), __uint_as_float(uc.z), __uint_as_float(uc.w));
+    o[4 * q] = (w0 * a.x + w1 * b.x) + w2 * c.x; o[4 * q + 1] = (w0 * a.y + w1 * b.y) + w2 * c.y;
+    o[4 * q + 2] = (w0 * a.z + w1 * b.z) + w2 * c.z; o[4 * q + 3] = (w0 * a.w + w1 * b.w) + w2 * c.w;
+  }
+#pragma unroll
+  for (int k = 0; k < 3; k++) d[k] = o[k];
+#pragma unroll
+  for (int k = 0; k < 9; k++) { Rb[k] = o[4 + k]; Sb[k] = o[13 + k]; }
 }
 
 __device__ __forceinline__ void deform_cov(const float* Rb, const float* Sb, const float* C, float* Rt, float* O) {
@@ -166,7 +188,14 @@
     for (int b = 0; b < 3; b++) O[3 * a + b] = (A[3 * a] * RS[3 * b] + A[3 * a + 1] * RS[3 * b + 1]) + A[3 * a + 2] * RS[3 * b + 2];
 }
 
-__device__ __forceinline__ void shade_rotated(int deg, const float* Rt, const float* npos, const float* __restrict__ campos, const float4* row,
+__device__ __forceinline__ void shade_dir(int deg, float x, float y, float z, const ShRow& row, float* col) {
+  float r[3];
+  sh_rgb_streamed(deg, row, x, y, z, r);
+#pragma unroll
+  for (int ch = 0; ch < 3; ch++) col[ch] = fmaxf(r[ch] + 0.5f, 0.0f);
+}
+
+__device__ __forceinline__ void shade_rotated(int deg, const float* Rt, const float* npos, const float* __restrict__ campos, const ShRow& row,
                                               float* col) {
   float dx = npos[0] - campos[0], dy = npos[1] - campos[1], dz = npos[2] - campos[2];
   const float len = sqrtf(dx * dx + dy * dy + dz * dz);
@@ -174,17 +203,14 @@
   const float x = (Rt[0] * dx + Rt[3] * dy) + Rt[6] * dz;
   const float y = (Rt[1] * dx + Rt[4] * dy) + Rt[7] * dz;
   const float z = (Rt[2] * dx + Rt[5] * dy) + Rt[8] * dz;
-  float sh[48];
-#pragma unroll
-  for (int c = 0; c < 12; c++) {
-    const float4 v = row[c];
-    sh[4 * c] = v.x; sh[4 * c + 1] = v.y; sh[4 * c + 2] = v.z; sh[4 * c + 3] = v.w;
-  }
-#pragma unroll
-  for (int ch = 0; ch < 3; ch++) {
-    const float r = sh_channel(deg, [&](int k) { return sh[3 * k + ch]; }, x, y, z);
-    col[ch] = fmaxf(r + 0.5f, 0.0f);
-  }
+  shade_dir(deg, x, y, z, row, col);
+}
+
+__device__ __forceinline__ void shade_unrotated(int deg, const V3 p, const float* __restrict__ campos, const ShRow& row, float* col) {
+  float dx = p.x - campos[0], dy = p.y - campos[1], dz = p.z - campos[2];
+  const float len = sqrtf(dx * dx + dy * dy + dz * dz);
+  dx = dx / len; dy = dy / len; dz = dz / len;
+  shade_dir(deg, dx, dy, dz, row, col);
 }
 
 struct PreSinks { float4* splat; int* radii_int; int* radii_out; uint32_t* tiles; uint4* bin; uint16_t* inst16; uint32_t* counters; uint32_t* slots; uint32_t* coarse; uint32_t* depth_key; };
@@ -284,7 +310,7 @@
     p0 = pos[3 * i]; p1 = pos[3 * i + 1]; p2 = pos[3 * i + 2];
   }
   __builtin_amdgcn_sched_barrier(0);
-  stage_sh_rows(l_sh, shs, row0, nrows, t, i);
+  const ShRow row = stage_sh_rows(l_sh, shs, row0, nrows, t, i, deg);
   float C[9];
   load_rest_cov(C, cov, i, live, PRE && fp.cov6);
   float d[3], Rb[9], Sb[9];
@@ -303,7 +329,7 @@
   __syncthreads();
   deform_cov(Rb, Sb, C, Rt, O);
   npos[0] = p0 + d[0]; npos[1] = p1 + d[1]; npos[2] = p2 + d[2];
-  shade_rotated(deg, Rt, npos, campos, l_sh + t * 12, col);
+  shade_rotated(deg, Rt, npos, campos, row, col);
   uint32_t tiles = 0, dkey = 0xFFFFFFFFu;
   uint4 dbin = make_uint4(0u, 0u, 0u, 0u);
   PreGeom pg;
@@ -359,7 +385,20 @@
 };
 struct FusedBatch { int frames, cov6; const float* opac; FusedFrame f[GM_BATCH_MAX]; };
 
-__global__ __launch_bounds__(64) void deform_shade_pre_batch_kernel(int N, int deg, const int* __restrict__ tri, const float* __restrict__ w,
+struct CamConsts { float view[16], proj[16], campos[3]; };
+__device__ __forceinline__ float cam_lane_load(const FusedFrame& F, int lane) {
+  const float* p = lane < 16 ? F.cam.view + lane : lane < 32 ? F.cam.proj + (lane - 16) : F.campos + (lane - 32);
+  return lane < 35 ? *p : 0.f;
+}
+__device__ __forceinline__ void cam_broadcast(float word, CamConsts& c) {
+  const int v = __float_as_int(word);
+#pragma unroll
+  for (int k = 0; k < 16; k++) { c.view[k] = __int_as_float(__builtin_amdgcn_readlane(v, k)); c.proj[k] = __int_as_float(__builtin_amdgcn_readlane(v, 16 + k)); }
+#pragma unroll
+  for (int k = 0; k < 3; k++) c.campos[k] = __int_as_float(__builtin_amdgcn_readlane(v, 32 + k));
+}
+
+__global__ __launch_bounds__(64) __attribute__((amdgpu_waves_per_eu(4, 4))) void deform_shade_pre_batch_kernel(int N, int deg, const int* __restrict__ tri, const float* __restrict__ w,
                                                                      const float* __restrict__ cov, const float* __restrict__ pos,
                                                                      const float* __restrict__ shs, const FusedBatch fb) {
   extern __shared__ __attribute__((aligned(16))) float lds[];
@@ -377,19 +416,25 @@
     opac = fb.opac[i];
   }
   __builtin_amdgcn_sched_barrier(0);
-  stage_sh_rows(l_sh, shs, row0, nrows, t, i);
+  const ShRow row = stage_sh_rows(l_sh, shs, row0, nrows, t, i, deg);
   float C[9];
   load_rest_cov(C, cov, i, live, fb.cov6);
   __builtin_amdgcn_s_waitcnt(0x0F70);
   __syncthreads();
+  float cam_word = cam_lane_load(fb.f[0], t);
 #pragma unroll 1
   for (int f = 0; f < fb.frames; f++) {
     const FusedFrame& F = fb.f[f];
+    CamConsts cc;
+    cam_broadcast(cam_word, cc);
+    if (f + 1 < fb.frames) cam_word = cam_lane_load(fb.f[f + 1], t);
+    PreCam cam = F.cam;
+    cam.view = cc.view; cam.proj = cc.proj;
     float d[3], Rb[9], Sb[9], O[9], Rt[9], npos[3], col[3];
     gather_blend(F.tab, t0, t1, t2, w0, w1, w2, d, Rb, Sb);
     deform_cov(Rb, Sb, C, Rt, O);
     npos[0] = p0 + d[0]; npos[1] = p1 + d[1]; npos[2] = p2 + d[2];
-    shade_rotated(deg, Rt, npos, F.campos, l_sh + t * 12, col);
+    shade_rotated(deg, Rt, npos, cc.campos, row, col);
     uint32_t tiles = 0, dkey = 0xFFFFFFFFu;
     uint4 dbin = make_uint4(0u, 0u, 0u, 0u);
     PreGeom pg;
@@ -397,13 +442,13 @@
     if (live) {
       const V3 p = {npos[0], npos[1], npos[2]};
       const float c3[6] = {O[0], O[1], O[2], O[4], O[5], O[8]};
-      vis = pre_project(F.cam, p, c3, pg);
+      vis = pre_project(cam, p, c3, pg);
       if (vis) dkey = __float_as_uint(pg.depth);
       int radius_i = 0;
       if (vis) {
         splat_store(F.out.splat, i, pg.pix, pg.piy, pg.conx, pg.cony, pg.conz, opac, col[0], col[1], col[2], pg.depth);
         radius_i = (int)pg.radius;
-        pre_emit(F.cam, pg, opac, tiles, dbin);
+        pre_emit(cam, pg, opac, tiles, dbin);
       }
       pre_write_row<false>(F.out, i, radius_i, tiles, dbin, dkey, F.cam.tile_cull);
     }
@@ -428,8 +473,15 @@
     if (!aligned16(fr[k].packed)) { set_error("gm_forward_deformed_batch: packed tables must be 16-byte aligned"); return 1; }
     fb.f[k] = fused_frame(fr[k], W, H, tile_cull);
   }
-  hipLaunchKernelGGL(deform_shade_pre_batch_kernel, dim3((P + 63) / 64), dim3(64), sizeof(float) * 64 * 48, s, P, deg, tri, w, cov, pos, shs, fb);
+  hipLaunchKernelGGL(deform_shade_pre_batch_kernel, dim3((P + 63) / 64), dim3(64), SH_LDS_BYTES, s, P, deg, tri, w, cov, pos, shs, fb);
   GM_LAUNCH_CHECK(debug, s);
+  return 0;
+}
+
+int fused_batch_occupancy(int* waves_per_cu) {
+  int blocks = 0;
+  GM_HIP(hipOccupancyMaxActiveBlocksPerMultiprocessor(&blocks, deform_shade_pre_batch_kernel, DS_THREADS, SH_LDS_BYTES));
+  *waves_per_cu = blocks * (DS_THREADS / 64);
   return 0;
 }
 
@@ -464,7 +516,7 @@
     set_error("gm_deform_shade_packed: needs M == 16 and 16-byte aligned buffers"); return 1;
   }
   StageScope sc(ST_DEFORM, s);
-  const size_t lds_bytes = sizeof(float) * 64 * 48;
+  const size_t lds_bytes = SH_LDS_BYTES;
   hipLaunchKernelGGL((deform_shade_kernel<true, false>), dim3((N + 63) / 64), dim3(64), lds_bytes, s, N, deg, tri, w, packed, nullptr, nullptr,
                      cov, pos, shs, campos, pos_out, cov6_out, rgb_out, cov_out, rot_out, FusedPre{});
   GM_HIP(hipGetLastError());
@@ -488,7 +540,7 @@
   fp.cov6 = cov6 ? 1 : 0;
   fp.dmap = g.dmap; fp.slab_cnt = nullptr; fp.slab_pairs = nullptr; fp.slab_recs = nullptr; fp.slab_cap = 0;
   if (slab) { fp.slab_cnt = slab->cnt; fp.slab_pairs = slab->pairs; fp.slab_recs = slab->recs; fp.slab_cap = slab->cap; }
-  const size_t lds_bytes = sizeof(float) * 64 * 48;
+  const size_t lds_bytes = SH_LDS_BYTES;
   if (slab)
     hipLaunchKernelGGL((deform_shade_kernel<true, true, true>), dim3((N + 63) / 64), dim3(64), lds_bytes, r.stream, N, deg, tri, w, packed, nullptr,
                        nullptr, cov, pos, shs, r.cam_pos, pos_out, cov6_out, rgb_out, nullptr, nullptr, fp);
@@ -510,7 +562,7 @@
     return launch_sh_colors(N, deg, M, pos_out, campos, rot_out, shs, rgb_out, s);
   }
   StageScope sc(ST_DEFORM, s);
-  const size_t lds_bytes = sizeof(float) * 64 * 48;
+  const size_t lds_bytes = SH_LDS_BYTES;
   hipLaunchKernelGGL((deform_shade_kernel<false, false>), dim3((N + 63) / 64), dim3(64), lds_bytes, s, N, deg, tri, w, dV, Rv, Sv, cov, pos,
                      shs, campos, pos_out, cov6_out, rgb_out, cov_out, rot_out, FusedPre{});
   GM_HIP(hipGetLastError());
@@ -543,7 +595,7 @@
   FusedFrame f[GM_BATCH_MAX];
 };
 
-__global__ __launch_bounds__(64) void scene_shade_pre_batch_kernel(int N, int deg, const float* __restrict__ pos, const float* __restrict__ scales,
+__global__ __launch_bounds__(64) __attribute__((amdgpu_waves_per_eu(4, 4))) void scene_shade_pre_batch_kernel(int N, int deg, const float* __restrict__ pos, const float* __restrict__ scales,
                                                                    const float* __restrict__ rots, const float* __restrict__ shs,
                                                                    const int* __restrict__ tri, const float* __restrict__ w,
                                                                    const float* __restrict__ cov, const SceneBatch sb) {
@@ -575,14 +627,20 @@
     w0 = w[3 * r]; w1 = w[3 * r + 1]; w2 = w[3 * r + 2];
   }
   __builtin_amdgcn_sched_barrier(0);
-  stage_sh_rows(l_sh, shs, row0, nrows, t, i);
+  const ShRow row = stage_sh_rows(l_sh, shs, row0, nrows, t, i, deg);
   float C[9];
   load_rest_cov(C, cov, r, moving, false);
   __builtin_amdgcn_s_waitcnt(0x0F70);
   __syncthreads();
+  float cam_word = cam_lane_load(sb.f[0], t);
 #pragma unroll 1
   for (int f = 0; f < sb.frames; f++) {
     const FusedFrame& F = sb.f[f];
+    CamConsts cc;
+    cam_broadcast(cam_word, cc);
+    if (f + 1 < sb.frames) cam_word = cam_lane_load(sb.f[f + 1], t);
+    PreCam cam = F.cam;
+    cam.view = cc.view; cam.proj = cc.proj;
     V3 p = {p0, p1, p2};
     float4 q = q0;
     float sc[3] = {s0, s1, s2};
@@ -591,7 +649,7 @@
       gather_blend(F.tab, t0, t1, t2, w0, w1, w2, d, Rb, Sb);
       deform_cov(Rb, Sb, C, Rt, O);
       p = V3{p0 + d[0], p1 + d[1], p2 + d[2]};
-      if (!(xform4x3(p, F.cam.view).z <= 0.2f)) cov_to_scale_rot_row(O, &q, sc, 0);
+      if (!(xform4x3(p, cam.view).z <= 0.2f)) cov_to_scale_rot_row(O, &q, sc, 0);
     }
     uint32_t tiles = 0, dkey = 0xFFFFFFFFu;
     uint4 dbin = make_uint4(0u, 0u, 0u, 0u);
@@ -599,15 +657,15 @@
       float c3[6];
       cov3d_from_scale_rot(q, sc, c3);
       PreGeom pg;
-      const bool vis = pre_project(F.cam, p, c3, pg);
+      const bool vis = pre_project(cam, p, c3, pg);
       int radius_i = 0;
       if (vis) {
         float col[3];
-        sh_color(deg, p, F.campos, l_sh + t * 12, col);
+        shade_unrotated(deg, p, cc.campos, row, col);
         dkey = __float_as_uint(pg.depth);
         splat_store(F.out.splat, i, pg.pix, pg.piy, pg.conx, pg.cony, pg.conz, opac, col[0], col[1], col[2], pg.depth);
         radius_i = (int)pg.radius;
-        pre_emit(F.cam, pg, opac, tiles, dbin);
+        pre_emit(cam, pg, opac, tiles, dbin);
       }
       pre_write_row<false>(F.out, i, radius_i, tiles, dbin, dkey, F.cam.tile_cull);
     }
@@ -633,7 +691,7 @@
     if (deformed[k] && !aligned16(fr[k].packed)) { set_error("gm_forward_scene_batch: packed tables must be 16-byte aligned"); return 1; }
     sb.f[k] = fused_frame(fr[k], W, H, tile_cull);
   }
-  hipLaunchKernelGGL(scene_shade_pre_batch_kernel, dim3((P + 63) / 64), dim3(64), sizeof(float) * 64 * 48, s, P, deg, pos, scales, rots, shs, tri, w,
+  hipLaunchKernelGGL(scene_shade_pre_batch_kernel, dim3((P + 63) / 64), dim3(64), SH_LDS_BYTES, s, P, deg, pos, scales, rots, shs, tri, w,
                      cov, sb);
   GM_LAUNCH_CHECK(debug, s);
   return 0;
diff --git a/gaussianmesh_amd/csrc/gm_pre_body.h b/gaussianmesh_amd/csrc/gm_pre_body.h
--- a/gaussianmesh_amd/csrc/gm_pre_body.h
+++ b/gaussianmesh_amd/csrc/gm_pre_body.h
@@ -75,22 +75,6 @@
 #include "gm_cov3d_body.inc"
 #undef GM_COV3D_SCALE
 }
-
-__device__ __forceinline__ uint8_t sh_color(int D, const V3 p, const float* campos, const float4* row, float* col) {
-#pragma clang fp contract(off)
-  uint8_t clampbits = 0;
-#define GM_SH_DEG D
-#define GM_SH_CAMPOS campos
-#define GM_SH_LOAD(sh)                                                                                                                  \
-  _Pragma("unroll")                                                                                                                     \
-  for (int c = 0; c < 12; c++) { const float4 v = row[c]; sh[4 * c] = v.x; sh[4 * c + 1] = v.y; sh[4 * c + 2] = v.z; sh[4 * c + 3] = v.w; }
-#include "gm_sh_color_body.inc"
-#undef GM_SH_LOAD
-#undef GM_SH_CAMPOS
-#undef GM_SH_DEG
-  return clampbits;
-}
-
 
 struct PreCam {
   int W, H, gx, gy, tile_cull;
diff --git a/gaussianmesh_amd/csrc/gm_sh.h b/gaussianmesh_amd/csrc/gm_sh.h
--- a/gaussianmesh_amd/csrc/gm_sh.h
+++ b/gaussianmesh_amd/csrc/gm_sh.h
@@ -32,6 +32,36 @@
   return r;
 }
 
+template <typename G>
+__device__ __forceinline__ void sh_rgb_streamed(int deg, G granule, float x, float y, float z, float* r) {
+  float b[16];
+  float4 g = granule(0);
+  float e[4] = {g.x, g.y, g.z, g.w};
+#define GM_SH_STREAM(J0, J1)                                                                               \
+  _Pragma("unroll")                                                                                        \
+  for (int j = (J0); j < (J1); j++) {                                                                      \
+    if ((j & 3) == 0) { g = granule(j >> 2); e[0] = g.x; e[1] = g.y; e[2] = g.z; e[3] = g.w; }             \
+    r[j % 3] = r[j % 3] + b[j / 3] * e[j & 3];                                                             \
+  }
+  r[0] = SH_C0 * e[0]; r[1] = SH_C0 * e[1]; r[2] = SH_C0 * e[2];
+  if (deg > 0) {
+    b[1] = -(SH_C1 * y); b[2] = SH_C1 * z; b[3] = -(SH_C1 * x);
+    GM_SH_STREAM(3, 12)
+    if (deg > 1) {
+      const float xx = x * x, yy = y * y, zz = z * z, xy = x * y, yz = y * z, xz = x * z;
+      b[4] = SH_C2[0] * xy; b[5] = SH_C2[1] * yz; b[6] = SH_C2[2] * (2.0f * zz - xx - yy); b[7] = SH_C2[3] * xz; b[8] = SH_C2[4] * (xx - yy);
+      GM_SH_STREAM(12, 27)
+      if (deg > 2) {
+        b[9] = SH_C3[0] * y * (3.0f * xx - yy); b[10] = SH_C3[1] * xy * z; b[11] = SH_C3[2] * y * (4.0f * zz - xx - yy);
+        b[12] = SH_C3[3] * z * (2.0f * zz - 3.0f * xx - 3.0f * yy); b[13] = SH_C3[4] * x * (4.0f * zz - xx - yy);
+        b[14] = SH_C3[5] * z * (xx - yy); b[15] = SH_C3[6] * x * (xx - 3.0f * yy);
+        GM_SH_STREAM(27, 48)
+      }
+    }
+  }
+#undef GM_SH_STREAM
+}
+
 __device__ __forceinline__ void load_sh(const float* __restrict__ shs, size_t idx, int M, int ncoef, float* sh) {
   const float* base = shs + idx * (size_t)M * 3;
   const int nf = ncoef * 3;
diff --git a/include/gmesh_hip.h b/include/gmesh_hip.h
--- a/include/gmesh_hip.h
+++ b/include/gmesh_hip.h
@@ -195,6 +195,7 @@
                                  int n_objects, const int* object_rows, const unsigned int* deformed, const float* pos, const float* scales,
                                  const float* rots, const float* shs, const float* opacities, const int* tri, const float* w, const float* cov,
                                  const float* background, int64_t binning_capacity, int flags, unsigned int* work_hint, int debug, void* stream);
+int gm_fused_batch_occupancy(int* waves_per_cu);
 int gm_mesh_rs_packed_batch(int K, int Vm, int nfaces, const float* V0, const float* const* V1, const int* faces, const int* adj_offsets,
                             const int* adj_faces, float* const* packed, void* stream);
 
```

Result: slower. 4880 frames/s (-1.7%).
